# POSTECH-CVLab/PyTorch-StudioGAN

Measured on AMD Instinct MI355X. Metric: images/sec (G+D step) BigGAN ImageNet-128 bs256, higher is better.
Workload: dtype bf16

## Files before the change

include/sgamd.h:

```cpp
#ifndef SGAMD_H
#define SGAMD_H
#include <stdint.h>
#ifdef __cplusplus
extern "C" {
#endif

typedef void* sg_stream_t;

#define SG_DTYPE_F32 0
#define SG_DTYPE_BF16 1
#define SG_DTYPE_F64 2

#define SG_PIX_RELU 1
#define SG_PIX_UPSAMPLE 2
#define SG_PIX_QUAD 4
#define SG_PIX_TRANSPOSED 8
#define SG_EPI_OUT_F32 1
#define SG_EPI_ATOMIC 2
#define SG_EPI_POOL 4
#define SG_EPI_RELU 8
#define SG_EPI_RES_F32 16

const char* sg_last_error(void);
int sg_version(void);
int sg_prof_enable(int on);
int sg_prof_collect(double* out, int nkinds);

typedef struct {
  int dtype;
  int N, Hs, Ws, C, ldx;
  int Ho, Wo, Cout;
  int R, S, stride, pad_h, pad_w;
  int pix_flags, epi_flags;
  float alpha, beta;
  const void* x; const void* w;
  const float* bias; const void* res; const void* mask; void* out; const float* alpha_ptr;
  int ldo, ldr, ldm;
} sg_conv_fwd_desc;
int sg_conv2d_fwd(const sg_conv_fwd_desc* d, sg_stream_t stream);
int sg_set_f32_mode(int mode);
int sg_get_f32_mode(void);
long long sg_f32_split_launches(int mode);
long long sg_ew_vec_launches(void);

typedef struct {
  sg_conv_fwd_desc main;
  const void* x2; const void* w2; const float* bias2;
  int C2, ldx2, x2_up;
  float* stats;
} sg_conv_skip_desc;
int sg_conv2d_fwd_skip_stat_rows(const sg_conv_skip_desc* d);
int sg_conv2d_fwd_skip(const sg_conv_skip_desc* d, sg_stream_t stream);
int sg_conv2d_fwd_skip_ok(const sg_conv_skip_desc* d);
long long sg_conv_rs_launches(void);

typedef struct {
  sg_conv_fwd_desc conv;
  const float* pre; const float* post; const float* noise;
  long long noise_stride;
} sg_modconv_desc;
int sg_modconv2d_fwd(const sg_modconv_desc* d, sg_stream_t stream);
int sg_modconv2d_ok(const sg_modconv_desc* d);
long long sg_modconv_launches(void);
int sg_modconv_dcoef(const float* w, const float* s, float* Q, float* d, int N, int C, int Cout, int RS, sg_stream_t stream);
int sg_modconv_reduce_slabs(int P);
int sg_modconv_reduce(int dtype, const void* a, const void* b, const float* rowsub, long long rowsub_stride, const float* scale, void* out, float* part,
                      float* rowsum, int N, int P, int C, int lda, int ldb, sg_stream_t stream);

#define SG_Q_POOL 0
#define SG_Q_UP 1
typedef struct {
  int dtype, form;
  int N, Hl, Wl;
  int C, ldx, Cout;
  int pix_flags, epi_flags;
  float alpha, beta;
  const void* x; const void* wq;
  const float* bias; const void* res; const void* mask; void* out; const float* alpha_ptr;
  int ldo, ldr, ldm;
  const void* x2; const void* w2q; const float* bias2;
  int C2, ldx2;
  float* stats;
  int x2_norelu;
} sg_convq_desc;
int sg_conv2d_q_stat_rows(const sg_convq_desc* d);
int sg_conv2d_q(const sg_convq_desc* d, sg_stream_t stream);
int sg_conv2d_q_ok(const sg_convq_desc* d);
int sg_quad_pack(int dtype, int mode, const void* src, void* dst, int M, int Cs, sg_stream_t stream);
typedef struct { const void* src; void* dst; int M, Cs, mode, pad_; } sg_quad_item;
int sg_quad_pack_batch(int dtype, const sg_quad_item* items_dev, const sg_quad_item* items_host, int n, sg_stream_t stream);
typedef struct {
  int dtype, form;
  int N, Hl, Wl;
  int C, ldx, x_flags;
  int Cout, ldg;
  float alpha; const float* alpha_ptr;
  const void* x; const void* dy; float* dw; float* dbias;
  float* work; long long work_floats;
  int splits;
} sg_convq_wgrad_desc;
int sg_conv2d_q_wgrad_plan(const sg_convq_wgrad_desc* d, int* splits, long long* work_floats);
int sg_conv2d_q_wgrad(const sg_convq_wgrad_desc* d, sg_stream_t stream);
int sg_prof_collect_ex(double* out, int nkinds);
int sg_prof_collect_tags(double* out, int ntags);

typedef struct {
  int dtype;
  int N;
  int xHs, xWs, C, ldx, x_flags;
  int gHs, gWs, Cout, ldg, g_flags;
  int Ho, Wo;
  int R, S, stride, pad_h, pad_w;
  float alpha;
  const void* x; const void* dy; float* dw;
  const float* alpha_ptr;
  int splits;
  int no_tr;
  float* work; long long work_floats;
  float* dbias;
} sg_conv_wgrad_desc;
int sg_conv2d_wgrad(const sg_conv_wgrad_desc* d, sg_stream_t stream);
int sg_conv2d_wgrad_fuses_bias(const sg_conv_wgrad_desc* d);
int sg_conv2d_wgrad_plan(const sg_conv_wgrad_desc* d, int* splits, long long* work_floats);

typedef struct {
  int dtype, p_form, q_form;
  int I, J, K, batch;
  const void* p; long long p_bstride; int ldp;
  const void* q; long long q_bstride; int ldq;
  void* out; long long out_bstride; int ldo;
  const float* bias; const void* res; long long res_bstride; int ldr; float beta;
  float alpha; const float* alpha_ptr;
  int epi_flags; int splits; int no_tr;
} sg_gemm_desc;
int sg_gemm(const sg_gemm_desc* d, sg_stream_t stream);
typedef struct { const float* w; const float* y; const float* bias; float* out; int rows, K, ldy, ldo; } sg_linear_item;
int sg_linear_group(const sg_linear_item* items_dev, const sg_linear_item* items_host, int n, int B, sg_stream_t stream);
typedef struct { const float* w; const float* y; const float* bias; float* out; int rows, K, ldy, ldo; float wscale, bscale, oscale; int pad_; } sg_linear_item_scaled;
int sg_linear_group_scaled(const sg_linear_item_scaled* items_dev, const sg_linear_item_scaled* items_host, int n, int B, sg_stream_t stream);
long long sg_linear_group_scaled_launches(void);

int sg_nchw_to_nhwc(int dtype, const float* src, void* dst, int N, int C, int H, int W, int ldo, sg_stream_t s);
int sg_nhwc_to_nchw(int dtype, const void* src, float* dst, int N, int C, int H, int W, int lds, int apply_tanh, sg_stream_t s);
int sg_nchw_grad_to_nhwc(int dtype, const float* dy, const float* y, void* dst, int N, int C, int H, int W, int ldo, int apply_tanh, sg_stream_t s);
int sg_avgpool2_fwd(int dtype, const void* x, void* y, int N, int H, int W, int C, sg_stream_t s);
int sg_avgpool2_bwd(int dtype, const void* dy, void* dx, int N, int H, int W, int C, sg_stream_t s);
int sg_maxpool2_fwd(int dtype, const void* x, int ldx, void* y, int ldy, uint8_t* idx, int N, int H, int W, int C, sg_stream_t s);
int sg_maxpool2_bwd(int dtype, const void* dy, int ldy, const uint8_t* idx, void* dx, int ldx, int N, int H, int W, int C, sg_stream_t s);
int sg_softmax_rows(int dtype, const float* s_in, void* p_out, long long rows, int cols, sg_stream_t st);
int sg_softmax_rows_bwd(int dtype, const void* p, const float* dp, void* ds, long long rows, int cols, sg_stream_t st);
int sg_convert(int src_dtype, int dst_dtype, const void* x, void* y, long long n, sg_stream_t s);
int sg_add_relu(int dtype, const void* a, const void* x, void* out, long long n, sg_stream_t s);
int sg_relu_mask(int dtype, const void* dy, const void* x, void* dx, long long n, sg_stream_t s);
int sg_axpby(int dtype, const void* x, void* y, long long n, float a, float b, sg_stream_t s);
int sg_dot(int dtype, const void* x, const void* y, long long n, float* out, float scale, const float* scale_ptr, sg_stream_t s);
int sg_colsum(int dtype, const void* x, int ldx, const void* mask, int ldm, long long rows, int C, float* out, float alpha, sg_stream_t s);

int sg_bn_partial_stats(int dtype, const void* x, int ldx, long long rows, int C, double* partial, sg_stream_t s);
int sg_bn_stats_from_tiles(const float* stats, int nrows, int C, double* partial, sg_stream_t s);
int sg_bn_finalize(const double* partial, double count, int C, float eps, float momentum, float* mean, float* invstd,
                   float* running_mean, float* running_var, sg_stream_t s);
typedef void* sg_comm_t;
int sg_comm_unique_id(void* out128);
int sg_comm_init_rank(const void* id128, int nranks, int rank, sg_comm_t* comm);
int sg_comm_size(sg_comm_t comm, int* nranks);
int sg_comm_destroy(sg_comm_t comm);
int sg_allreduce_flat(sg_comm_t comm, void* buf, long long count, int dtype, sg_stream_t s);
int sg_bn_stats_sync(int dtype, const void* x, int ldx, long long rows, int C, double* partial, sg_comm_t comm, float eps, float momentum,
                     float* mean, float* invstd, float* running_mean, float* running_var, sg_stream_t s);
int sg_reduce_scatter_flat(sg_comm_t comm, float* buf, long long per_rank, sg_stream_t s);
int sg_allgather_flat(sg_comm_t comm, float* buf, long long per_rank, sg_stream_t s);

typedef void* sg_p2p_t;
int sg_p2p_create(int world, int rank, long long max_doubles, sg_p2p_t* out, void* handle_out64);
int sg_p2p_connect(sg_p2p_t p, const void* handles);
int sg_p2p_destroy(sg_p2p_t p);
int sg_p2p_timeouts(sg_p2p_t p, int* count);
int sg_p2p_allreduce_f64(sg_p2p_t p, double* buf, int n, sg_stream_t s);
int sg_bn_finalize_p2p(sg_p2p_t p, const double* partial, double count, int C, float eps, float momentum, float* mean, float* invstd,
                       float* running_mean, float* running_var, sg_stream_t s);
int sg_bn_stats_sync_p2p(int dtype, const void* x, int ldx, long long rows, int C, double* partial, sg_p2p_t p, float eps, float momentum,
                         float* mean, float* invstd, float* running_mean, float* running_var, sg_stream_t s);
int sg_bn_from_running(const float* running_mean, const float* running_var, int C, float eps, float* mean, float* invstd, sg_stream_t s);
int sg_bn_apply(int dtype, const void* x, void* y, int N, long long HW, int C, const float* mean, const float* invstd,
                const float* gain, const float* bias, int gb_stride_n, int relu, sg_stream_t s);
int sg_bn_bwd_reduce(int dtype, const void* x, const void* dy, int N, long long HW, int C, const float* mean, const float* invstd,
                     const float* gain, const float* bias, int gb_stride_n, int relu, float* sums, sg_stream_t s);
int sg_bn_bwd_finalize(const float* sums, int N, int C, const float* gain, int gb_stride_n, float* dgain, float* dbias,
                       double* chan, sg_stream_t s);
int sg_bn_bwd_apply(int dtype, const void* x, const void* dy, void* dx, int N, long long HW, int C, const float* mean,
                    const float* invstd, const float* gain, const float* bias, int gb_stride_n, int relu,
                    const double* chan, double count, int use_batch_stats, sg_stream_t s);
int sg_bn_bwd_apply_res(int dtype, const void* x, const void* dy, void* dx, int N, long long HW, int C, const float* mean,
                        const float* invstd, const float* gain, const float* bias, int gb_stride_n, int relu,
                        const double* chan, double count, int use_batch_stats, const void* res, sg_stream_t s);

int sg_bn_bwd2_reduce(int dtype, const void* x, const void* dy, const void* u, int N, long long HW, int C, const float* mean,
                      const float* invstd, const float* gain, const float* bias, int relu, float* sums, sg_stream_t s);
int sg_bn_bwd2_finalize(const float* sums, int N, int C, double* chan, sg_stream_t s);
int sg_bn_bwd2_dgain(const double* chan_local, const double* chan, double count, const float* invstd, int C,
                     int use_batch_stats, float* dgain, sg_stream_t s);
int sg_bn_bwd2_apply(int dtype, const void* x, const void* dy, const void* u, void* g_dy, void* g_x, int N, long long HW, int C,
                     const float* mean, const float* invstd, const float* gain, const float* bias, int relu, const double* chan,
                     double count, int use_batch_stats, sg_stream_t s);

int sg_cbn_bwd2_reduce(int dtype, const void* x, const void* dy, const void* u, int N, long long HW, int C, const float* mean,
                       const float* invstd, const float* gain, const float* bias, int gb_stride_n, int relu, float* sums,
                       sg_stream_t s);
int sg_cbn_bwd2_finalize(const float* sums, int N, int C, const float* gain, const float* A, int gb_stride_n, double* chan,
                         sg_stream_t s);
int sg_cbn_bwd2_dgain(const float* sums, const double* chan, double count, const float* invstd, int N, int C, int gb_stride_n,
                      int use_batch_stats, float* dgain, sg_stream_t s);
int sg_cbn_bwd2_apply(int dtype, const void* x, const void* dy, const void* u, void* g_dy, void* g_x, int N, long long HW, int C,
                      const float* mean, const float* invstd, const float* gain, const float* bias, const float* A, const float* B,
                      int gb_stride_n, int relu, const double* chan, double count, int use_batch_stats, sg_stream_t s);

typedef struct {
  const float* w;
  float* u; float* v;
  float* sigma;
  float* u_snap; float* v_snap;
  void* w_fwd;
  void* w_dgrad;
  float* w_f32;
  int rows, cols;
  int Cin, RS;
  int do_power_iter;
  int apply_sn;
  int rows_pad;
  long long work_off;
  int trans;
  int dgrad_noflip;
  int Cin_pad;
} sg_sn_layer;
int sg_sn_forward(int dtype, const sg_sn_layer* layers_dev, const sg_sn_layer* layers_host, int n, float eps, float* work, long long work_floats, sg_stream_t s);

typedef struct {
  const float* dwt;
  const float* w;
  const float* u; const float* v; const float* sigma;
  float* dw;
  int rows, cols, Cin, RS, natural, apply_sn, trans;
  int Cin_pad;
} sg_sn_bwd_layer;
int sg_sn_backward(const sg_sn_bwd_layer* layers_dev, const sg_sn_bwd_layer* layers_host, int n, float* work, long long work_floats, sg_stream_t s);

int sg_embedding_fwd(const float* table, const int64_t* idx, float* out, int B, int dim, int num, sg_stream_t s);
int sg_embedding_bwd(const float* dout, const int64_t* idx, float* dtable, int B, int dim, int num, sg_stream_t s);
int sg_relu_sum_hw_fwd(int dtype, const void* x, float* h, int B, int HW, int C, sg_stream_t s);
int sg_relu_sum_hw_bwd(int dtype, const void* x, const float* dh, void* dx, int B, int HW, int C, sg_stream_t s);
int sg_pd_head_fwd(const float* h, const float* w1, const float* b1, const float* emb, float* adv, int B, int C, sg_stream_t s);
int sg_pd_head_bwd(const float* h, const float* w1, const float* emb, const float* dadv, float* dh, float* dw1, float* db1,
                   float* demb, int B, int C, sg_stream_t s);
int sg_loss_d(int kind, const float* real, const float* fake, int B, float* loss, float* d_real, float* d_fake, sg_stream_t s);
int sg_loss_g(int kind, const float* fake, int B, float* loss, float* d_fake, sg_stream_t s);

int sg_interp_rows(const float* real, const float* fake, const float* alpha, float* out, int B, long long n, sg_stream_t s);
int sg_gp_fwd(int kind, const float* grads, int B, long long n, float* norms, float* loss, sg_stream_t s);
int sg_gp_bwd(int kind, const float* grads, const float* norms, const float* gout, float* dgrads, int B, long long n, sg_stream_t s);
int sg_masked_sum_hw(int dtype, const void* t, const void* x, float* out, int B, int HW, int C, sg_stream_t s);

int sg_attn_fwd_flash_ok(int B, int HW, int HW4, int Dp, int Cg);
int sg_attn_fwd_fused(const void* theta, const void* phi, const void* g, float* lse, void* O, float* O32, int B, int HW, int HW4, int Dp, int Cg, sg_stream_t s);
int sg_attn_bwd_fused_ok(int B, int HW, int HW4, int Dp, int Cg);
int sg_attn_bwd_fused(const void* theta, const void* phi, const void* g, const void* dO, const float* O32, const float* lse, float* delta, void* dtheta, void* dphi,
                      void* dg, int B, int HW, int HW4, int Dp, int Cg, sg_stream_t s);

int sg_attn_proj_ok(int B, int H, int W, int C, int ldx, int Dp, int Cg);
int sg_attn_proj_fwd(const void* x, int ldx, const void* w_theta, const void* w_phi, const void* w_g, void* theta, void* phi, void* g,
                     uint8_t* idx_phi, uint8_t* idx_g, int B, int H, int W, int C, int Dp, int Cg, int relu, sg_stream_t s);
int sg_attn_proj_bwd_data(const void* dtheta, const void* dphi, const void* dg, const uint8_t* idx_phi, const uint8_t* idx_g, const void* wd_theta,
                          const void* wd_phi, const void* wd_g, const void* res, void* dx, int B, int H, int W, int C, int Dp, int Cg, sg_stream_t s);

int sg_slice_up_fwd(int dtype, const void* x, void* y, int N, int Hs, int Ws, int ldx, int C, int up, sg_stream_t s);
int sg_slice_up_bwd(int dtype, const void* dy, void* dx, int N, int Hs, int Ws, int ldx, int C, int up, sg_stream_t s);
int sg_copy_channels(int dtype, const void* src, int ld_src, void* dst, int ld_dst, long long rows, int C, sg_stream_t s);

int sg_adam_ema(float* p, const float* g, float* m, float* v, float* ema, long long n, float lr, float beta1, float beta2,
                float eps, float wd, int step, float ema_decay, float grad_scale, sg_stream_t s);
int sg_ema_lerp(const float* src, float* ema, long long n, float decay, sg_stream_t s);

int sg_lecam(const float* real, const float* fake, int B, float ema_real, float ema_fake, float* loss, float* d_real, float* d_fake, sg_stream_t s);
int sg_u8_to_nhwc(int dtype, const uint8_t* x, const uint8_t* flip, void* y, int N, int H, int W, int cpad, sg_stream_t s);

int sg_quantize_resize_normalize(int dtype, const float* x, void* out, uint8_t* quant_out, int N, int C, int H, int W,
                                 int OH, int OW, int quantize, sg_stream_t s);
int sg_quantize_resize_normalize_ms(int dtype, const float* x, void* out, uint8_t* quant_out, int N, int C, int H, int W,
                                    int OH, int OW, int quantize, const float* mean, const float* std, sg_stream_t s);
int sg_pool2d(int dtype, const void* x, void* y, int N, int H, int W, int C, int k, int stride, int pad, int mode, int ldy, int c_off, sg_stream_t s);
int sg_pil_resize_normalize(int dtype, const float* x, void* out, float* tmp, int N, int C, int H, int W, int OH, int OW,
                            const int* bounds_h, const double* kk_h, int ksize_h, const int* bounds_v, const double* kk_v, int ksize_v,
                            int quantize, sg_stream_t s);
int sg_pil_resize_normalize_ms(int dtype, const float* x, void* out, float* tmp, int N, int C, int H, int W, int OH, int OW,
                               const int* bounds_h, const double* kk_h, int ksize_h, const int* bounds_v, const double* kk_v, int ksize_v,
                               int quantize, const float* mean, const float* std, sg_stream_t s);
int sg_global_avgpool(int dtype, const void* x, float* y, int N, int HW, int C, sg_stream_t s);
int sg_topk_hits(const float* scores, int ld, int ncls, const int64_t* labels, int k, int N, uint8_t* hits, sg_stream_t s);
int sg_topk_select(const float* x, int n, int k, float* vals, int* idx, sg_stream_t s);
int sg_topk_scatter(const float* g, const int* idx, int k, float* dx, int n, sg_stream_t s);
int sg_feat_moments_accumulate(const float* f, int n, int C, double* sum_f, double* sum_ff, sg_stream_t s);
int sg_gather_images_u8(const uint8_t* src, const int64_t* idx, const uint8_t* flip, uint8_t* dst, int B, int H, int W,
                        const int64_t* lab_src, int64_t* lab_dst, sg_stream_t s);
int sg_row_normalize_fwd(const float* x, float* y, float* inv, int rows, int cols, float eps, sg_stream_t s);
int sg_row_normalize_bwd(const float* y, const float* inv, const float* dy, float* dx, int rows, int cols, sg_stream_t s);
int sg_row_dot(const float* a, const float* b, float* p, int rows, int cols, sg_stream_t s);
int sg_row_scale(const float* g, const float* x, float* out, int rows, int cols, int accumulate, sg_stream_t s);
int sg_class_loss(int kind, const float* z, const int64_t* label, int rows, int cols, float* row_loss, float* loss, float* dz, sg_stream_t s);
int sg_contrastive_loss(int kind, const float* S, const float* p, const int64_t* label, int B, float temperature, float m_p,
                        float* row_loss, float* loss, float* dS, float* dp, sg_stream_t s);
int sg_gather_cols(const float* z, const int64_t* label, int rows, int cols, float* out, sg_stream_t s);
int sg_scatter_cols(const float* g, const int64_t* label, int rows, int cols, float* dz, sg_stream_t s);
int sg_layernorm_rows(int out_dtype, const float* x, long long pitch, const float* gamma, const float* beta, void* y, long long ldo, int rows, int C,
                      float eps, sg_stream_t s);
int sg_vit_tokens(const float* patch, const float* cls, const float* pos, float* x, int B, int N, int C, sg_stream_t s);
int sg_gelu_f32(const float* x, float* y, long long n, sg_stream_t s);
int sg_tok_gemm(int epi, const void* a, int lda, const void* w, const float* bias, void* out, int ldo, int M, int N, int K, sg_stream_t s);
int sg_mha_fwd_ok(int B, int N, int H, int D);
int sg_mha_fwd(const void* qkv, void* out, int B, int N, int H, int D, float scale, sg_stream_t s);
long long sg_tok_gemm_launches(void);
long long sg_mha_launches(void);

int sg_row_sqnorm(const float* f, int n, int C, float* sq, sg_stream_t s);
int sg_kth_smallest_rows(const float* D, long long ld, int rows, int cols, int k, const float* row_add, float* out, sg_stream_t s);
int sg_prdc_rows(const float* D, long long ld, int rows, int cols, const float* row_add, const float* r2_row, const float* r2_col,
                 int* col_cnt, uint8_t* row_any, float* row_min, sg_stream_t s);
int sg_chol_lower(double* A, int n, int* flag, sg_stream_t s);
int sg_dgemm_tn(const double* A, const double* B, double* C, int n, sg_stream_t s);
int sg_jacobi_sweep(double* M, int n, double* offd, sg_stream_t s);
int sg_row_norm_sum(const double* M, int n, double* out, sg_stream_t s);
int sg_seg_moments(const float* f, const long long* seg, int K, int C, double* mu, double* tr, sg_stream_t s);
int sg_seg_cross_gram(const float* fa, const long long* sega, const double* mua, const float* fb, const long long* segb, const double* mub, int K, int C,
                      double* M, const long long* moff, sg_stream_t s);
int sg_seg_nuclear_norm(const double* M, const long long* moff, const int* rows, const int* cols, int K, int max_sweeps, double tol,
                        double* nuc, double* offd, int* sweeps, sg_stream_t s);
int sg_seg_nuclear_fits(int rows, int cols);
int sg_seg_nuclear_lds_budget(void);

int sg_bias_act(int dtype, const void* x, const void* b, const void* xref, const void* yref, const void* dy, void* y, long long n,
                long long step_b, int size_b, int grad, int act, float alpha, float gain, float clamp, sg_stream_t s);
int sg_upfirdn2d(int dtype, const void* x, const float* f, void* y, int planes, int H, int W, int fh, int fw, int upx, int upy,
                 int downx, int downy, int padx0, int padx1, int pady0, int pady1, int flip_filter, float gain, sg_stream_t s);
int sg_filtered_lrelu(int dtype, const void* x, const float* fu, const float* fd, const void* b, void* y, int N, int C, int H, int W,
                      int fu_n, int fd_n, int up, int down, int px0, int px1, int py0, int py1, float gain, float slope, float clamp,
                      int flip_filter, sg_stream_t s);
int sg_fir_bias_act_nhwc(int dtype, const void* x, const float* f, void* y, const float* noise, long long noise_stride, const float* bias,
                         int N, int Hi, int Wi, int C, int fh, int fw, int padx0, int padx1, int pady0, int pady1, int flip_filter,
                         float filter_gain, int act, float alpha, float gain, float clamp, sg_stream_t s);
long long sg_fir_bias_act_launches(void);

#define SG_AUG_BRIGHTNESS 1
#define SG_AUG_SATURATION 2
#define SG_AUG_CONTRAST 4
#define SG_AUG_FLIP 8
#define SG_AUG_TRANSLATE 16
#define SG_AUG_TRANSLATE_REFLECT 32
#define SG_AUG_CUTOUT 64
typedef struct {
  int N, C, H, W;
  int ops;
  int cut_h, cut_w;
  int max_t;
  const float* color;
  const int* geom;
} sg_aug_desc;
int sg_augment_work_floats(const sg_aug_desc* d);
int sg_augment_fwd(const sg_aug_desc* d, const float* x, float* y, float* work, sg_stream_t s);
int sg_augment_bwd(const sg_aug_desc* d, const float* dy, float* dx, float* work, sg_stream_t s);
int sg_mse_work_floats(void);
int sg_mse_fwd(const float* a, const float* b, long long n, float* work, float* loss, sg_stream_t s);
int sg_mse_bwd(const float* a, const float* b, const float* gout, long long n, float* da, float* db, sg_stream_t s);
int sg_loss_ls_d(const float* real, const float* fake, int B, float* loss, float* d_real, float* d_fake, sg_stream_t s);
int sg_loss_ls_g(const float* fake, int B, float* loss, float* d_fake, sg_stream_t s);
int sg_fm_work_floats(int C);
int sg_fm_loss(const float* real_h, const float* fake_h, int B, int C, float* work, float* loss, float* d_fake, sg_stream_t s);
int sg_exp_fwd(const float* x, float* y, long long n, sg_stream_t s);
int sg_exp_bwd(const float* dy, const float* y, float* dx, long long n, sg_stream_t s);
int sg_normal_nll(const float* x, const float* mu, const float* var, int B, int K, float* loss, float* dmu, float* dvar, sg_stream_t s);
int sg_maxpool2_gather(int dtype, const void* x, int ldx, const uint8_t* idx, void* y, int ldy, int N, int H, int W, int C, sg_stream_t s);
int sg_softmax_rows_bwd2(const float* P, const float* dP, const float* u, float* gP, long long rows, int cols, sg_stream_t s);
int sg_scale_by_ptr(int dtype, const void* x, const float* sigma, void* y, long long n, sg_stream_t s);
int sg_tanh_bwd(const float* dy, const float* y, float* t, long long n, sg_stream_t s);
int sg_tanh_bwd2(const float* g, const float* dy, const float* y, float* out, long long n, sg_stream_t s);
int sg_clamp_flat(float* p, long long n, float lo, float hi, sg_stream_t s);
int sg_select_rows(const uint8_t* flag, const float* a, const float* b, float* out, int N, long long row, sg_stream_t s);
int sg_sign_count(const float* logit, int B, float* acc, sg_stream_t s);
int sg_reflect_pad2d_fwd(const float* x, float* y, int planes, int H, int W, int l, int r, int t, int b, sg_stream_t s);
int sg_reflect_pad2d_bwd(const float* dy, float* dx, int planes, int H, int W, int l, int r, int t, int b, sg_stream_t s);
int sg_affine_sample_fwd(const float* x, const float* theta, float* y, int N, int C, int Hi, int Wi, int Ho, int Wo, sg_stream_t s);
int sg_affine_sample_bwd(const float* dy, const float* theta, float* dx, int N, int C, int Hi, int Wi, int Ho, int Wo, sg_stream_t s);
int sg_color_affine(const float* x, const float* M, float* y, int N, int C, int HW, int transpose, sg_stream_t s);
int sg_fir_reflect(const float* x, const float* taps, float* y, int N, int C, int H, int W, int T, int axis, int transpose, sg_stream_t s);
int sg_ada_noise_cutout(const float* x, const float* noise, const float* sigma, const float* cut, float* y, int N, int C, int H, int W, sg_stream_t s);

#ifdef __cplusplus
}
#endif
#endif
```

pytorch-studiogan_amd/_lib.py:

```python
import ctypes as C
import os
import subprocess
import sys

import torch

_HERE = os.path.dirname(os.path.abspath(__file__))
LIB_PATH = os.path.join(_HERE, "libsgamd.so")
if os.environ.get("SG_LIBSGAMD"):
    LIB_PATH = os.path.abspath(os.environ["SG_LIBSGAMD"])
CSRC = os.path.join(_HERE, "csrc")

F32, BF16, F64 = 0, 1, 2
PIX_RELU, PIX_UPSAMPLE, PIX_QUAD, PIX_TRANSPOSED = 1, 2, 4, 8
Q_POOL, Q_UP = 0, 1
EPI_OUT_F32, EPI_ATOMIC, EPI_POOL, EPI_RELU, EPI_RES_F32 = 1, 2, 4, 8, 16

_vp, _i, _f, _ll = C.c_void_p, C.c_int, C.c_float, C.c_longlong


class ConvFwdDesc(C.Structure):
    _fields_ = [("dtype", _i), ("N", _i), ("Hs", _i), ("Ws", _i), ("C", _i), ("ldx", _i), ("Ho", _i), ("Wo", _i), ("Cout", _i),
                ("R", _i), ("S", _i), ("stride", _i), ("pad_h", _i), ("pad_w", _i), ("pix_flags", _i), ("epi_flags", _i),
                ("alpha", _f), ("beta", _f), ("x", _vp), ("w", _vp), ("bias", _vp), ("res", _vp), ("mask", _vp), ("out", _vp),
                ("alpha_ptr", _vp), ("ldo", _i), ("ldr", _i), ("ldm", _i)]


class ConvSkipDesc(C.Structure):
    _fields_ = [("main", ConvFwdDesc), ("x2", _vp), ("w2", _vp), ("bias2", _vp), ("C2", _i), ("ldx2", _i), ("x2_up", _i), ("stats", _vp)]


class ModConvDesc(C.Structure):
    _fields_ = [("conv", ConvFwdDesc), ("pre", _vp), ("post", _vp), ("noise", _vp), ("noise_stride", _ll)]


class ConvWgradDesc(C.Structure):
    _fields_ = [("dtype", _i), ("N", _i), ("xHs", _i), ("xWs", _i), ("C", _i), ("ldx", _i), ("x_flags", _i), ("gHs", _i), ("gWs", _i),
                ("Cout", _i), ("ldg", _i), ("g_flags", _i), ("Ho", _i), ("Wo", _i), ("R", _i), ("S", _i), ("stride", _i),
                ("pad_h", _i), ("pad_w", _i), ("alpha", _f), ("x", _vp), ("dy", _vp), ("dw", _vp), ("alpha_ptr", _vp),
                ("splits", _i), ("no_tr", _i), ("work", _vp), ("work_floats", _ll), ("dbias", _vp)]


class ConvQDesc(C.Structure):
    _fields_ = [("dtype", _i), ("form", _i), ("N", _i), ("Hl", _i), ("Wl", _i), ("C", _i), ("ldx", _i), ("Cout", _i),
                ("pix_flags", _i), ("epi_flags", _i), ("alpha", _f), ("beta", _f), ("x", _vp), ("wq", _vp), ("bias", _vp), ("res", _vp),
                ("mask", _vp), ("out", _vp), ("alpha_ptr", _vp), ("ldo", _i), ("ldr", _i), ("ldm", _i),
                ("x2", _vp), ("w2q", _vp), ("bias2", _vp), ("C2", _i), ("ldx2", _i), ("stats", _vp), ("x2_norelu", _i)]


class ConvQWgradDesc(C.Structure):
    _fields_ = [("dtype", _i), ("form", _i), ("N", _i), ("Hl", _i), ("Wl", _i), ("C", _i), ("ldx", _i), ("x_flags", _i), ("Cout", _i),
                ("ldg", _i), ("alpha", _f), ("alpha_ptr", _vp), ("x", _vp), ("dy", _vp), ("dw", _vp), ("dbias", _vp), ("work", _vp),
                ("work_floats", _ll), ("splits", _i)]


class QuadItem(C.Structure):
    _fields_ = [("src", _vp), ("dst", _vp), ("M", _i), ("Cs", _i), ("mode", _i), ("pad_", _i)]


class LinearItem(C.Structure):
    _fields_ = [("w", _vp), ("y", _vp), ("bias", _vp), ("out", _vp), ("rows", _i), ("K", _i), ("ldy", _i), ("ldo", _i)]


class LinearItemScaled(C.Structure):
    _fields_ = [("w", _vp), ("y", _vp), ("bias", _vp), ("out", _vp), ("rows", _i), ("K", _i), ("ldy", _i), ("ldo", _i),
                ("wscale", _f), ("bscale", _f), ("oscale", _f), ("pad_", _i)]


class GemmDesc(C.Structure):
    _fields_ = [("dtype", _i), ("p_form", _i), ("q_form", _i), ("I", _i), ("J", _i), ("K", _i), ("batch", _i),
                ("p", _vp), ("p_bstride", _ll), ("ldp", _i), ("q", _vp), ("q_bstride", _ll), ("ldq", _i),
                ("out", _vp), ("out_bstride", _ll), ("ldo", _i), ("bias", _vp), ("res", _vp), ("res_bstride", _ll), ("ldr", _i),
                ("beta", _f), ("alpha", _f), ("alpha_ptr", _vp), ("epi_flags", _i), ("splits", _i), ("no_tr", _i)]


class SnLayer(C.Structure):
    _fields_ = [("w", _vp), ("u", _vp), ("v", _vp), ("sigma", _vp), ("u_snap", _vp), ("v_snap", _vp), ("w_fwd", _vp), ("w_dgrad", _vp),
                ("w_f32", _vp), ("rows", _i), ("cols", _i), ("Cin", _i), ("RS", _i), ("do_power_iter", _i), ("apply_sn", _i),
                ("rows_pad", _i), ("work_off", _ll), ("trans", _i), ("dgrad_noflip", _i), ("Cin_pad", _i)]


class SnBwdLayer(C.Structure):
    _fields_ = [("dwt", _vp), ("w", _vp), ("u", _vp), ("v", _vp), ("sigma", _vp), ("dw", _vp), ("rows", _i), ("cols", _i),
                ("Cin", _i), ("RS", _i), ("natural", _i), ("apply_sn", _i), ("trans", _i), ("Cin_pad", _i)]


class AugDesc(C.Structure):
    _fields_ = [("N", _i), ("C", _i), ("H", _i), ("W", _i), ("ops", _i), ("cut_h", _i), ("cut_w", _i), ("max_t", _i), ("color", _vp), ("geom", _vp)]


AUG_BRIGHTNESS, AUG_SATURATION, AUG_CONTRAST, AUG_FLIP, AUG_TRANSLATE, AUG_TRANSLATE_REFLECT, AUG_CUTOUT = 1, 2, 4, 8, 16, 32, 64

_lib = None


def build(force=False, verbose=False):
    cmd = ["make", "-C", CSRC, "-j", str(max(2, os.cpu_count() or 2))]
    if force:
        subprocess.run(["make", "-C", CSRC, "clean"], check=True, stdout=subprocess.DEVNULL)
    res = subprocess.run(cmd, stdout=subprocess.PIPE, stderr=subprocess.STDOUT, text=True)
    if verbose or res.returncode != 0:
        sys.stderr.write(res.stdout)
    if res.returncode != 0:
        raise RuntimeError("building libsgamd.so failed")
    return LIB_PATH


_PROTOS = {
    "sg_prof_enable": [_i],
    "sg_prof_collect": [C.POINTER(C.c_double), _i],
    "sg_conv2d_fwd": [C.POINTER(ConvFwdDesc), _vp],
    "sg_conv2d_fwd_skip": [C.POINTER(ConvSkipDesc), _vp],
    "sg_conv2d_fwd_skip_ok": [C.POINTER(ConvSkipDesc)],
    "sg_conv_rs_launches": [],
    "sg_modconv2d_fwd": [C.POINTER(ModConvDesc), _vp],
    "sg_modconv2d_ok": [C.POINTER(ModConvDesc)],
    "sg_modconv_launches": [],
    "sg_modconv_dcoef": [_vp, _vp, _vp, _vp, _i, _i, _i, _i, _vp],
    "sg_modconv_reduce_slabs": [_i],
    "sg_modconv_reduce": [_i, _vp, _vp, _vp, _ll, _vp, _vp, _vp, _vp, _i, _i, _i, _i, _i, _vp],
    "sg_conv2d_q": [C.POINTER(ConvQDesc), _vp],
    "sg_conv2d_q_ok": [C.POINTER(ConvQDesc)],
    "sg_conv2d_q_stat_rows": [C.POINTER(ConvQDesc)],
    "sg_conv2d_fwd_skip_stat_rows": [C.POINTER(ConvSkipDesc)],
    "sg_bn_stats_from_tiles": [_vp, _i, _i, _vp, _vp],
    "sg_quad_pack": [_i, _i, _vp, _vp, _i, _i, _vp],
    "sg_quad_pack_batch": [_i, _vp, C.POINTER(QuadItem), _i, _vp],
    "sg_linear_group": [_vp, C.POINTER(LinearItem), _i, _i, _vp],
    "sg_linear_group_scaled": [_vp, C.POINTER(LinearItemScaled), _i, _i, _vp],
    "sg_linear_group_scaled_launches": [],
    "sg_conv2d_q_wgrad_plan": [C.POINTER(ConvQWgradDesc), C.POINTER(_i), C.POINTER(_ll)],
    "sg_conv2d_q_wgrad": [C.POINTER(ConvQWgradDesc), _vp],
    "sg_prof_collect_ex": [C.POINTER(C.c_double), _i],
    "sg_prof_collect_tags": [C.POINTER(C.c_double), _i],
    "sg_conv2d_wgrad": [C.POINTER(ConvWgradDesc), _vp],
    "sg_conv2d_wgrad_plan": [C.POINTER(ConvWgradDesc), C.POINTER(_i), C.POINTER(_ll)],
    "sg_conv2d_wgrad_fuses_bias": [C.POINTER(ConvWgradDesc)],
    "sg_gemm": [C.POINTER(GemmDesc), _vp],
    "sg_nchw_to_nhwc": [_i, _vp, _vp, _i, _i, _i, _i, _i, _vp],
    "sg_nhwc_to_nchw": [_i, _vp, _vp, _i, _i, _i, _i, _i, _i, _vp],
    "sg_nchw_grad_to_nhwc": [_i, _vp, _vp, _vp, _i, _i, _i, _i, _i, _i, _vp],
    "sg_avgpool2_fwd": [_i, _vp, _vp, _i, _i, _i, _i, _vp],
    "sg_avgpool2_bwd": [_i, _vp, _vp, _i, _i, _i, _i, _vp],
    "sg_maxpool2_fwd": [_i, _vp, _i, _vp, _i, _vp, _i, _i, _i, _i, _vp],
    "sg_maxpool2_bwd": [_i, _vp, _i, _vp, _vp, _i, _i, _i, _i, _i, _vp],
    "sg_softmax_rows": [_i, _vp, _vp, _ll, _i, _vp],
    "sg_softmax_rows_bwd": [_i, _vp, _vp, _vp, _ll, _i, _vp],
    "sg_axpby": [_i, _vp, _vp, _ll, _f, _f, _vp],
    "sg_convert": [_i, _i, _vp, _vp, _ll, _vp],
    "sg_add_relu": [_i, _vp, _vp, _vp, _ll, _vp],
    "sg_relu_mask": [_i, _vp, _vp, _vp, _ll, _vp],
    "sg_dot": [_i, _vp, _vp, _ll, _vp, _f, _vp, _vp],
    "sg_colsum": [_i, _vp, _i, _vp, _i, _ll, _i, _vp, _f, _vp],
    "sg_bn_partial_stats": [_i, _vp, _i, _ll, _i, _vp, _vp],
    "sg_bn_finalize": [_vp, C.c_double, _i, _f, _f, _vp, _vp, _vp, _vp, _vp],
    "sg_comm_unique_id": [_vp],
    "sg_comm_init_rank": [_vp, _i, _i, C.POINTER(_vp)],
    "sg_comm_size": [_vp, C.POINTER(_i)],
    "sg_comm_destroy": [_vp],
    "sg_allreduce_flat": [_vp, _vp, _ll, _i, _vp],
    "sg_bn_stats_sync": [_i, _vp, _i, _ll, _i, _vp, _vp, _f, _f, _vp, _vp, _vp, _vp, _vp],
    "sg_set_f32_mode": [_i],
    "sg_get_f32_mode": [],
    "sg_f32_split_launches": [_i],
    "sg_ew_vec_launches": [],
    "sg_reduce_scatter_flat": [_vp, _vp, _ll, _vp],
    "sg_allgather_flat": [_vp, _vp, _ll, _vp],
    "sg_p2p_create": [_i, _i, _ll, C.POINTER(_vp), _vp],
    "sg_p2p_connect": [_vp, _vp],
    "sg_p2p_destroy": [_vp],
    "sg_p2p_timeouts": [_vp, C.POINTER(_i)],
    "sg_p2p_allreduce_f64": [_vp, _vp, _i, _vp],
    "sg_bn_finalize_p2p": [_vp, _vp, C.c_double, _i, _f, _f, _vp, _vp, _vp, _vp, _vp],
    "sg_bn_stats_sync_p2p": [_i, _vp, _i, _ll, _i, _vp, _vp, _f, _f, _vp, _vp, _vp, _vp, _vp],
    "sg_bn_from_running": [_vp, _vp, _i, _f, _vp, _vp, _vp],
    "sg_bn_apply": [_i, _vp, _vp, _i, _ll, _i, _vp, _vp, _vp, _vp, _i, _i, _vp],
    "sg_bn_bwd_reduce": [_i, _vp, _vp, _i, _ll, _i, _vp, _vp, _vp, _vp, _i, _i, _vp, _vp],
    "sg_bn_bwd_finalize": [_vp, _i, _i, _vp, _i, _vp, _vp, _vp, _vp],
    "sg_bn_bwd_apply": [_i, _vp, _vp, _vp, _i, _ll, _i, _vp, _vp, _vp, _vp, _i, _i, _vp, C.c_double, _i, _vp],
    "sg_bn_bwd_apply_res": [_i, _vp, _vp, _vp, _i, _ll, _i, _vp, _vp, _vp, _vp, _i, _i, _vp, C.c_double, _i, _vp, _vp],
    "sg_bn_bwd2_reduce": [_i, _vp, _vp, _vp, _i, _ll, _i, _vp, _vp, _vp, _vp, _i, _vp, _vp],
    "sg_bn_bwd2_finalize": [_vp, _i, _i, _vp, _vp],
    "sg_bn_bwd2_dgain": [_vp, _vp, C.c_double, _vp, _i, _i, _vp, _vp],
    "sg_bn_bwd2_apply": [_i, _vp, _vp, _vp, _vp, _vp, _i, _ll, _i, _vp, _vp, _vp, _vp, _i, _vp, C.c_double, _i, _vp],
    "sg_cbn_bwd2_reduce": [_i, _vp, _vp, _vp, _i, _ll, _i, _vp, _vp, _vp, _vp, _i, _i, _vp, _vp],
    "sg_cbn_bwd2_finalize": [_vp, _i, _i, _vp, _vp, _i, _vp, _vp],
    "sg_cbn_bwd2_dgain": [_vp, _vp, C.c_double, _vp, _i, _i, _i, _i, _vp, _vp],
    "sg_cbn_bwd2_apply": [_i, _vp, _vp, _vp, _vp, _vp, _i, _ll, _i, _vp, _vp, _vp, _vp, _vp, _vp, _i, _i, _vp, C.c_double, _i, _vp],
    "sg_attn_fwd_flash_ok": [_i, _i, _i, _i, _i],
    "sg_attn_fwd_fused": [_vp, _vp, _vp, _vp, _vp, _vp, _i, _i, _i, _i, _i, _vp],
    "sg_attn_bwd_fused_ok": [_i, _i, _i, _i, _i],
    "sg_attn_bwd_fused": [_vp, _vp, _vp, _vp, _vp, _vp, _vp, _vp, _vp, _vp, _i, _i, _i, _i, _i, _vp],
    "sg_attn_proj_ok": [_i, _i, _i, _i, _i, _i, _i],
    "sg_attn_proj_fwd": [_vp, _i, _vp, _vp, _vp, _vp, _vp, _vp, _vp, _vp, _i, _i, _i, _i, _i, _i, _i, _vp],
    "sg_attn_proj_bwd_data": [_vp, _vp, _vp, _vp, _vp, _vp, _vp, _vp, _vp, _vp, _i, _i, _i, _i, _i, _i, _vp],
    "sg_slice_up_fwd": [_i, _vp, _vp, _i, _i, _i, _i, _i, _i, _vp],
    "sg_slice_up_bwd": [_i, _vp, _vp, _i, _i, _i, _i, _i, _i, _vp],
    "sg_copy_channels": [_i, _vp, _i, _vp, _i, _ll, _i, _vp],
    "sg_interp_rows": [_vp, _vp, _vp, _vp, _i, _ll, _vp],
    "sg_gp_fwd": [_i, _vp, _i, _ll, _vp, _vp, _vp],
    "sg_gp_bwd": [_i, _vp, _vp, _vp, _vp, _i, _ll, _vp],
    "sg_masked_sum_hw": [_i, _vp, _vp, _vp, _i, _i, _i, _vp],
    "sg_sn_forward": [_i, _vp, C.POINTER(SnLayer), _i, _f, _vp, _ll, _vp],
    "sg_sn_backward": [_vp, C.POINTER(SnBwdLayer), _i, _vp, _ll, _vp],
    "sg_embedding_fwd": [_vp, _vp, _vp, _i, _i, _i, _vp],
    "sg_embedding_bwd": [_vp, _vp, _vp, _i, _i, _i, _vp],
    "sg_relu_sum_hw_fwd": [_i, _vp, _vp, _i, _i, _i, _vp],
    "sg_relu_sum_hw_bwd": [_i, _vp, _vp, _vp, _i, _i, _i, _vp],
    "sg_pd_head_fwd": [_vp, _vp, _vp, _vp, _vp, _i, _i, _vp],
    "sg_pd_head_bwd": [_vp, _vp, _vp, _vp, _vp, _vp, _vp, _vp, _i, _i, _vp],
    "sg_loss_d": [_i, _vp, _vp, _i, _vp, _vp, _vp, _vp],
    "sg_loss_g": [_i, _vp, _i, _vp, _vp, _vp],
    "sg_adam_ema": [_vp, _vp, _vp, _vp, _vp, _ll, _f, _f, _f, _f, _f, _i, _f, _f, _vp],
    "sg_ema_lerp": [_vp, _vp, _ll, _f, _vp],
    "sg_quantize_resize_normalize": [_i, _vp, _vp, _vp, _i, _i, _i, _i, _i, _i, _i, _vp],
    "sg_pil_resize_normalize": [_i, _vp, _vp, _vp, _i, _i, _i, _i, _i, _i, _vp, _vp, _i, _vp, _vp, _i, _i, _vp],
    "sg_quantize_resize_normalize_ms": [_i, _vp, _vp, _vp, _i, _i, _i, _i, _i, _i, _i, C.POINTER(_f), C.POINTER(_f), _vp],
    "sg_pil_resize_normalize_ms": [_i, _vp, _vp, _vp, _i, _i, _i, _i, _i, _i, _vp, _vp, _i, _vp, _vp, _i, _i, C.POINTER(_f), C.POINTER(_f), _vp],
    "sg_layernorm_rows": [_i, _vp, _ll, _vp, _vp, _vp, _ll, _i, _i, _f, _vp],
    "sg_vit_tokens": [_vp, _vp, _vp, _vp, _i, _i, _i, _vp],
    "sg_gelu_f32": [_vp, _vp, _ll, _vp],
    "sg_tok_gemm": [_i, _vp, _i, _vp, _vp, _vp, _i, _i, _i, _i, _vp],
    "sg_mha_fwd_ok": [_i, _i, _i, _i],
    "sg_mha_fwd": [_vp, _vp, _i, _i, _i, _i, _f, _vp],
    "sg_tok_gemm_launches": [],
    "sg_mha_launches": [],
    "sg_pool2d": [_i, _vp, _vp, _i, _i, _i, _i, _i, _i, _i, _i, _i, _i, _vp],
    "sg_global_avgpool": [_i, _vp, _vp, _i, _i, _i, _vp],
    "sg_feat_moments_accumulate": [_vp, _i, _i, _vp, _vp, _vp],
    "sg_topk_hits": [_vp, _i, _i, _vp, _i, _i, _vp, _vp],
    "sg_row_normalize_fwd": [_vp, _vp, _vp, _i, _i, _f, _vp],
    "sg_row_normalize_bwd": [_vp, _vp, _vp, _vp, _i, _i, _vp],
    "sg_row_dot": [_vp, _vp, _vp, _i, _i, _vp],
    "sg_row_scale": [_vp, _vp, _vp, _i, _i, _i, _vp],
    "sg_class_loss": [_i, _vp, _vp, _i, _i, _vp, _vp, _vp, _vp],
    "sg_contrastive_loss": [_i, _vp, _vp, _vp, _i, _f, _f, _vp, _vp, _vp, _vp, _vp],
    "sg_gather_cols": [_vp, _vp, _i, _i, _vp, _vp],
    "sg_scatter_cols": [_vp, _vp, _i, _i, _vp, _vp],
    "sg_chol_lower": [_vp, _i, _vp, _vp],
    "sg_dgemm_tn": [_vp, _vp, _vp, _i, _vp],
    "sg_jacobi_sweep": [_vp, _i, _vp, _vp],
    "sg_row_norm_sum": [_vp, _i, _vp, _vp],
    "sg_seg_moments": [_vp, _vp, _i, _i, _vp, _vp, _vp],
    "sg_seg_cross_gram": [_vp, _vp, _vp, _vp, _vp, _vp, _i, _i, _vp, _vp, _vp],
    "sg_seg_nuclear_norm": [_vp, _vp, _vp, _vp, _i, _i, C.c_double, _vp, _vp, _vp, _vp],
    "sg_seg_nuclear_fits": [_i, _i],
    "sg_seg_nuclear_lds_budget": [],
    "sg_row_sqnorm": [_vp, _i, _i, _vp, _vp],
    "sg_kth_smallest_rows": [_vp, _ll, _i, _i, _i, _vp, _vp, _vp],
    "sg_prdc_rows": [_vp, _ll, _i, _i, _vp, _vp, _vp, _vp, _vp, _vp, _vp],
    "sg_topk_select": [_vp, _i, _i, _vp, _vp, _vp],
    "sg_lecam": [_vp, _vp, _i, _f, _f, _vp, _vp, _vp, _vp],
    "sg_u8_to_nhwc": [_i, _vp, _vp, _vp, _i, _i, _i, _i, _vp],
    "sg_gather_images_u8": [_vp, _vp, _vp, _vp, _i, _i, _i, _vp, _vp, _vp],
    "sg_topk_scatter": [_vp, _vp, _i, _vp, _i, _vp],
    "sg_bias_act": [_i, _vp, _vp, _vp, _vp, _vp, _vp, _ll, _ll, _i, _i, _i, _f, _f, _f, _vp],
    "sg_upfirdn2d": [_i, _vp, _vp, _vp, _i, _i, _i, _i, _i, _i, _i, _i, _i, _i, _i, _i, _i, _i, _f, _vp],
    "sg_filtered_lrelu": [_i, _vp, _vp, _vp, _vp, _vp, _i, _i, _i, _i, _i, _i, _i, _i, _i, _i, _i, _i, _f, _f, _f, _i, _vp],
    "sg_fir_bias_act_nhwc": [_i, _vp, _vp, _vp, _vp, _ll, _vp, _i, _i, _i, _i, _i, _i, _i, _i, _i, _i, _i, _f, _i, _f, _f, _f, _vp],
    "sg_fir_bias_act_launches": [],
    "sg_augment_work_floats": [C.POINTER(AugDesc)],
    "sg_augment_fwd": [C.POINTER(AugDesc), _vp, _vp, _vp, _vp],
    "sg_augment_bwd": [C.POINTER(AugDesc), _vp, _vp, _vp, _vp],
    "sg_mse_work_floats": [],
    "sg_mse_fwd": [_vp, _vp, _ll, _vp, _vp, _vp],
    "sg_mse_bwd": [_vp, _vp, _vp, _ll, _vp, _vp, _vp],
    "sg_loss_ls_d": [_vp, _vp, _i, _vp, _vp, _vp, _vp],
    "sg_loss_ls_g": [_vp, _i, _vp, _vp, _vp],
    "sg_fm_work_floats": [_i],
    "sg_fm_loss": [_vp, _vp, _i, _i, _vp, _vp, _vp, _vp],
    "sg_exp_fwd": [_vp, _vp, _ll, _vp],
    "sg_exp_bwd": [_vp, _vp, _vp, _ll, _vp],
    "sg_normal_nll": [_vp, _vp, _vp, _i, _i, _vp, _vp, _vp, _vp],
    "sg_maxpool2_gather": [_i, _vp, _i, _vp, _vp, _i, _i, _i, _i, _i, _vp],
    "sg_softmax_rows_bwd2": [_vp, _vp, _vp, _vp, _ll, _i, _vp],
    "sg_scale_by_ptr": [_i, _vp, _vp, _vp, _ll, _vp],
    "sg_tanh_bwd": [_vp, _vp, _vp, _ll, _vp],
    "sg_tanh_bwd2": [_vp, _vp, _vp, _vp, _ll, _vp],
    "sg_clamp_flat": [_vp, _ll, _f, _f, _vp],
    "sg_select_rows": [_vp, _vp, _vp, _vp, _i, _ll, _vp],
    "sg_sign_count": [_vp, _i, _vp, _vp],
    "sg_reflect_pad2d_fwd": [_vp, _vp, _i, _i, _i, _i, _i, _i, _i, _vp],
    "sg_reflect_pad2d_bwd": [_vp, _vp, _i, _i, _i, _i, _i, _i, _i, _vp],
    "sg_affine_sample_fwd": [_vp, _vp, _vp, _i, _i, _i, _i, _i, _i, _vp],
    "sg_affine_sample_bwd": [_vp, _vp, _vp, _i, _i, _i, _i, _i, _i, _vp],
    "sg_color_affine": [_vp, _vp, _vp, _i, _i, _i, _i, _vp],
    "sg_fir_reflect": [_vp, _vp, _vp, _i, _i, _i, _i, _i, _i, _i, _vp],
    "sg_ada_noise_cutout": [_vp, _vp, _vp, _vp, _vp, _i, _i, _i, _i, _vp],
}


def exported_symbols():
    return sorted(list(_PROTOS.keys()) + ["sg_last_error", "sg_version"])


def lib():
    global _lib
    if _lib is None:
        if not os.path.exists(LIB_PATH):
            raise RuntimeError(
                f"{LIB_PATH} is missing: run `python -c 'import __graft_entry__ as g; g.build()'` (make -C {CSRC}). "
                "There is no CPU/eager fallback on the product path.")
        l = C.CDLL(LIB_PATH)
        l.sg_last_error.restype = C.c_char_p
        l.sg_version.restype = _i
        for name, args in _PROTOS.items():
            fn = getattr(l, name)
            fn.argtypes = args
            fn.restype = _i
        l.sg_conv_rs_launches.restype = _ll
        l.sg_modconv_launches.restype = _ll
        l.sg_tok_gemm_launches.restype = _ll
        l.sg_mha_launches.restype = _ll
        l.sg_f32_split_launches.restype = _ll
        l.sg_ew_vec_launches.restype = _ll
        l.sg_linear_group_scaled_launches.restype = _ll
        l.sg_fir_bias_act_launches.restype = _ll
        f32_mode = {"bf16x3": 3, "bf16x6": 6}.get(os.environ.get("SG_F32_MODE", "exact"), 0)
        if f32_mode:
            l.sg_set_f32_mode(f32_mode)
        _lib = l
    return _lib


def check(rc, name=""):
    if rc != 0:
        raise RuntimeError(f"{name}: {lib().sg_last_error().decode()} (rc={rc})")


_STATE_WRITERS = frozenset(("sg_adam_ema", "sg_ema_lerp", "sg_allreduce_flat", "sg_clamp_flat", "sg_allgather_flat"))
write_epoch = [0]


def call(name, *args):
    if name in _STATE_WRITERS:
        write_epoch[0] += 1
    rc = getattr(lib(), name)(*args)
    if rc != 0:
        raise RuntimeError(f"{name}: {lib().sg_last_error().decode()} (rc={rc})")


def stream():
    return torch.cuda.current_stream().cuda_stream


def upload_bytes(raw, device):
    t = torch.frombuffer(bytearray(raw), dtype=torch.uint8)
    if torch.device(device).type == "cuda":
        return t.pin_memory().to(device, non_blocking=True)
    return t.to(device)


def dt(t):
    d = t if isinstance(t, torch.dtype) else t.dtype
    if d == torch.float32:
        return F32
    if d == torch.bfloat16:
        return BF16
    raise RuntimeError(f"unsupported dtype {d} (float32 / bfloat16 only)")


def require_gpu(dev):
    if dev.type != "cuda":
        raise RuntimeError("studiogan_amd modules run on the GPU only (no CPU fallback on the product path)")


def ptr(t):
    if t is None:
        return None
    if not t.is_cuda:
        raise RuntimeError("studiogan_amd kernels need a GPU tensor (no CPU fallback on the product path)")
    return t.data_ptr()
```

pytorch-studiogan_amd/backbones/big_resnet.py:

```python
import torch
import torch.nn as nn

from .. import functional as F
from .. import ops
from ..bank import get_bank
from .heads import build_heads, apply_heads


def _dtype(mixed_precision):
    return torch.bfloat16 if mixed_precision else torch.float32


def _need_graph(module, *inputs):
    if not torch.is_grad_enabled():
        return False
    for t in inputs:
        if torch.is_tensor(t) and t.requires_grad:
            return True
    return any(p.requires_grad for p in module.parameters())


class GenBlock(nn.Module):
    def __init__(self, in_channels, out_channels, g_cond_mtd, affine_input_dim, MODULES):
        super().__init__()
        self.g_cond_mtd = g_cond_mtd
        self.bn1 = MODULES.g_bn(affine_input_dim, in_channels, MODULES)
        self.bn2 = MODULES.g_bn(affine_input_dim, out_channels, MODULES)
        self.activation = MODULES.g_act_fn
        self.conv2d0 = MODULES.g_conv2d(in_channels=in_channels, out_channels=out_channels, kernel_size=1, stride=1, padding=0)
        self.conv2d1 = MODULES.g_conv2d(in_channels=in_channels, out_channels=out_channels, kernel_size=3, stride=1, padding=1)
        self.conv2d2 = MODULES.g_conv2d(in_channels=out_channels, out_channels=out_channels, kernel_size=3, stride=1, padding=1)

    def forward_nhwc(self, x, affine, slot):
        link = F.GradLink()
        h = self.bn1.forward_nhwc(x, affine, slot, relu=True, link=link)
        h = self.conv2d1.forward_nhwc(h, slot, in_upsample=True, stats=True)
        h = self.bn2.forward_nhwc(h, affine, slot, relu=True)
        return ops.conv_skip_nhwc(self.conv2d2, self.conv2d0, h, x, slot, skip_upsample=True, link=link, stats=True)


class Generator(nn.Module):
    def __init__(self, z_dim, g_shared_dim, img_size, g_conv_dim, apply_attn, attn_g_loc, g_cond_mtd, num_classes, g_init, g_depth,
                 mixed_precision, MODULES, MODEL):
        super().__init__()
        g_in_dims_collection = {
            "32": [g_conv_dim * 4, g_conv_dim * 4, g_conv_dim * 4],
            "64": [g_conv_dim * 16, g_conv_dim * 8, g_conv_dim * 4, g_conv_dim * 2],
            "128": [g_conv_dim * 16, g_conv_dim * 16, g_conv_dim * 8, g_conv_dim * 4, g_conv_dim * 2],
            "256": [g_conv_dim * 16, g_conv_dim * 16, g_conv_dim * 8, g_conv_dim * 8, g_conv_dim * 4, g_conv_dim * 2],
            "512": [g_conv_dim * 16, g_conv_dim * 16, g_conv_dim * 8, g_conv_dim * 8, g_conv_dim * 4, g_conv_dim * 2, g_conv_dim]
        }
        g_out_dims_collection = {
            "32": [g_conv_dim * 4, g_conv_dim * 4, g_conv_dim * 4],
            "64": [g_conv_dim * 8, g_conv_dim * 4, g_conv_dim * 2, g_conv_dim],
            "128": [g_conv_dim * 16, g_conv_dim * 8, g_conv_dim * 4, g_conv_dim * 2, g_conv_dim],
            "256": [g_conv_dim * 16, g_conv_dim * 8, g_conv_dim * 8, g_conv_dim * 4, g_conv_dim * 2, g_conv_dim],
            "512": [g_conv_dim * 16, g_conv_dim * 8, g_conv_dim * 8, g_conv_dim * 4, g_conv_dim * 2, g_conv_dim, g_conv_dim]
        }
        self.z_dim = z_dim
        self.g_shared_dim = g_shared_dim
        self.g_cond_mtd = g_cond_mtd
        self.num_classes = num_classes
        self.mixed_precision = mixed_precision
        self.MODEL = MODEL
        self.in_dims = g_in_dims_collection[str(img_size)]
        self.out_dims = g_out_dims_collection[str(img_size)]
        self.bottom = 4
        self.num_blocks = len(self.in_dims)
        self.chunk_size = z_dim // (self.num_blocks + 1)
        self.affine_input_dim = self.chunk_size
        assert self.z_dim % (self.num_blocks + 1) == 0, "z_dim should be divided by the number of blocks"
        self.info_type = getattr(MODEL, "info_type", "N/A")
        self.g_info_injection = getattr(MODEL, "g_info_injection", "N/A")
        info_dim = 0
        if self.info_type in ("discrete", "both"):
            info_dim += MODEL.info_num_discrete_c * MODEL.info_dim_discrete_c
        if self.info_type in ("continuous", "both"):
            info_dim += MODEL.info_num_conti_c
        if self.info_type != "N/A":
            if self.g_info_injection == "concat":
                self.info_mix_linear = MODULES.g_linear(in_features=self.z_dim + info_dim, out_features=self.z_dim, bias=True)
            elif self.g_info_injection == "cBN":
                self.affine_input_dim += self.g_shared_dim
                self.info_proj_linear = MODULES.g_linear(in_features=info_dim, out_features=self.g_shared_dim, bias=True)
            else:
                raise NotImplementedError(f"g_info_injection = {self.g_info_injection}")

        self.linear0 = MODULES.g_linear(in_features=self.chunk_size, out_features=self.in_dims[0] * self.bottom * self.bottom, bias=True)
        if self.g_cond_mtd != "W/O":
            self.affine_input_dim += self.g_shared_dim
            self.shared = ops.embedding(num_embeddings=self.num_classes, embedding_dim=self.g_shared_dim)

        blocks = []
        for index in range(self.num_blocks):
            blocks += [[GenBlock(in_channels=self.in_dims[index], out_channels=self.out_dims[index], g_cond_mtd=self.g_cond_mtd,
                                 affine_input_dim=self.affine_input_dim, MODULES=MODULES)]]
            if index + 1 in attn_g_loc and apply_attn:
                blocks += [[ops.SelfAttention(self.out_dims[index], is_generator=True, MODULES=MODULES)]]
        self.blocks = nn.ModuleList([nn.ModuleList(block) for block in blocks])

        self.bn4 = ops.batchnorm_2d(in_features=self.out_dims[-1])
        self.activation = MODULES.g_act_fn
        self.conv2d5 = MODULES.g_conv2d(in_channels=self.out_dims[-1], out_channels=3, kernel_size=3, stride=1, padding=1)
        self.tanh = nn.Tanh()
        self.conv2d5._sg_rows_pad = 8
        ops.init_weights(self.modules, g_init)
        ops.adopt(self, _dtype(mixed_precision))

    def forward(self, z, label, shared_label=None, eval=False):
        dtype = self.compute_dtype
        bank = get_bank(self, dtype)
        slot = bank.begin_forward(_need_graph(self, z, shared_label))
        affine_list = []
        if self.info_type != "N/A":
            if self.g_info_injection == "concat":
                z = self.info_mix_linear.forward_rt(z, slot)
            else:
                z, z_info = z[:, :self.z_dim], z[:, self.z_dim:]
                affine_list.append(self.info_proj_linear.forward_rt(z_info, slot))
        zs = torch.split(z, self.chunk_size, 1)
        z0 = zs[0]
        if self.g_cond_mtd != "W/O":
            if shared_label is None:
                shared_label = self.shared(label)
            affine_list.append(shared_label)
        if len(affine_list) == 0:
            affines = [item for item in zs[1:]]
        else:
            affines = [torch.cat(affine_list + [item], 1) for item in zs[1:]]

        pairs, counter = [], 0
        for blocklist in self.blocks:
            for block in blocklist:
                if not isinstance(block, ops.SelfAttention):
                    if isinstance(block.bn1, ops.ConditionalBatchNorm2d):
                        pairs += [(block.bn1, affines[counter]), (block.bn2, affines[counter])]
                    counter += 1
        F.cbn_prefetch(slot, pairs)

        act = self.linear0.forward_rt(z0, slot)
        act = F.NchwToNhwcFn.apply(act.view(-1, self.in_dims[0], self.bottom, self.bottom), dtype)
        act = ops.block_boundary(self, -1, act)
        counter = 0
        nxt = bank.boundaries(self.blocks) if bank.exchange is not None else None
        with ops.bump_batches_tracked(self):
            for bi, blocklist in enumerate(self.blocks):
                for block in blocklist:
                    if isinstance(block, ops.SelfAttention):
                        act = block.forward_nhwc(act, slot)
                    else:
                        act = block.forward_nhwc(act, affines[counter], slot)
                        counter += 1
                if nxt is not None:
                    act = bank.mark(act, nxt[bi])
                act = ops.block_boundary(self, bi, act)
            act = self.bn4.forward_nhwc(act, relu=True)
        act = self.conv2d5.forward_nhwc(act, slot)
        return F.NhwcToNchwFn.apply(act, True, 3)


class DiscOptBlock(nn.Module):
    def __init__(self, in_channels, out_channels, apply_d_sn, MODULES):
        super().__init__()
        self.apply_d_sn = apply_d_sn
        self.conv2d0 = MODULES.d_conv2d(in_channels=in_channels, out_channels=out_channels, kernel_size=1, stride=1, padding=0)
        self.conv2d1 = MODULES.d_conv2d(in_channels=in_channels, out_channels=out_channels, kernel_size=3, stride=1, padding=1)
        self.conv2d2 = MODULES.d_conv2d(in_channels=out_channels, out_channels=out_channels, kernel_size=3, stride=1, padding=1)
        if not apply_d_sn:
            self.bn0 = MODULES.d_bn(in_features=in_channels)
            self.bn1 = MODULES.d_bn(in_features=out_channels)
        self.activation = MODULES.d_act_fn
        self.average_pooling = nn.AvgPool2d(2)
        self.cpad = 8 if (apply_d_sn and in_channels < 8) else 0
        if self.cpad:
            self.conv2d1._sg_cin_pad = self.conv2d0._sg_cin_pad = self.cpad

    def forward_nhwc(self, x, slot):
        h = self.conv2d1.forward_nhwc(x, slot)
        if not self.apply_d_sn:
            h = self.bn1.forward_nhwc(h, relu=True)
            h = self.conv2d2.forward_nhwc(h, slot, out_pool=True)
        else:
            if self.cpad == 8 and h.dtype == torch.bfloat16 and not x.requires_grad:
                return ops.conv_skip_nhwc(self.conv2d2, self.conv2d0, h, x, slot, in_relu=True, out_pool=True, skip_relu=False)
            h = self.conv2d2.forward_nhwc(h, slot, in_relu=True, out_pool=True)
        x0 = F.AvgPool2Fn.apply(x)
        if not self.apply_d_sn:
            x0 = self.bn0.forward_nhwc(x0)
        return self.conv2d0.forward_nhwc(x0, slot, res=h)


class DiscBlock(nn.Module):
    def __init__(self, in_channels, out_channels, apply_d_sn, MODULES, downsample=True):
        super().__init__()
        self.apply_d_sn = apply_d_sn
        self.downsample = downsample
        self.activation = MODULES.d_act_fn
        self.ch_mismatch = in_channels != out_channels
        if self.ch_mismatch or downsample:
            self.conv2d0 = MODULES.d_conv2d(in_channels=in_channels, out_channels=out_channels, kernel_size=1, stride=1, padding=0)
            if not apply_d_sn:
                self.bn0 = MODULES.d_bn(in_features=in_channels)
        self.conv2d1 = MODULES.d_conv2d(in_channels=in_channels, out_channels=out_channels, kernel_size=3, stride=1, padding=1)
        self.conv2d2 = MODULES.d_conv2d(in_channels=out_channels, out_channels=out_channels, kernel_size=3, stride=1, padding=1)
        if not apply_d_sn:
            self.bn1 = MODULES.d_bn(in_features=in_channels)
            self.bn2 = MODULES.d_bn(in_features=out_channels)
        self.average_pooling = nn.AvgPool2d(2)

    def forward_nhwc(self, x, slot):
        if self.apply_d_sn:
            if self.downsample or self.ch_mismatch:
                link = F.GradLink()
                h = self.conv2d1.forward_nhwc(x, slot, in_relu=True, link=link)
                return ops.conv_skip_nhwc(self.conv2d2, self.conv2d0, h, x, slot, in_relu=True, out_pool=self.downsample, link=link)
            h = self.conv2d1.forward_nhwc(x, slot, in_relu=True)
            h = self.conv2d2.forward_nhwc(h, slot, in_relu=True, out_pool=False)
            return F.AddReluFn.apply(h, x)
        h = self.bn1.forward_nhwc(x, relu=True)
        h = self.conv2d1.forward_nhwc(h, slot)
        h = self.bn2.forward_nhwc(h, relu=True)
        h = self.conv2d2.forward_nhwc(h, slot, out_pool=self.downsample)
        if self.downsample or self.ch_mismatch:
            x0 = self.bn0.forward_nhwc(x)
            return self.conv2d0.forward_nhwc(x0, slot, out_pool=self.downsample, res=h)
        return F.AddFn.apply(h, x)


class Discriminator(nn.Module):
    def __init__(self, img_size, d_conv_dim, apply_d_sn, apply_attn, attn_d_loc, d_cond_mtd, aux_cls_type, d_embed_dim, normalize_d_embed,
                 num_classes, d_init, d_depth, mixed_precision, MODULES, MODEL):
        super().__init__()
        d_in_dims_collection = {
            "32": [3] + [d_conv_dim * 2, d_conv_dim * 2, d_conv_dim * 2],
            "64": [3] + [d_conv_dim, d_conv_dim * 2, d_conv_dim * 4, d_conv_dim * 8],
            "128": [3] + [d_conv_dim, d_conv_dim * 2, d_conv_dim * 4, d_conv_dim * 8, d_conv_dim * 16],
            "256": [3] + [d_conv_dim, d_conv_dim * 2, d_conv_dim * 4, d_conv_dim * 8, d_conv_dim * 8, d_conv_dim * 16],
            "512": [3] + [d_conv_dim, d_conv_dim, d_conv_dim * 2, d_conv_dim * 4, d_conv_dim * 8, d_conv_dim * 8, d_conv_dim * 16]
        }
        d_out_dims_collection = {
            "32": [d_conv_dim * 2, d_conv_dim * 2, d_conv_dim * 2, d_conv_dim * 2],
            "64": [d_conv_dim, d_conv_dim * 2, d_conv_dim * 4, d_conv_dim * 8, d_conv_dim * 16],
            "128": [d_conv_dim, d_conv_dim * 2, d_conv_dim * 4, d_conv_dim * 8, d_conv_dim * 16, d_conv_dim * 16],
            "256": [d_conv_dim, d_conv_dim * 2, d_conv_dim * 4, d_conv_dim * 8, d_conv_dim * 8, d_conv_dim * 16, d_conv_dim * 16],
            "512": [d_conv_dim, d_conv_dim, d_conv_dim * 2, d_conv_dim * 4, d_conv_dim * 8, d_conv_dim * 8, d_conv_dim * 16, d_conv_dim * 16]
        }
        d_down = {
            "32": [True, True, False, False],
            "64": [True, True, True, True, False],
            "128": [True, True, True, True, True, False],
            "256": [True, True, True, True, True, True, False],
            "512": [True, True, True, True, True, True, True, False]
        }
        self.d_cond_mtd = d_cond_mtd
        self.aux_cls_type = aux_cls_type
        self.normalize_d_embed = normalize_d_embed
        self.num_classes = num_classes
        self.mixed_precision = mixed_precision
        self.in_dims = d_in_dims_collection[str(img_size)]
        self.out_dims = d_out_dims_collection[str(img_size)]
        self.MODEL = MODEL
        down = d_down[str(img_size)]

        blocks = []
        for index in range(len(self.in_dims)):
            if index == 0:
                blocks += [[DiscOptBlock(in_channels=self.in_dims[index], out_channels=self.out_dims[index], apply_d_sn=apply_d_sn, MODULES=MODULES)]]
            else:
                blocks += [[DiscBlock(in_channels=self.in_dims[index], out_channels=self.out_dims[index], apply_d_sn=apply_d_sn,
                                      MODULES=MODULES, downsample=down[index])]]
            if index + 1 in attn_d_loc and apply_attn:
                blocks += [[ops.SelfAttention(self.out_dims[index], is_generator=False, MODULES=MODULES)]]
        self.blocks = nn.ModuleList([nn.ModuleList(block) for block in blocks])
        self.activation = MODULES.d_act_fn
        build_heads(self, MODULES, self.out_dims[-1], d_cond_mtd, aux_cls_type, d_embed_dim, num_classes, MODEL)
        if d_init:
            ops.init_weights(self.modules, d_init)
        ops.adopt(self, _dtype(mixed_precision))

    def forward(self, x, label, eval=False, adc_fake=False):
        dtype = self.compute_dtype
        bank = get_bank(self, dtype)
        slot = bank.begin_forward(_need_graph(self, x))
        h = ops.to_nhwc(x, dtype, self.blocks[0][0].cpad)
        nxt = bank.boundaries(self.blocks) if bank.exchange is not None else None
        for bi, blocklist in enumerate(self.blocks):
            for block in blocklist:
                h = block.forward_nhwc(h, slot)
            if nxt is not None:
                h = bank.mark(h, nxt[bi])
            h = ops.block_boundary(self, bi, h)
        hw = h.shape[1] * h.shape[2]
        h = F.ReluSumFn.apply(h)
        return apply_heads(self, h, label, slot, adc_fake, hw=hw)
```

pytorch-studiogan_amd/csrc/conv.hip:

```cpp
#include <type_traits>
#include "conv_common.h"
#include "conv_v2.h"

int g_sg_f32_mode = 0;
long long g_sg_f32_split_launches[2] = {0, 0};
extern "C" int sg_set_f32_mode(int mode) {
  SG_CHECK(mode == 0 || mode == 3 || mode == 6, "sg_set_f32_mode: 0 (exact fp32 MFMA), 3 (bf16x3 split) or 6 (bf16x6 split)");
  g_sg_f32_mode = mode;
  return 0;
}
extern "C" int sg_get_f32_mode() { return g_sg_f32_mode; }
extern "C" long long sg_f32_split_launches(int mode) {
  if (mode != 3 && mode != 6) return -1;
  return __atomic_load_n(&g_sg_f32_split_launches[mode == 6], __ATOMIC_RELAXED);
}

template <typename T, bool FAST>
static void conv_fwd_launch(const sg_conv_fwd_desc* d, const Epilogue<T>& e, int I, int J, int K, int pflags, hipStream_t st) {
  typedef StridedKC<T, FAST> LP;
  typedef ConvPixKC<T, FAST> LQ;
  LP lp;
  lp.base = (const T*)d->w; lp.bstride = 0; lp.ld = K; lp.rows = I; lp.K = K;
  lp.vec_ok = (K % ET<T>::VEC == 0) && aligned16(d->w);
  LQ lq;
  fill_geom<T>(lq.g, d->x, d->N, d->Hs, d->Ws, d->C, d->ldx, d->Ho, d->Wo, d->R, d->S, d->stride, d->pad_h, d->pad_w, pflags);
  lq.rows = J; lq.K = K;
  if constexpr (sizeof(T) == 4 && FAST) {
    const int mode = g_sg_f32_mode;
    if (mode == 3) { sg_f32_split_count(3); return conv_fwd_tiles<T, LP, LQ, 3>(lp, lq, e, I, J, K, st); }
    if (mode == 6) { sg_f32_split_count(6); return conv_fwd_tiles<T, LP, LQ, 6>(lp, lq, e, I, J, K, st); }
  }
  conv_fwd_tiles<T, LP, LQ, 0>(lp, lq, e, I, J, K, st);
}

static bool conv_fwd_v2_try(const ConvFwdProblem& pb, hipStream_t st) {
  const sg_conv_fwd_desc* d = pb.d;
  const int I = pb.I, J = pb.J, K = pb.K, pflags = pb.pflags;
  const char mode = env_mode("SG_CONV_V2");
  const bool force = mode == 'f';
  if (mode == '0' || (pflags & SG_PIX_TRANSPOSED)) return false;
  if (d->stride != 1 && (d->stride != 2 || (pflags & (SG_PIX_UPSAMPLE | SG_PIX_QUAD)))) return false;
  if (d->C % 8 || d->ldx % 8 || d->R * d->S > 25 || J < 256) return false;
  if (pb.xbytes >= (1ll << 31) || pb.wbytes >= (1ll << 30)) return false;
  if (!aligned16(d->x) || !aligned16(d->w)) return false;
  if (!epi_bf16_rows_ok(pb.e)) return false;
  const int tj = (J + 255) / 256;
  int best_tiles = 0;
  int best = cout_tile_search(I, tj, best_tiles);
  if (!best && I % 8 == 0 && I >= 32) {
    int best_pad = 0;
    for (int c = 0; c < 3; c++) {
      const int padded = ((I + kCoutTiles[c] - 1) / kCoutTiles[c]) * kCoutTiles[c];
      if (2 * padded > 3 * I) continue;
      const int tiles = (padded / kCoutTiles[c]) * tj;
      if (!best || padded < best_pad) { best = kCoutTiles[c]; best_pad = padded; best_tiles = tiles; }
    }
  }
  int min_tiles = 160;
  if (const char* mt = getenv("SG_CONV_V2_MIN_TILES")) { const int v = atoi(mt); if (v > 0) min_tiles = v; }
  if (!best || (best_tiles < min_tiles && !force)) return false;
  ConvV2Params p;
  p.x = (const bf16_t*)d->x; p.w = (const bf16_t*)d->w;
  p.N = d->N; p.Hs = d->Hs; p.Ws = d->Ws; p.C = d->C; p.ldx = d->ldx;
  p.Hin = d->Hs * (pb.up ? 2 : 1); p.Win = d->Ws * (pb.up ? 2 : 1); p.Ho = d->Ho; p.Wo = d->Wo;
  p.R = d->R; p.S = d->S; p.pad_h = d->pad_h; p.pad_w = d->pad_w; p.flags = pflags; p.stride = d->stride;
  p.I = I; p.J = J; p.K = K; p.cpt = d->C / 8; p.ntap = d->R * d->S;
  p.wshift = pb.wshift; p.hshift = pb.hshift;
  p.xbytes = (unsigned)pb.xbytes; p.wbytes = (unsigned)pb.wbytes;
  const Epilogue<bf16_t>& e = pb.e;
  int rc = 0;
  if (best == 192) rc = sg_launch_conv_v2<192, 4, 2, 256, 7>(p, e, st);
  else if (best == 128) rc = sg_launch_conv_v2<128, 4, 2, 256, 7>(p, e, st);
  else {
    if (J >= 512 * 256) rc = sg_launch_conv_v2<96, 8, 1, 512, 1>(p, e, st);
    else rc = sg_launch_conv_v2<96, 8, 1, 256, 1>(p, e, st);
  }
  return rc == 0;
}

template <typename T> static int conv_fwd_t(const sg_conv_fwd_desc* d, hipStream_t st) {
  const int K = d->R * d->S * d->C;
  const int I = d->Cout;
  const long long Jll = (long long)d->N * d->Ho * d->Wo;
  SG_CHECK(Jll < (1ll << 31), "sg_conv2d_fwd: too many output pixels");
  SG_CHECK((long long)d->N * d->Hs * d->Ws * d->ldx < (1ll << 31), "sg_conv2d_fwd: input tensor too large for 32-bit element offsets");
  const int J = (int)Jll;
  int pflags = d->pix_flags;
  if (d->epi_flags & SG_EPI_POOL) {
    SG_CHECK((d->Ho % 2 == 0) && (d->Wo % 2 == 0), "sg_conv2d_fwd: pooled output needs even Ho, Wo");
    pflags |= SG_PIX_QUAD;
  } else {
    pflags &= ~SG_PIX_QUAD;
  }
  const bool w_vec = (K % ET<T>::VEC == 0) && aligned16(d->w);
  const bool x_vec = (d->C % ET<T>::VEC == 0) && (d->ldx % ET<T>::VEC == 0) && aligned16(d->x);
  const Epilogue<T> e = make_epilogue<T>(d, I, J);
  const int prof = sg_prof_begin(st, 2.0 * (double)I * (double)J * (double)K, 0);
  int eng = SG_ENG_CONV_GEMM;
  if constexpr (std::is_same_v<T, bf16_t>) {
    if (w_vec && x_vec) {
      const ConvFwdProblem pb = conv_fwd_problem(d, e, I, J, K, pflags);
      if (sg_conv_fwd_sk_try(pb, st)) eng = SG_ENG_CONV_SK;
      else if (sg_conv_fwd_rs_try(pb, st)) eng = SG_ENG_CONV_RS;
      else if (sg_conv_fwd_v4_try(pb, st)) eng = SG_ENG_CONV_V4;
      else if (sg_conv_fwd_v3_try(pb, st)) eng = SG_ENG_CONV_V3;
      else if (conv_fwd_v2_try(pb, st)) eng = SG_ENG_CONV_V2;
    }
  }
  if (eng == SG_ENG_CONV_GEMM) {
    if (w_vec && x_vec) conv_fwd_launch<T, true>(d, e, I, J, K, pflags, st);
    else conv_fwd_launch<T, false>(d, e, I, J, K, pflags, st);
  }
  {
    const double es = sizeof(T), jout = (d->epi_flags & SG_EPI_POOL) ? (double)J / 4.0 : (double)J;
    const double b = es * ((double)d->N * d->Hs * d->Ws * d->C + (double)I * K + jout * I * (1.0 + (d->mask ? 1.0 : 0.0) + (d->res ? 1.0 : 0.0)));
    sg_prof_tag(prof, eng, b);
  }
  sg_prof_end(st, prof);
  SG_LAUNCH_CHECK();
  return 0;
}

static int conv_fwd_skip(const sg_conv_skip_desc* sk, hipStream_t st, bool dry) {
  const sg_conv_fwd_desc* d = &sk->main;
  if (d->dtype != SG_DTYPE_BF16 || d->R != 3 || d->S != 3 || d->stride != 1 || (d->pix_flags & (SG_PIX_UPSAMPLE | SG_PIX_TRANSPOSED))) return 0;
  const int K = 9 * d->C, I = d->Cout;
  const long long Jll = (long long)d->N * d->Ho * d->Wo;
  if (Jll >= (1ll << 31) || (long long)d->N * d->Hs * d->Ws * d->ldx >= (1ll << 31)) return 0;
  const int J = (int)Jll;
  int pflags = d->pix_flags;
  if (d->epi_flags & SG_EPI_POOL) { if ((d->Ho & 1) || (d->Wo & 1)) return 0; pflags |= SG_PIX_QUAD; } else pflags &= ~SG_PIX_QUAD;
  const ConvFwdProblem pb = conv_fwd_problem(d, make_epilogue<bf16_t>(d, I, J), I, J, K, pflags);
  if (dry) return sg_conv_fwd_v4_skip_try(pb, sk, st, true) ? 1 : 0;
  const int prof = sg_prof_begin(st, 2.0 * (double)I * (double)J * ((double)K + (double)sk->C2), 0);
  const bool ok = sg_conv_fwd_v4_skip_try(pb, sk, st, false);
  {
    const double jout = (d->epi_flags & SG_EPI_POOL) ? (double)J / 4.0 : (double)J;
    const double x2 = (double)d->N * (sk->x2_up ? (d->Ho / 2) * (d->Wo / 2) : d->Ho * d->Wo) * sk->C2;
    sg_prof_tag(prof, SG_ENG_CONV_V4_SKIP, 2.0 * ((double)d->N * d->Hs * d->Ws * d->C + x2 + (double)I * (K + sk->C2) + jout * I));
  }
  sg_prof_end(st, prof);
  return ok ? 1 : 0;
}
extern "C" int sg_conv2d_fwd_skip_stat_rows(const sg_conv_skip_desc* d) {
  if (!d) return 0;
  const long long J = (long long)d->main.N * d->main.Ho * d->main.Wo;
  return (int)((J + 255) / 256);
}
extern "C" int sg_conv2d_fwd_skip_ok(const sg_conv_skip_desc* d) {
  if (!d || !d->main.x || !d->main.w || !d->main.out || !d->x2 || !d->w2) return 0;
  return conv_fwd_skip(d, nullptr, true);
}
extern "C" int sg_conv2d_fwd_skip(const sg_conv_skip_desc* d, sg_stream_t stream) {
  SG_CHECK(d && d->main.x && d->main.w && d->main.out && d->x2 && d->w2, "sg_conv2d_fwd_skip: null pointer");
  SG_CHECK(conv_fwd_skip(d, (hipStream_t)stream, false) == 1, "sg_conv2d_fwd_skip: problem not eligible for the fused kernel (ask sg_conv2d_fwd_skip_ok first)");
  SG_LAUNCH_CHECK();
  return 0;
}

extern "C" int sg_conv2d_fwd(const sg_conv_fwd_desc* d, sg_stream_t stream) {
  SG_CHECK(d && d->x && d->w && d->out, "sg_conv2d_fwd: null pointer");
  SG_CHECK(d->N > 0 && d->C > 0 && d->Cout > 0 && d->R > 0 && d->S > 0 && d->stride > 0, "sg_conv2d_fwd: bad shape");
  SG_CHECK(!(d->epi_flags & SG_EPI_ATOMIC), "sg_conv2d_fwd: atomic epilogue not supported");
  if (d->dtype == SG_DTYPE_F32) return conv_fwd_t<float>(d, (hipStream_t)stream);
  if (d->dtype == SG_DTYPE_BF16) return conv_fwd_t<bf16_t>(d, (hipStream_t)stream);
  sg_set_error("sg_conv2d_fwd: bad dtype");
  return -1;
}
```

pytorch-studiogan_amd/csrc/conv_common.h:

```cpp
#pragma once
#include <stdlib.h>
#include "gemm_core.h"
#include "../../include/sgamd.h"

static inline int ilog2_exact(int v) {
  if (v <= 0 || (v & (v - 1))) return -1;
  int s = 0;
  while ((1 << s) < v) s++;
  return s;
}
static inline bool aligned16(const void* p) { return (((uintptr_t)p) & 15) == 0; }

template <typename T>
static void fill_geom(PixGeom<T>& g, const void* x, int N, int Hs, int Ws, int C, int ldx, int Ho, int Wo, int R, int S,
                      int stride, int pad_h, int pad_w, int flags) {
  g.x = (const T*)x; g.N = N; g.Hs = Hs; g.Ws = Ws;
  const int up = (flags & SG_PIX_UPSAMPLE) ? 2 : 1;
  g.Hin = Hs * up; g.Win = Ws * up; g.C = C; g.ldx = ldx; g.Ho = Ho; g.Wo = Wo;
  g.R = R; g.S = S; g.stride = stride; g.pad_h = pad_h; g.pad_w = pad_w; g.flags = flags;
  g.vec_ok = (C % ET<T>::VEC == 0) && (ldx % ET<T>::VEC == 0) && aligned16(x);
  g.wshift = ilog2_exact(Wo); g.hshift = ilog2_exact(Ho);
}

static inline char env_mode(const char* name) { const char* m = getenv(name); return m ? m[0] : 0; }

static inline long long bf16_extent(long long npix, int ld, int C) { return ((npix - 1) * ld + C) * 2; }

template <typename D> static inline bool is_3x3_s1_p1(const D* d) { return d->R == 3 && d->S == 3 && d->stride == 1 && d->pad_h == 1 && d->pad_w == 1; }

static inline int cout_blocks(int Cout) { return Cout % 96 == 0 ? 3 : Cout % 64 == 0 ? 2 : 0; }

static const int kCoutTiles[3] = {192, 128, 96};
static inline int cout_tile_search(int I, int tj, int& best_tiles) {
  int best = 0;
  best_tiles = 0;
  for (int c = 0; c < 3; c++) {
    if (I % kCoutTiles[c]) continue;
    const int tiles = (I / kCoutTiles[c]) * tj;
    if (tiles >= 512) { best = kCoutTiles[c]; best_tiles = tiles; break; }
    if (tiles > best_tiles) { best = kCoutTiles[c]; best_tiles = tiles; }
  }
  return best;
}

template <typename T, class LP, class LQ, int SPLIT, class EPI = Epilogue<T>>
static void conv_fwd_tiles(const LP& lp, const LQ& lq, const EPI& e, int I, int J, int K, hipStream_t st) {
  if (I <= 32) sg_launch_gemm<T, LP, LQ, 32, 256, 1, 4, true, SPLIT, EPI>(lp, lq, e, I, J, K, 1, 1, st);
  else if (I % 128 != 0 && (I % 96 == 0 || (I < 128 && I > 64))) sg_launch_gemm<T, LP, LQ, 96, 256, 1, 4, true, SPLIT, EPI>(lp, lq, e, I, J, K, 1, 1, st);
  else sg_launch_gemm<T, LP, LQ, 128, 128, 2, 2, true, SPLIT, EPI>(lp, lq, e, I, J, K, 1, 1, st);
}

template <typename T, typename D> static Epilogue<T> make_epilogue(const D* d, int I, int J) {
  Epilogue<T> e;
  e.out = d->out; e.out_bstride = 0; e.ldo = d->ldo; e.bias = d->bias;
  e.res = d->res; e.res_bstride = 0; e.ldr = d->ldr; e.beta = d->beta;
  e.mask = (const T*)d->mask; e.mask_bstride = 0; e.ldm = d->ldm; e.split_stride = 0;
  e.alpha = d->alpha; e.alpha_ptr = d->alpha_ptr; e.flags = d->epi_flags; e.I = I; e.J = J;
  return e;
}
static inline bool epi_bf16_rows_ok(const Epilogue<bf16_t>& e) {
  if ((e.flags & (SG_EPI_ATOMIC | SG_EPI_OUT_F32)) || (e.ldo & 7) || !aligned16(e.out)) return false;
  if (e.mask && ((e.ldm & 7) || !aligned16(e.mask))) return false;
  if (e.res && ((e.flags & SG_EPI_RES_F32) || (e.ldr & 7) || !aligned16(e.res))) return false;
  return true;
}

struct ConvFwdProblem {
  const sg_conv_fwd_desc* d;
  Epilogue<bf16_t> e;
  int I, J, K, pflags;
  bool up, quad;
  int wshift, hshift;
  long long xbytes, wbytes;
  bool out_is_in_times_up() const { return d->Ho == d->Hs * (up ? 2 : 1) && d->Wo == d->Ws * (up ? 2 : 1); }
};
static inline ConvFwdProblem conv_fwd_problem(const sg_conv_fwd_desc* d, const Epilogue<bf16_t>& e, int I, int J, int K, int pflags) {
  ConvFwdProblem pb;
  pb.d = d; pb.e = e; pb.I = I; pb.J = J; pb.K = K; pb.pflags = pflags;
  pb.up = (pflags & SG_PIX_UPSAMPLE) != 0; pb.quad = (pflags & SG_PIX_QUAD) != 0;
  pb.wshift = ilog2_exact(d->Wo); pb.hshift = ilog2_exact(d->Ho);
  pb.xbytes = bf16_extent((long long)d->N * d->Hs * d->Ws, d->ldx, d->C); pb.wbytes = (long long)I * K * 2;
  return pb;
}

bool sg_conv_fwd_sk_try(const ConvFwdProblem& pb, hipStream_t st);
bool sg_conv_fwd_rs_try(const ConvFwdProblem& pb, hipStream_t st);
bool sg_conv_fwd_v4_try(const ConvFwdProblem& pb, hipStream_t st);
bool sg_conv_fwd_v3_try(const ConvFwdProblem& pb, hipStream_t st);
bool sg_conv_fwd_v4_skip_try(const ConvFwdProblem& pb, const sg_conv_skip_desc* sk, hipStream_t st, bool dry);
```

pytorch-studiogan_amd/csrc/conv_sk.h:

```cpp
#pragma once
#include "conv_v2.h"

struct ConvSkParams {
  const bf16_t* x; const bf16_t* w;
  int C, ldx, Hs, Ws;
  int Ho, Wo, wshift, hshift;
  int mode3;
  int flags;
  int I, J, K;
  unsigned xbytes;
  unsigned obytes, sbytes;
  int nrb;
};

template <int TI, int NP, int TJ, int KS, int NW, bool POOL>
__global__ __launch_bounds__(64 * NW) void sg_conv_sk_kernel(ConvSkParams p, Epilogue<bf16_t> epi) {
  constexpr int BI = TI * NP * 32;
  constexpr int NCH = 2 * KS;
  constexpr int WP = KS * 32 + 16;
  constexpr int CP = TI * 64 + 16;
  constexpr int ROWS = 32 * TJ;
  constexpr int CPR = TI * 4;
  extern __shared__ __attribute__((aligned(16))) char smem[];
  char* const wsm = smem;
  float* const sbias = (float*)(smem + BI * WP);
  const int tid = threadIdx.x, lane = tid & 63;
  const int wave = __builtin_amdgcn_readfirstlane(tid >> 6);
  char* const stg = smem + BI * WP + BI * 4 + wave * (ROWS * CP);
  const int i0 = blockIdx.y * BI;

  for (int idx = tid; idx < BI * NCH; idx += 64 * NW) {
    const int row = idx / NCH, c = idx - row * NCH;
    u32x4 v = {0u, 0u, 0u, 0u};
    if (i0 + row < p.I && c * 8 < p.K) v = *(const u32x4*)(p.w + (long long)(i0 + row) * p.K + c * 8);
    *(u32x4*)(wsm + row * WP + c * 16) = v;
  }
  for (int i = tid; i < BI; i += 64 * NW) sbias[i] = (epi.bias && i0 + i < epi.I) ? epi.bias[i0 + i] : 0.f;
  __syncthreads();

  const auto rsx = __builtin_amdgcn_make_buffer_rsrc((void*)p.x, 0, (int)p.xbytes, 0x00020000);
  const auto rso = __builtin_amdgcn_make_buffer_rsrc(epi.out, 0, (int)p.obytes, 0x00020000);
  const auto rss = __builtin_amdgcn_make_buffer_rsrc((void*)(epi.mask ? (const void*)epi.mask : epi.res), 0, (int)p.sbytes, 0x00020000);
  constexpr int NIT = ((POOL ? ROWS / 4 : ROWS) * CPR + 63) / 64;
  const int frow = lane & 31, fhi = lane >> 5;
  const unsigned ldx2 = 2u * (unsigned)p.ldx;
  const bool up = (p.flags & SG_PIX_UPSAMPLE) != 0, quad = (p.flags & SG_PIX_QUAD) != 0;
  typedef short s16x2_t __attribute__((ext_vector_type(2)));
  const short fl = (p.flags & SG_PIX_RELU) ? (short)0 : (short)-32768;
  const s16x2_t floor2 = {fl, fl};

  int ctr[KS], cts[KS];
  unsigned cdelta[KS];
  bool cok[KS];
#pragma unroll
  for (int ks = 0; ks < KS; ks++) {
    const int c = 2 * ks + fhi;
    const int tr3 = (c * 11) >> 5;
    const int ts3 = c - 3 * tr3;
    ctr[ks] = p.mode3 ? tr3 : 1;
    cts[ks] = p.mode3 ? ts3 : 1;
    cdelta[ks] = p.mode3 ? (unsigned)((tr3 - 1) * p.Ws + (ts3 - 1)) * ldx2 : (unsigned)c * 16u;
    cok[ks] = p.mode3 ? (c < 9) : (c * 8 < p.C);
  }

  auto fetch = [&](int rb, u32x4 (&q)[TJ][KS]) {
#pragma unroll
    for (int b = 0; b < TJ; b++) {
      const int row = rb * ROWS + b * 32 + frow;
      int n, ho, wo;
      if (quad) {
        const int qd = row >> 2, dy = (row >> 1) & 1, dx = row & 1;
        const int wq = qd & ((p.Wo >> 1) - 1);
        const int t = qd >> (p.wshift - 1);
        const int hq = t & ((p.Ho >> 1) - 1);
        n = t >> (p.hshift - 1);
        ho = 2 * hq + dy; wo = 2 * wq + dx;
      } else {
        wo = row & (p.Wo - 1); const int t = row >> p.wshift; ho = t & (p.Ho - 1); n = t >> p.hshift;
      }
      const bool rok = row < p.J;
      const int hs = up ? (ho >> 1) : ho, ws = up ? (wo >> 1) : wo;
      const unsigned pixoff = ((unsigned)(n * p.Hs + hs) * (unsigned)p.Ws + (unsigned)ws) * ldx2;
      if constexpr (KS == 6) {
#pragma unroll
        for (int ks = 0; ks < KS; ks++) {
          const bool ok = rok && cok[ks] && (unsigned)(ho + ctr[ks] - 1) < (unsigned)p.Ho && (unsigned)(wo + cts[ks] - 1) < (unsigned)p.Wo;
          unsigned off = pixoff + cdelta[ks];
          off = ok ? off : 0x80000000u;
          q[b][ks] = __builtin_bit_cast(u32x4, __builtin_amdgcn_raw_buffer_load_b128(rsx, (int)off, 0, 0));
        }
      } else {
        const unsigned base = rok ? pixoff + (unsigned)fhi * 16u : 0x80000000u;
#pragma unroll
        for (int ks = 0; ks < KS; ks++) {
          const unsigned off = ((2 * ks + fhi) * 8 < p.C) ? base + (unsigned)ks * 32u : 0x80000000u;
          q[b][ks] = __builtin_bit_cast(u32x4, __builtin_amdgcn_raw_buffer_load_b128(rsx, (int)off, 0, 0));
        }
      }
    }
  };

  float al = epi.alpha;
  if (epi.alpha_ptr) al *= *epi.alpha_ptr;
  constexpr bool pool = POOL;
  const bool relu_out = (epi.flags & SG_EPI_RELU) != 0;
  const bool pre_mask = epi.mask != nullptr, pre_res = epi.res != nullptr;
  const int Jout = pool ? (epi.J >> 2) : epi.J;
  const int ncr = ((epi.I - i0 < BI ? epi.I - i0 : BI) + 7) >> 3;
  constexpr int rows_out_full = ROWS;

  auto compute_store = [&](int rb, u32x4 (&q)[TJ][KS]) {
#pragma unroll
    for (int b = 0; b < TJ; b++)
#pragma unroll
      for (int ks = 0; ks < KS; ks++)
#pragma unroll
        for (int e = 0; e < 4; e++) {
          const uint32_t xw = q[b][ks][e];
          s16x2_t t = __builtin_bit_cast(s16x2_t, xw);
          t = __builtin_elementwise_max(t, floor2);
          q[b][ks][e] = __builtin_bit_cast(uint32_t, t);
        }
    const int r0 = rb * ROWS;
    constexpr int rows_out = pool ? rows_out_full / 4 : rows_out_full;
    const int jbase = pool ? (r0 >> 2) : r0;
#pragma unroll
    for (int ps = 0; ps < NP; ps++) {
      f32x16 acc[TI][TJ];
#pragma unroll
      for (int a = 0; a < TI; a++)
#pragma unroll
        for (int b = 0; b < TJ; b++)
#pragma unroll
          for (int r = 0; r < 16; r++) acc[a][b][r] = 0.f;
#pragma unroll
      for (int ks = 0; ks < KS; ks++) {
        bf16x8_t pf[TI], qf[TJ];
#pragma unroll
        for (int a = 0; a < TI; a++) {
          const u32x4 v = *(const u32x4*)(wsm + ((ps * TI + a) * 32 + frow) * WP + (2 * ks + fhi) * 16);
          pf[a] = __builtin_bit_cast(bf16x8_t, v);
        }
#pragma unroll
        for (int b = 0; b < TJ; b++) qf[b] = __builtin_bit_cast(bf16x8_t, q[b][ks]);
#pragma unroll
        for (int a = 0; a < TI; a++)
#pragma unroll
          for (int b = 0; b < TJ; b++)
            acc[a][b] = __builtin_amdgcn_mfma_f32_32x32x16_bf16(pf[a], qf[b], acc[a][b], 0, 0, 0);
      }
      const int ic0 = ps * TI * 32;
      const int ncp = ncr - ps * CPR;
      asm volatile("s_waitcnt lgkmcnt(0)" ::: "memory");
      if (pre_mask || pre_res) {
        const int ld = pre_mask ? epi.ldm : epi.ldr;
        u32x4 pre[NIT];
#pragma unroll
        for (int it = 0; it < NIT; it++) {
          const int idx = lane + 64 * it;
          const int r = idx / CPR, c = idx - r * CPR;
          const int jg = jbase + r;
          const bool ok = idx < rows_out * CPR && jg < Jout && c < ncp;
          const unsigned off = ok ? ((unsigned)jg * (unsigned)ld + (unsigned)(i0 + ic0 + c * 8)) * 2u : 0x80000000u;
          pre[it] = __builtin_bit_cast(u32x4, __builtin_amdgcn_raw_buffer_load_b128(rss, (int)off, 0, 0));
        }
#pragma unroll
        for (int it = 0; it < NIT; it++) {
          const int idx = lane + 64 * it;
          const int r = idx / CPR, c = idx - r * CPR;
          if (idx < rows_out * CPR) *(u32x4*)(stg + r * CP + c * 16) = pre[it];
        }
        asm volatile("s_waitcnt lgkmcnt(0)" ::: "memory");
      }
#pragma unroll
      for (int ta = 0; ta < TI; ta++)
#pragma unroll
        for (int tb = 0; tb < TJ; tb++) {
          const int jl = tb * 32 + (lane & 31);
#pragma unroll
          for (int g4 = 0; g4 < 4; g4++) {
            const int il = ta * 32 + 8 * g4 + 4 * (lane >> 5);
            float v[4] = {acc[ta][tb][4 * g4 + 0], acc[ta][tb][4 * g4 + 1], acc[ta][tb][4 * g4 + 2], acc[ta][tb][4 * g4 + 3]};
            if (pool) {
#pragma unroll
              for (int e = 0; e < 4; e++) v[e] = quad_sum(v[e]);
            }
            const int jo = pool ? (jl >> 2) : jl;
            const bool act = (!pool || (lane & 3) == 0) && (jbase + jo < Jout);
            if (act) {
              char* loc = stg + jo * CP + il * 2;
#pragma unroll
              for (int e = 0; e < 4; e++) v[e] *= al;
              {
                const f32x4 bv = *(const f32x4*)(sbias + ic0 + il);
#pragma unroll
                for (int e = 0; e < 4; e++) v[e] += bv[e];
              }
              if (pre_mask) {
                const u32x2 m = *(const u32x2*)loc;
#pragma unroll
                for (int e = 0; e < 4; e++) { const bf16_t h = (bf16_t)((m[e >> 1] >> (16 * (e & 1))) & 0xffffu); if (!(bf2f(h) > 0.f)) v[e] = 0.f; }
              }
              if (pre_res) {
                const u32x2 r = *(const u32x2*)loc;
#pragma unroll
                for (int e = 0; e < 4; e++) { const bf16_t h = (bf16_t)((r[e >> 1] >> (16 * (e & 1))) & 0xffffu); v[e] += epi.beta * bf2f(h); }
              }
              if (relu_out) {
#pragma unroll
                for (int e = 0; e < 4; e++) v[e] = fmaxf(v[e], 0.f);
              }
              u32x2 t;
              t[0] = pack2bf(v[0], v[1]);
              t[1] = pack2bf(v[2], v[3]);
              *(u32x2*)loc = t;
            }
          }
        }
      asm volatile("s_waitcnt lgkmcnt(0)" ::: "memory");
#pragma unroll
      for (int it = 0; it < NIT; it++) {
        const int idx = lane + 64 * it;
        const int r = idx / CPR, c = idx - r * CPR;
        const int jg = jbase + r;
        const bool ok = idx < rows_out * CPR && jg < Jout && c < ncp;
        const unsigned off = ok ? ((unsigned)jg * (unsigned)epi.ldo + (unsigned)(i0 + ic0 + c * 8)) * 2u : 0x80000000u;
        const int rr = idx < rows_out * CPR ? r : 0;
        const u32x4 v = *(const u32x4*)(stg + rr * CP + c * 16);
        __builtin_amdgcn_raw_buffer_store_b128(v, rso, (int)off, 0, 0);
      }
    }
  };

  const int stride = gridDim.x * NW;
  int rb = blockIdx.x * NW + wave;
  u32x4 qa[TJ][KS], qb[TJ][KS];
  if (rb >= p.nrb) return;
  fetch(rb, qa);
#pragma unroll
  for (int it = 0; it < NP * NIT; it++) {
    const u32x4 z = {0u, 0u, 0u, 0u};
    __builtin_amdgcn_raw_buffer_store_b128(z, rso, (int)(0x80000000u + 16u * it), 0, 0);
  }
  while (true) {
    fetch(rb + stride, qb);
    compute_store(rb, qa);
    rb += stride;
    if (rb >= p.nrb) break;
    fetch(rb + stride, qa);
    compute_store(rb, qb);
    rb += stride;
    if (rb >= p.nrb) break;
  }
}

template <int TI, int NP, int TJ, int KS, bool POOL>
static inline int sg_launch_conv_sk_tp(ConvSkParams p, const Epilogue<bf16_t>& e, hipStream_t st) {
  constexpr int BI = TI * NP * 32, WP = KS * 32 + 16, CP = TI * 64 + 16, ROWS = 32 * TJ;
  constexpr int lds4 = BI * WP + BI * 4 + 4 * ROWS * CP;
  constexpr int NW = (2 * lds4 <= 160 * 1024) ? 4 : 8;
  constexpr int lds = BI * WP + BI * 4 + NW * ROWS * CP;
  static_assert(lds <= 160 * 1024, "LDS");
  static bool attr_done = false;
  if (!attr_done) {
    if (hipFuncSetAttribute((const void*)sg_conv_sk_kernel<TI, NP, TJ, KS, NW, POOL>, hipFuncAttributeMaxDynamicSharedMemorySize, lds) != hipSuccess) return -1;
    attr_done = true;
  }
  p.nrb = (p.J + ROWS - 1) / ROWS;
  const int tilesI = (p.I + BI - 1) / BI;
  int gx = (p.nrb + NW - 1) / NW;
  const int cap = (256 * (8 / NW) + tilesI - 1) / tilesI;
  if (gx > cap) gx = cap;
  hipLaunchKernelGGL((sg_conv_sk_kernel<TI, NP, TJ, KS, NW, POOL>), dim3(gx, tilesI), dim3(64 * NW), lds, st, p, e);
  return 0;
}
template <int TI, int NP, int TJ, int KS>
static inline int sg_launch_conv_sk_t(const ConvSkParams& p, const Epilogue<bf16_t>& e, hipStream_t st) {
  return (e.flags & SG_EPI_POOL) ? sg_launch_conv_sk_tp<TI, NP, TJ, KS, true>(p, e, st) : sg_launch_conv_sk_tp<TI, NP, TJ, KS, false>(p, e, st);
}

static inline int sg_launch_conv_sk(const ConvSkParams& p, const Epilogue<bf16_t>& e, hipStream_t st) {
  const int ti = p.I <= 32 ? 1 : p.I <= 64 ? 2 : p.I <= 96 ? 3 : p.I <= 128 ? 4 : 6;
  const int ks = p.K <= 16 ? 1 : p.K <= 48 ? 3 : p.K <= 96 ? 6 : 12;
#define SG_SK_CASE(T_, TI_, NP_, KS_, TJ_) if (ti == T_ && ks == KS_) return sg_launch_conv_sk_t<TI_, NP_, TJ_, KS_>(p, e, st);
  SG_SK_CASE(1, 1, 1, 1, 2) SG_SK_CASE(1, 1, 1, 3, 2) SG_SK_CASE(1, 1, 1, 6, 2) SG_SK_CASE(1, 1, 1, 12, 1)
  SG_SK_CASE(2, 2, 1, 1, 2) SG_SK_CASE(2, 2, 1, 3, 2) SG_SK_CASE(2, 2, 1, 6, 1) SG_SK_CASE(2, 2, 1, 12, 1)
  SG_SK_CASE(3, 3, 1, 1, 1) SG_SK_CASE(3, 3, 1, 3, 1) SG_SK_CASE(3, 3, 1, 6, 1) SG_SK_CASE(3, 3, 1, 12, 1)
  SG_SK_CASE(4, 2, 2, 1, 2) SG_SK_CASE(4, 2, 2, 3, 2) SG_SK_CASE(4, 2, 2, 6, 1) SG_SK_CASE(4, 2, 2, 12, 1)
  SG_SK_CASE(6, 3, 2, 1, 1) SG_SK_CASE(6, 3, 2, 3, 1) SG_SK_CASE(6, 3, 2, 6, 1) SG_SK_CASE(6, 2, 3, 12, 1)
#undef SG_SK_CASE
  return -1;
}
```

pytorch-studiogan_amd/csrc/conv_sk.hip:

```cpp
#include "conv_common.h"
#include "conv_sk.h"

bool sg_conv_fwd_sk_try(const ConvFwdProblem& pb, hipStream_t st) {
  const sg_conv_fwd_desc* d = pb.d;
  const Epilogue<bf16_t>& e = pb.e;
  const int I = pb.I, J = pb.J;
  const char mode = env_mode("SG_CONV_SK");
  if (mode == '0') return false;
  const bool force = mode == 'f';
  if (d->stride != 1 || (pb.pflags & SG_PIX_TRANSPOSED)) return false;
  const bool one = d->R == 1 && d->S == 1 && d->pad_h == 0 && d->pad_w == 0 && d->C <= 192;
  const bool stem = is_3x3_s1_p1(d) && d->C == 8 && !pb.up;
  if (!one && !stem) return false;
  if (d->C % 8 || d->ldx % 8 || I % 8 || I > 384 || !aligned16(d->x) || !aligned16(d->w)) return false;
  if (!pb.out_is_in_times_up()) return false;
  if (pb.wshift < 1 || pb.hshift < 1) return false;
  if (pb.xbytes >= (1ll << 31) || J >= (1 << 30)) return false;
  if (!epi_bf16_rows_ok(e) || (e.mask && e.res)) return false;
  if (J < 16384 && !force) return false;
  const long long jout = (e.flags & SG_EPI_POOL) ? (J >> 2) : J;
  const long long obytes = bf16_extent(jout, e.ldo, I);
  const long long sbytes = e.mask ? bf16_extent(jout, e.ldm, I) : (e.res ? bf16_extent(jout, e.ldr, I) : 16);
  if (obytes >= (1ll << 31) || sbytes >= (1ll << 31)) return false;
  ConvSkParams p;
  p.obytes = (unsigned)obytes; p.sbytes = (unsigned)sbytes;
  p.x = (const bf16_t*)d->x; p.w = (const bf16_t*)d->w;
  p.C = d->C; p.ldx = d->ldx; p.Hs = d->Hs; p.Ws = d->Ws;
  p.Ho = d->Ho; p.Wo = d->Wo; p.wshift = pb.wshift; p.hshift = pb.hshift;
  p.mode3 = stem ? 1 : 0; p.flags = pb.pflags;
  p.I = I; p.J = J; p.K = pb.K; p.xbytes = (unsigned)pb.xbytes; p.nrb = 0;
  return sg_launch_conv_sk(p, e, st) == 0;
}
```

pytorch-studiogan_amd/csrc/conv_wgrad.hip:

```cpp
#include <type_traits>
#include "conv_common.h"
#include "wgrad_v2.h"
#include "wgrad_sk.h"
#include "wgrad_v3.h"

static bool wgrad_bf16_ok(const sg_conv_wgrad_desc* d) {
  if (d->dtype != SG_DTYPE_BF16 || d->stride != 1 || d->no_tr) return false;
  if ((d->x_flags | d->g_flags) & SG_PIX_TRANSPOSED) return false;
  return (long long)d->N * d->xHs * d->xWs * d->ldx * 2 < (1ll << 31) && (long long)d->N * d->gHs * d->gWs * d->ldg * 2 < (1ll << 31);
}
static inline unsigned wgrad_xbytes(const sg_conv_wgrad_desc* d) { return (unsigned)bf16_extent((long long)d->N * d->xHs * d->xWs, d->ldx, d->C); }
static inline unsigned wgrad_gbytes(const sg_conv_wgrad_desc* d) { return (unsigned)bf16_extent((long long)d->N * d->gHs * d->gWs, d->ldg, d->Cout); }

struct SkPlan { bool ok, taps; int NI, NJ, swap, nw; long long n; };
static SkPlan wgrad_sk_plan(const sg_conv_wgrad_desc* d) {
  SkPlan s; s.ok = false; s.taps = false; s.NI = s.NJ = s.swap = s.nw = 0; s.n = 0;
  if (env_mode("SG_WGRAD_SK") == '0' || !wgrad_bf16_ok(d)) return s;
  if (ilog2_exact(d->Wo) < 0 || ilog2_exact(d->Ho) < 0) return s;
  if (d->C % 8 || d->ldx % 8 || d->Cout % 8 || d->ldg % 8 || !aligned16(d->x) || !aligned16(d->dy)) return s;
  const long long K = (long long)d->N * d->Ho * d->Wo;
  if (K % 32 || K / 32 >= (1ll << 30)) return s;
  const bool xup = d->x_flags & SG_PIX_UPSAMPLE, gup = d->g_flags & SG_PIX_UPSAMPLE, xrelu = d->x_flags & SG_PIX_RELU;
  if (d->R == 1 && d->S == 1 && d->pad_h == 0 && d->pad_w == 0) {
    if (d->C > 192 || d->Cout > 96) return s;
    const int ni = (d->C + 31) / 32, nj = (d->Cout + 31) / 32;
    if (ni == 4 || ni == 5) return s;
    s.ok = true; s.NI = ni; s.NJ = nj; s.n = (long long)d->C * d->Cout;
  } else if (is_3x3_s1_p1(d) && !xup && !gup && !xrelu && d->Wo >= 32) {
    if (d->C == 8 && d->Cout <= 96) { s.ok = true; s.taps = true; s.NI = 3; s.NJ = (d->Cout + 31) / 32; s.n = 72ll * d->Cout; }
    else if (d->Cout == 8 && d->C <= 96) { s.ok = true; s.taps = true; s.swap = 1; s.NI = 3; s.NJ = (d->C + 31) / 32; s.n = 72ll * d->C; }
  }
  if (s.ok) s.nw = sg_wgrad_sk_waves((int)(K / 32));
  return s;
}
static int wgrad_sk_launch(const sg_conv_wgrad_desc* d, const SkPlan& s, hipStream_t st) {
  WgradSkParams p;
  const long long K = (long long)d->N * d->Ho * d->Wo;
  const unsigned xbytes = wgrad_xbytes(d), gbytes = wgrad_gbytes(d);
  p.H = d->Ho; p.W = d->Wo; p.wshift = ilog2_exact(d->Wo); p.hshift = ilog2_exact(d->Ho);
  p.nchunk = (int)(K / 32);
  p.arelu = (d->x_flags & SG_PIX_RELU) ? 1 : 0;
  p.work = (float*)d->work; p.n = s.n;
  p.alpha = d->alpha; p.alpha_ptr = d->alpha_ptr;
  const int xup = (d->x_flags & SG_PIX_UPSAMPLE) ? 1 : 0, gup = (d->g_flags & SG_PIX_UPSAMPLE) ? 1 : 0;
  if (!s.swap) {
    p.a = (const bf16_t*)d->x; p.lda = d->ldx; p.CA = d->C; p.upA = xup; p.HsA = d->xHs; p.WsA = d->xWs; p.abytes = xbytes;
    p.b = (const bf16_t*)d->dy; p.ldb = d->ldg; p.CB = d->Cout; p.upB = gup; p.HsB = d->gHs; p.WsB = d->gWs; p.bbytes = gbytes;
    p.sgn = 1; p.swap = 0; p.I = s.taps ? 72 : d->C; p.J = d->Cout;
  } else {
    p.a = (const bf16_t*)d->dy; p.lda = d->ldg; p.CA = 8; p.upA = 0; p.HsA = d->gHs; p.WsA = d->gWs; p.abytes = gbytes;
    p.b = (const bf16_t*)d->x; p.ldb = d->ldx; p.CB = d->C; p.upB = 0; p.HsB = d->xHs; p.WsB = d->xWs; p.bbytes = xbytes;
    p.sgn = -1; p.swap = 1; p.I = 72; p.J = d->C;
  }
  return sg_launch_wgrad_sk(p, s.taps, s.NI, s.NJ, st);
}

struct V3Plan { bool ok; int NB, nci, nco, splits, nchunk; long long n, stride; };
static V3Plan wgrad_v3_plan(const sg_conv_wgrad_desc* d) {
  V3Plan s; s.ok = false; s.NB = s.nci = s.nco = s.splits = s.nchunk = 0; s.n = 0; s.stride = 0;
  const char mode = env_mode("SG_WGRAD_V3");
  if (mode == '0') return s;
  const bool force = mode == 'f';
  if (!wgrad_bf16_ok(d) || !is_3x3_s1_p1(d)) return s;
  if (d->Wo != 4 && d->Wo != 8 && d->Wo != 16 && d->Wo != 32 && d->Wo % 64) return s;
  if (d->Wo == 4) {
    if (d->Ho != 4 || d->N % 4 || ((d->x_flags | d->g_flags) & SG_PIX_UPSAMPLE)) return s;
  } else if (d->Wo < 64 && d->Ho % (64 / d->Wo)) return s;
  if (d->C % 32 || d->ldx % 8 || d->ldg % 8 || !aligned16(d->x) || !aligned16(d->dy)) return s;
  s.NB = cout_blocks(d->Cout);
  if (!s.NB) return s;
  const long long K = (long long)d->N * d->Ho * d->Wo;
  if (K % 64 || (!force && K < (d->Wo == 4 ? 4096 : 16384)) || K >= (1ll << 31)) return s;
  s.nci = d->C / 32; s.nco = d->Cout / (32 * s.NB); s.nchunk = (int)(K / 64);
  s.n = 9ll * d->C * d->Cout;
  s.stride = s.n + (d->dbias ? d->Cout : 0);
  const int tiles = s.nci * s.nco;
  int sp = d->splits > 0 ? d->splits : (768 >= tiles ? 768 / tiles : 1);
  const int maxs = s.nchunk / 8 > 0 ? s.nchunk / 8 : 1;
  if (sp > maxs) sp = maxs;
  if (sp > 512) sp = 512;
  s.splits = sp;
  s.ok = true;
  return s;
}
static int wgrad_v3_launch(const sg_conv_wgrad_desc* d, const V3Plan& s, hipStream_t st) {
  WgradV3Params p;
  p.x = (const bf16_t*)d->x; p.dy = (const bf16_t*)d->dy;
  p.xHs = d->xHs; p.xWs = d->xWs; p.ldx = d->ldx; p.x_up = (d->x_flags & SG_PIX_UPSAMPLE) ? 1 : 0; p.x_relu = (d->x_flags & SG_PIX_RELU) ? 1 : 0;
  p.gHs = d->gHs; p.gWs = d->gWs; p.ldg = d->ldg; p.g_up = (d->g_flags & SG_PIX_UPSAMPLE) ? 1 : 0;
  p.N = d->N; p.H = d->Ho; p.W = d->Wo; p.C = d->C; p.Cout = d->Cout;
  p.nci = s.nci; p.nco = s.nco; p.nchunk = s.nchunk; p.splits = s.splits;
  p.xbytes = wgrad_xbytes(d); p.gbytes = wgrad_gbytes(d);
  p.out = d->work; p.split_stride = s.stride;
  p.bias_off = d->dbias ? s.n : -1; p.bias_scale = p.g_up ? 0.25f : 1.f;
  p.alpha = d->alpha; p.alpha_ptr = d->alpha_ptr;
  return sg_launch_wgrad_v3(p, s.NB, env_mode("SG_WGRAD_V3_LEAN") != '0', st);
}

static bool wgrad_v2_ok(const sg_conv_wgrad_desc* d) {
  const char mode = env_mode("SG_CONV_V2");
  if (mode == '0' || !wgrad_bf16_ok(d)) return false;
  if (ilog2_exact(d->Ho) < 0 || ilog2_exact(d->Wo) < 0) return false;
  if (d->C % 8 || d->ldx % 8 || d->Cout % 8 || d->ldg % 8 || !aligned16(d->x) || !aligned16(d->dy)) return false;
  const long long K = (long long)d->N * d->Ho * d->Wo;
  const int I = d->R * d->S * d->C;
  if (mode != 'f' && (I < 64 || d->Cout < 64 || K < 4096)) return false;
  return true;
}
static int wgrad_v2_launch(const sg_conv_wgrad_desc* d, const Epilogue<bf16_t>& e, int I, int J, int K, int splits, hipStream_t st) {
  WgradV2Params p;
  p.x = (const bf16_t*)d->x; p.dy = (const bf16_t*)d->dy;
  p.xHs = d->xHs; p.xWs = d->xWs; p.C = d->C; p.ldx = d->ldx;
  p.x_up = (d->x_flags & SG_PIX_UPSAMPLE) ? 1 : 0; p.x_relu = (d->x_flags & SG_PIX_RELU) ? 1 : 0;
  p.Hin = d->xHs * (p.x_up ? 2 : 1); p.Win = d->xWs * (p.x_up ? 2 : 1);
  p.gHs = d->gHs; p.gWs = d->gWs; p.Cout = d->Cout; p.ldg = d->ldg; p.g_up = (d->g_flags & SG_PIX_UPSAMPLE) ? 1 : 0;
  p.Ho = d->Ho; p.Wo = d->Wo; p.wshift = ilog2_exact(d->Wo); p.hshift = ilog2_exact(d->Ho);
  p.R = d->R; p.S = d->S; p.pad_h = d->pad_h; p.pad_w = d->pad_w;
  p.I = I; p.J = J; p.K = K;
  p.xbytes = wgrad_xbytes(d); p.gbytes = wgrad_gbytes(d);
  int klen = K;
  if (splits > 1) { klen = (K + splits - 1) / splits; klen = ((klen + 63) / 64) * 64; splits = (K + klen - 1) / klen; }
  p.klen = klen;
  return sg_launch_wgrad_v2(p, e, splits, st);
}

static void wgrad_plan(int I, int J, int K, int bk, int want_splits, int& BI, int& BJ, int& splits, bool v2 = false) {
  if (v2) { BI = 256; BJ = sg_wgrad_v2_bj(I, J, K); bk = 64; }
  else if (I <= 32) { BI = 32; BJ = 256; }
  else if (J <= 32) { BI = 256; BJ = 32; }
  else if (J % 128 != 0 && (J % 96 == 0 || (J < 128 && J > 64))) { BI = 256; BJ = 96; }
  else { BI = 128; BJ = 128; }
  const int tiles = ((I + BI - 1) / BI) * ((J + BJ - 1) / BJ);
  splits = want_splits;
  if (splits <= 0) {
    splits = (768 + tiles - 1) / tiles;
    int maxs = K / (bk * 16); if (maxs < 1) maxs = 1;
    if (splits > maxs) splits = maxs;
    if (splits > 512) splits = 512;
  }
  if (splits > 1) {
    int klen = (K + splits - 1) / splits; klen = ((klen + bk - 1) / bk) * bk;
    splits = (K + klen - 1) / klen;
  }
}

enum WgradEngine { WG_SK, WG_V3, WG_V2, WG_GEMM };
struct WgradChoice {
  WgradEngine engine;
  int splits; long long n, stride, work_floats;
  bool fuses_bias;
  SkPlan sk; V3Plan v3; int BI, BJ;
};
static WgradChoice wgrad_choose(const sg_conv_wgrad_desc* d, bool launching) {
  WgradChoice c = {};
  const auto have = [&](long long floats) { return !launching || (d->work && d->work_floats >= floats); };
  c.sk = wgrad_sk_plan(d);
  if (c.sk.ok && have((long long)c.sk.nw * c.sk.n)) {
    c.engine = WG_SK; c.splits = c.sk.nw; c.n = c.stride = c.sk.n; c.work_floats = (long long)c.sk.nw * c.sk.n;
    return c;
  }
  c.v3 = wgrad_v3_plan(d);
  if (c.v3.ok && have((long long)c.v3.splits * c.v3.stride)) {
    c.engine = WG_V3; c.splits = c.v3.splits; c.n = c.v3.n; c.stride = c.v3.stride; c.work_floats = (long long)c.v3.splits * c.v3.stride;
    c.fuses_bias = d->dbias != nullptr;
    return c;
  }
  const int I = d->R * d->S * d->C, J = d->Cout, K = (int)((long long)d->N * d->Ho * d->Wo);
  const bool v2 = wgrad_v2_ok(d);
  wgrad_plan(I, J, K, d->dtype == SG_DTYPE_BF16 ? ET<bf16_t>::BK : ET<float>::BK, d->splits, c.BI, c.BJ, c.splits, v2);
  c.engine = v2 ? WG_V2 : WG_GEMM; c.n = c.stride = (long long)I * J; c.work_floats = c.splits > 1 ? c.splits * c.n : 0;
  return c;
}

extern "C" int sg_conv2d_wgrad_fuses_bias(const sg_conv_wgrad_desc* d) {
  return (d && wgrad_choose(d, false).fuses_bias) ? 1 : 0;
}

extern "C" int sg_conv2d_wgrad_plan(const sg_conv_wgrad_desc* d, int* splits, long long* work_floats) {
  SG_CHECK(d && splits && work_floats, "sg_conv2d_wgrad_plan: null");
  const WgradChoice c = wgrad_choose(d, false);
  *splits = c.splits;
  *work_floats = c.work_floats;
  return 0;
}

__global__ __launch_bounds__(256) void k_splitk_reduce(const float* partial, float* out, int splits, long long n, long long stride = 0, float* out2 = nullptr, long long n2 = 0) {
  __shared__ float sm[4][64];
  if (stride == 0) stride = n;
  const long long nt = n + n2;
  const int li = threadIdx.x & 63, q = threadIdx.x >> 6;
  for (long long i0 = blockIdx.x * 64ll; i0 < nt; i0 += (long long)gridDim.x * 64) {
    const long long i = i0 + li;
    float a0 = 0.f, a1 = 0.f, a2 = 0.f, a3 = 0.f;
    if (i < nt) {
      int s = q;
      for (; s + 12 < splits; s += 16) {
        a0 += partial[(long long)s * stride + i];
        a1 += partial[(long long)(s + 4) * stride + i];
        a2 += partial[(long long)(s + 8) * stride + i];
        a3 += partial[(long long)(s + 12) * stride + i];
      }
      for (; s < splits; s += 4) a0 += partial[(long long)s * stride + i];
    }
    sm[q][li] = (a0 + a1) + (a2 + a3);
    __syncthreads();
    if (q == 0 && i < nt) {
      const float t = (sm[0][li] + sm[1][li]) + (sm[2][li] + sm[3][li]);
      if (i < n) out[i] += t; else out2[i - n] += t;
    }
    __syncthreads();
  }
}

__global__ __launch_bounds__(256) void k_splitk_reduce_v4(const float* partial, float* out, int splits, long long n, long long stride, float* out2, long long n2) {
  __shared__ f32x4 sm[4][64];
  const long long nt4 = (n + n2) >> 2, n4 = n >> 2;
  const int li = threadIdx.x & 63, q = threadIdx.x >> 6;
  for (long long i0 = blockIdx.x * 64ll; i0 < nt4; i0 += (long long)gridDim.x * 64) {
    const long long i = i0 + li;
    f32x4 a[8];
#pragma unroll
    for (int k = 0; k < 8; k++) a[k] = (f32x4){0.f, 0.f, 0.f, 0.f};
    if (i < nt4) {
      const float* src = partial + 4 * i;
      int s = q;
      for (; s + 28 < splits; s += 32) {
        f32x4 v[8];
#pragma unroll
        for (int k = 0; k < 8; k++) v[k] = *(const f32x4*)(src + (long long)(s + 4 * k) * stride);
#pragma unroll
        for (int k = 0; k < 8; k++) a[k] += v[k];
      }
      for (; s < splits; s += 4) a[0] += *(const f32x4*)(src + (long long)s * stride);
    }
    sm[q][li] = ((a[0] + a[1]) + (a[2] + a[3])) + ((a[4] + a[5]) + (a[6] + a[7]));
    __syncthreads();
    if (q == 0 && i < nt4) {
      const f32x4 t = (sm[0][li] + sm[1][li]) + (sm[2][li] + sm[3][li]);
      float* dst = i < n4 ? out + 4 * i : out2 + 4 * (i - n4);
      f32x4 o = *(f32x4*)dst;
      *(f32x4*)dst = o + t;
    }
    __syncthreads();
  }
}
static void splitk_reduce_launch(const float* partial, float* out, int splits, long long n, long long stride, float* out2, long long n2, hipStream_t st) {
  const bool v4 = (n % 4 == 0) && (n2 % 4 == 0) && (stride % 4 == 0) && ((((uintptr_t)partial | (uintptr_t)out | (uintptr_t)out2) & 15) == 0);
  if (v4) {
    long long blocks = ((n + n2) / 4 + 63) / 64; if (blocks > 8192) blocks = 8192; if (blocks < 1) blocks = 1;
    hipLaunchKernelGGL(k_splitk_reduce_v4, dim3((int)blocks), dim3(256), 0, st, partial, out, splits, n, stride, out2, n2);
  } else {
    long long blocks = (n + n2 + 63) / 64; if (blocks > 8192) blocks = 8192;
    hipLaunchKernelGGL(k_splitk_reduce, dim3((int)blocks), dim3(256), 0, st, partial, out, splits, n, stride, out2, n2);
  }
}

template <typename T, class LM, bool TR, int SPLIT>
static void conv_wgrad_tiles(const LM& lp, const LM& lq, const Epilogue<T>& e, int I, int J, int K, int BI, int BJ, int splits, hipStream_t st) {
  if (BI == 32) sg_launch_gemm<T, LM, LM, 32, 256, 1, 4, TR, SPLIT>(lp, lq, e, I, J, K, splits, 1, st);
  else if (BJ == 32) sg_launch_gemm<T, LM, LM, 256, 32, 4, 1, TR, SPLIT>(lp, lq, e, I, J, K, splits, 1, st);
  else if (BJ == 96) sg_launch_gemm<T, LM, LM, 256, 96, 4, 1, TR, SPLIT>(lp, lq, e, I, J, K, splits, 1, st);
  else sg_launch_gemm<T, LM, LM, 128, 128, 2, 2, TR, SPLIT>(lp, lq, e, I, J, K, splits, 1, st);
}

template <typename T, bool TR, bool FAST>
static void conv_wgrad_launch(const sg_conv_wgrad_desc* d, const Epilogue<T>& e, int I, int J, int K, int BI, int BJ, int splits, hipStream_t st) {
  typedef ConvPixMC<T, FAST> LM;
  LM lp;
  fill_geom<T>(lp.g, d->x, d->N, d->xHs, d->xWs, d->C, d->ldx, d->Ho, d->Wo, d->R, d->S, d->stride, d->pad_h, d->pad_w,
               d->x_flags & ~SG_PIX_QUAD);
  lp.rows = I; lp.K = K;
  LM lq;
  fill_geom<T>(lq.g, d->dy, d->N, d->gHs, d->gWs, d->Cout, d->ldg, d->Ho, d->Wo, 1, 1, 1, 0, 0, d->g_flags & ~SG_PIX_QUAD);
  lq.rows = J; lq.K = K;
  if constexpr (sizeof(T) == 4 && FAST) {
    const int mode = g_sg_f32_mode;
    if (mode == 3) { sg_f32_split_count(3); return conv_wgrad_tiles<T, LM, TR, 3>(lp, lq, e, I, J, K, BI, BJ, splits, st); }
    if (mode == 6) { sg_f32_split_count(6); return conv_wgrad_tiles<T, LM, TR, 6>(lp, lq, e, I, J, K, BI, BJ, splits, st); }
  }
  conv_wgrad_tiles<T, LM, TR, 0>(lp, lq, e, I, J, K, BI, BJ, splits, st);
}

template <typename T> static double wgrad_alg_bytes(const sg_conv_wgrad_desc* d) {
  return sizeof(T) * ((double)d->N * d->xHs * d->xWs * d->C + (double)d->N * d->gHs * d->gWs * d->Cout) + 8.0 * (double)d->R * d->S * d->C * d->Cout;
}
template <typename T, bool TR> static int conv_wgrad_t(const sg_conv_wgrad_desc* d, hipStream_t st) {
  const int I = d->R * d->S * d->C;
  const int J = d->Cout;
  const long long Kll = (long long)d->N * d->Ho * d->Wo;
  SG_CHECK(Kll < (1ll << 31), "sg_conv2d_wgrad: too many pixels");
  SG_CHECK((long long)d->N * d->xHs * d->xWs * d->ldx < (1ll << 31) && (long long)d->N * d->gHs * d->gWs * d->ldg < (1ll << 31),
           "sg_conv2d_wgrad: tensor too large for 32-bit element offsets");
  const int K = (int)Kll;
  const WgradChoice c = wgrad_choose(d, true);
  const int prof = sg_prof_begin(st, 2.0 * (double)I * (double)J * (double)K, 1);
  int eng = SG_ENG_WGRAD_GEMM;
  bool two_stage = true;
  if (c.engine == WG_SK) {
    if (wgrad_sk_launch(d, c.sk, st) != 0) { sg_set_error("sg_conv2d_wgrad: streaming kernel launch failed"); return -2; }
    eng = SG_ENG_WGRAD_SK;
  } else if (c.engine == WG_V3) {
    if (wgrad_v3_launch(d, c.v3, st) != 0) { sg_set_error("sg_conv2d_wgrad: halo kernel launch failed"); return -2; }
    eng = SG_ENG_WGRAD_V3;
  } else {
    two_stage = c.work_floats > 0 && d->work && d->work_floats >= c.work_floats;
    Epilogue<T> e;
    e.out = d->dw; e.out_bstride = 0; e.ldo = I; e.bias = nullptr; e.res = nullptr; e.res_bstride = 0; e.ldr = 0; e.beta = 0.f;
    e.mask = nullptr; e.mask_bstride = 0; e.ldm = 0; e.alpha = d->alpha; e.alpha_ptr = d->alpha_ptr; e.split_stride = 0;
    e.flags = SG_EPI_OUT_F32; e.I = I; e.J = J;
    if (c.splits == 1) { e.res = d->dw; e.ldr = I; e.beta = 1.f; e.flags |= SG_EPI_RES_F32; }
    else if (two_stage) { e.out = d->work; e.split_stride = c.n; }
    else e.flags |= SG_EPI_ATOMIC;
    if constexpr (std::is_same_v<T, bf16_t>) {
      if (c.engine == WG_V2 && wgrad_v2_launch(d, e, I, J, K, c.splits, st) == 0) eng = SG_ENG_WGRAD_V2;
    }
    if (eng == SG_ENG_WGRAD_GEMM) {
      const bool fast = (d->C % ET<T>::VEC == 0) && (d->ldx % ET<T>::VEC == 0) && aligned16(d->x) &&
                        (d->Cout % ET<T>::VEC == 0) && (d->ldg % ET<T>::VEC == 0) && aligned16(d->dy);
      if (fast) conv_wgrad_launch<T, TR, true>(d, e, I, J, K, c.BI, c.BJ, c.splits, st);
      else conv_wgrad_launch<T, TR, false>(d, e, I, J, K, c.BI, c.BJ, c.splits, st);
    }
  }
  if (two_stage) {
    splitk_reduce_launch((const float*)d->work, d->dw, c.splits, c.n, c.stride, c.fuses_bias ? d->dbias : nullptr, c.fuses_bias ? d->Cout : 0, st);
  }
  sg_prof_tag(prof, eng, wgrad_alg_bytes<T>(d));
  sg_prof_end(st, prof);
  SG_LAUNCH_CHECK();
  return 0;
}

extern "C" int sg_conv2d_wgrad(const sg_conv_wgrad_desc* d, sg_stream_t stream) {
  SG_CHECK(d && d->x && d->dy && d->dw, "sg_conv2d_wgrad: null pointer");
  SG_CHECK(d->N > 0 && d->C > 0 && d->Cout > 0 && d->R > 0 && d->S > 0 && d->stride > 0, "sg_conv2d_wgrad: bad shape");
  if (d->dtype == SG_DTYPE_F32) return conv_wgrad_t<float, true>(d, (hipStream_t)stream);
  if (d->dtype == SG_DTYPE_BF16) {
    if (d->no_tr) return conv_wgrad_t<bf16_t, false>(d, (hipStream_t)stream);
    return conv_wgrad_t<bf16_t, true>(d, (hipStream_t)stream);
  }
  sg_set_error("sg_conv2d_wgrad: bad dtype");
  return -1;
}
```

pytorch-studiogan_amd/functional/_base.py:

```python
import os

import torch
import torch.distributed as dist

from .. import _lib as L
from .. import comm as _comm
from ..bank import ensure_grad


def _first_order_only(name):
    if torch.is_grad_enabled():
        raise NotImplementedError(name + ": no differentiable backward (create_graph=True). Second-order passes exist for the discriminator's conv / BN / pooling / "
                                         "self-attention / head path (gradient penalties, R1) and for the ResNet / BigGAN / BigGAN-Deep generators incl. conditional "
                                         "batch norm (latent optimisation); not for third order, nor for the DCGAN generator's transposed convolutions")


def _param_grad_wanted(*params):
    for p in params:
        if p is None or not torch.is_tensor(p) or not p.requires_grad:
            continue
        try:
            if torch._C._will_engine_execute_node(torch.autograd.graph.get_gradient_edge(p).node):
                return True
        except Exception:
            return True
    return False


def _c(t):
    return t if t.is_contiguous() else t.contiguous()


_ZERO_POOL = {}
_ZERO_POOL_BYTES = 8 << 20
_ZERO_POOL_ON = [os.environ.get("SG_ZERO_POOL", "1") != "0"]


def zeros_small(shape, dtype, device):
    if isinstance(shape, int):
        shape = (shape,)
    n = 1
    for d in shape:
        n *= int(d)
    nbytes = n * torch.empty((), dtype=dtype).element_size()
    if not _ZERO_POOL_ON[0] or nbytes == 0 or nbytes > (_ZERO_POOL_BYTES >> 1) or torch.device(device).type != "cuda":
        return torch.zeros(shape, dtype=dtype, device=device)
    key = torch.device(device)
    ent = _ZERO_POOL.get(key)
    step = (nbytes + 255) & ~255
    if ent is None or ent[1] + step > _ZERO_POOL_BYTES:
        ent = _ZERO_POOL[key] = [torch.zeros(_ZERO_POOL_BYTES, dtype=torch.uint8, device=device), 0]
    off = ent[1]
    ent[1] = off + step
    return ent[0][off:off + nbytes].view(dtype).view(shape)


def zeros_like_small(t):
    return zeros_small(tuple(t.shape), t.dtype, t.device)


_SEQ = [0]
_STATS_OFFER = [None]
_BN_FUSED_STATS = [os.environ.get("SG_BN_FUSED_STATS", "1") != "0"]
_CBN_MERGED = [os.environ.get("SG_CBN_MERGED", "1") != "0"]


def _tick():
    _SEQ[0] += 1


def _offer_stats(out, st, rows, C):
    _STATS_OFFER[0] = (_SEQ[0], out.data_ptr(), tuple(out.shape), st, rows, C, out._version)


def _take_stats(x):
    ent, _STATS_OFFER[0] = _STATS_OFFER[0], None
    if ent is None or ent[0] != _SEQ[0] - 1 or ent[1] != x.data_ptr() or ent[2] != tuple(x.shape) or ent[5] != x.shape[3] or ent[6] != x._version:
        return None
    return ent[3], ent[4]


class f32_mode:
    MODES = {"exact": 0, "bf16x3": 3, "bf16x6": 6}

    def __init__(self, mode):
        if mode not in self.MODES:
            raise ValueError(f"f32_mode: {mode!r} (one of {sorted(self.MODES)})")
        self.mode = self.MODES[mode]

    def __enter__(self):
        self.saved = L.lib().sg_get_f32_mode()
        L.call("sg_set_f32_mode", self.mode)
        return self

    def __exit__(self, *exc):
        L.call("sg_set_f32_mode", self.saved)
        return False


def conv2d_raw(x, w_ptr, Cin, Cout, R, S, stride=1, pad_h=0, pad_w=0, pix_flags=0, epi_flags=0, bias=None, res=None, mask=None,
               alpha=1.0, beta=1.0, alpha_ptr=None, out=None, ldx=None, transposed_out_hw=None, out_coff=0, x_coff=0, desc=None):
    N, Hs, Ws = x.shape[0], x.shape[1], x.shape[2]
    ldx = x.shape[3] if ldx is None else ldx
    up = 2 if (pix_flags & L.PIX_UPSAMPLE) else 1
    Hin, Win = Hs * up, Ws * up
    if pix_flags & L.PIX_TRANSPOSED:
        Ho, Wo = transposed_out_hw
    else:
        Ho = (Hin + 2 * pad_h - R) // stride + 1
        Wo = (Win + 2 * pad_w - S) // stride + 1
    pool = bool(epi_flags & L.EPI_POOL)
    Hy, Wy = (Ho // 2, Wo // 2) if pool else (Ho, Wo)
    if out is None:
        odt = torch.float32 if (epi_flags & L.EPI_OUT_F32) else x.dtype
        out = torch.empty((N, Hy, Wy, Cout), dtype=odt, device=x.device)
    d = desc if desc is not None else L.ConvFwdDesc()
    d.dtype = L.dt(x)
    d.N, d.Hs, d.Ws, d.C, d.ldx = N, Hs, Ws, Cin, ldx
    d.Ho, d.Wo, d.Cout = Ho, Wo, Cout
    d.R, d.S, d.stride, d.pad_h, d.pad_w = R, S, stride, pad_h, pad_w
    d.pix_flags, d.epi_flags = pix_flags, epi_flags
    d.alpha, d.beta = alpha, beta
    d.x, d.w = L.ptr(x) + x_coff * x.element_size(), w_ptr
    d.bias = L.ptr(bias)
    d.res = L.ptr(res)
    d.mask = L.ptr(mask)
    d.out = L.ptr(out) + out_coff * out.element_size()
    d.alpha_ptr = L.ptr(alpha_ptr)
    d.ldo = out.shape[-1]
    d.ldr = res.shape[-1] if res is not None else 0
    d.ldm = mask.shape[-1] if mask is not None else 0
    if desc is not None:
        return out
    L.call("sg_conv2d_fwd", d, L.stream())
    return out


def conv2d_skip_raw(x, w_ptr, Cin, Cout, x2, w2_ptr, C2, x2_up=False, pix_flags=0, epi_flags=0, bias=None, bias2=None, alpha=1.0, dry=False, stats=False):
    sk = L.ConvSkipDesc()
    out = conv2d_raw(x, w_ptr, Cin, Cout, 3, 3, 1, 1, 1, pix_flags, epi_flags, bias=bias, alpha=alpha, desc=sk.main)
    sk.x2, sk.w2, sk.bias2 = L.ptr(x2), w2_ptr, L.ptr(bias2)
    sk.C2, sk.ldx2, sk.x2_up = C2, x2.shape[3], 1 if x2_up else 0
    if L.lib().sg_conv2d_fwd_skip_ok(L.C.byref(sk)) != 1:
        return None
    if dry:
        return out
    if stats and not (epi_flags & L.EPI_POOL):
        rows = L.lib().sg_conv2d_fwd_skip_stat_rows(L.C.byref(sk))
        st = torch.empty((rows, Cout, 2), dtype=torch.float32, device=x.device)
        sk.stats = st.data_ptr()
        L.call("sg_conv2d_fwd_skip", sk, L.stream())
        _offer_stats(out, st, rows, Cout)
        return out
    L.call("sg_conv2d_fwd_skip", sk, L.stream())
    return out


def conv2d_wgrad_raw(x, dy, dw_ptr, Cin, Cout, R, S, Ho, Wo, stride=1, pad_h=0, pad_w=0, x_flags=0, g_flags=0, alpha=1.0,
                     alpha_ptr=None, splits=0, no_tr=0, ldg=None, dy_coff=0, dbias=None):
    d = L.ConvWgradDesc()
    d.dtype = L.dt(x)
    d.N = x.shape[0]
    d.xHs, d.xWs, d.C, d.ldx, d.x_flags = x.shape[1], x.shape[2], Cin, x.shape[3], x_flags
    d.gHs, d.gWs, d.Cout, d.ldg, d.g_flags = dy.shape[1], dy.shape[2], Cout, (dy.shape[3] if ldg is None else ldg), g_flags
    d.Ho, d.Wo = Ho, Wo
    d.R, d.S, d.stride, d.pad_h, d.pad_w = R, S, stride, pad_h, pad_w
    d.alpha = alpha
    d.x, d.dy, d.dw = L.ptr(x), L.ptr(dy) + dy_coff * dy.element_size(), dw_ptr
    d.alpha_ptr = L.ptr(alpha_ptr)
    d.splits, d.no_tr = splits, no_tr
    fused = False
    if dbias is not None:
        d.dbias = L.ptr(dbias)
        fused = L.lib().sg_conv2d_wgrad_fuses_bias(L.C.byref(d)) == 1
        if not fused:
            d.dbias = None
    sp, wf = L.C.c_int(0), L.C.c_longlong(0)
    L.call("sg_conv2d_wgrad_plan", d, L.C.byref(sp), L.C.byref(wf))
    work = None
    if wf.value > 0:
        work = torch.empty(wf.value, dtype=torch.float32, device=x.device)
        d.splits, d.work, d.work_floats = sp.value, work.data_ptr(), wf.value
    L.call("sg_conv2d_wgrad", d, L.stream())
    return fused


def quad_pack_raw(src_ptr, dst, mode, M, Cs):
    L.call("sg_quad_pack", L.dt(dst), mode, src_ptr, L.ptr(dst), M, Cs, L.stream())
    return dst


def conv2d_q_raw(x, wq_ptr, form, Cin, Cout, pix_flags=0, epi_flags=0, bias=None, res=None, mask=None, alpha=1.0, beta=1.0, dry=False,
                 x2=None, w2q_ptr=None, bias2=None, stats=False, x2_norelu=False):
    N = x.shape[0]
    if form == L.Q_POOL:
        if x.shape[1] % 2 or x.shape[2] % 2:
            return None
        Hl, Wl = x.shape[1] // 2, x.shape[2] // 2
        oshape = (N, Hl, Wl, Cout)
    else:
        Hl, Wl = x.shape[1], x.shape[2]
        oshape = (N, 2 * Hl, 2 * Wl, Cout)
    if x.dtype != torch.bfloat16:
        return None
    d = L.ConvQDesc()
    d.dtype, d.form = L.dt(x), form
    d.N, d.Hl, d.Wl, d.C, d.ldx, d.Cout = N, Hl, Wl, Cin, x.shape[3], Cout
    d.pix_flags, d.epi_flags, d.alpha, d.beta = pix_flags, epi_flags, alpha, beta
    out = torch.empty(oshape, dtype=x.dtype, device=x.device)
    d.x, d.wq, d.bias, d.res, d.mask, d.out = L.ptr(x), wq_ptr, L.ptr(bias), L.ptr(res), L.ptr(mask), L.ptr(out)
    d.ldo = Cout
    d.ldr = res.shape[-1] if res is not None else 0
    d.ldm = mask.shape[-1] if mask is not None else 0
    if x2 is not None:
        d.x2, d.w2q, d.bias2, d.C2, d.ldx2 = L.ptr(x2), w2q_ptr, L.ptr(bias2), x2.shape[3], x2.shape[3]
        d.x2_norelu = 1 if x2_norelu else 0
    if L.lib().sg_conv2d_q_ok(L.C.byref(d)) != 1:
        return None
    if not dry:
        st = None
        if stats:
            rows = L.lib().sg_conv2d_q_stat_rows(L.C.byref(d))
            st = torch.empty((rows, Cout, 2), dtype=torch.float32, device=x.device)
            d.stats = st.data_ptr()
        L.call("sg_conv2d_q", d, L.stream())
        if st is not None:
            _offer_stats(out, st, rows, Cout)
    return out


def conv2d_q_wgrad_raw(x, dy, dw_ptr, form, Cin, Cout, x_flags=0, alpha=1.0, dbias=None, splits=0):
    if x.dtype != torch.bfloat16:
        return False
    d = L.ConvQWgradDesc()
    d.dtype, d.form = L.dt(x), form
    lo = dy if form == L.Q_POOL else x
    d.N, d.Hl, d.Wl = lo.shape[0], lo.shape[1], lo.shape[2]
    d.C, d.ldx, d.x_flags, d.Cout, d.ldg = Cin, x.shape[3], x_flags, Cout, dy.shape[3]
    d.alpha = alpha
    d.x, d.dy, d.dw, d.dbias = L.ptr(x), L.ptr(dy), dw_ptr, L.ptr(dbias)
    d.splits = splits
    sp, wf = L.C.c_int(0), L.C.c_longlong(0)
    L.call("sg_conv2d_q_wgrad_plan", d, L.C.byref(sp), L.C.byref(wf))
    if sp.value == 0:
        return False
    work = torch.empty(wf.value, dtype=torch.float32, device=x.device)
    d.work, d.work_floats, d.splits = work.data_ptr(), wf.value, sp.value
    L.call("sg_conv2d_q_wgrad", d, L.stream())
    return True


def gemm_raw(dtype, p, p_form, ldp, q, q_form, ldq, out, ldo, I, J, K, batch=1, p_bs=0, q_bs=0, out_bs=0, bias=None, res=None,
             res_bs=0, ldr=0, beta=1.0, alpha=1.0, alpha_ptr=None, epi_flags=0, splits=1, no_tr=0):
    d = L.GemmDesc()
    d.dtype, d.p_form, d.q_form = dtype, p_form, q_form
    d.I, d.J, d.K, d.batch = I, J, K, batch
    d.p = p if isinstance(p, int) else L.ptr(p)
    d.q = q if isinstance(q, int) else L.ptr(q)
    d.out = out if isinstance(out, int) else L.ptr(out)
    d.p_bstride, d.ldp, d.q_bstride, d.ldq, d.out_bstride, d.ldo = p_bs, ldp, q_bs, ldq, out_bs, ldo
    d.bias = bias if (bias is None or isinstance(bias, int)) else L.ptr(bias)
    d.res = res if (res is None or isinstance(res, int)) else L.ptr(res)
    d.res_bstride, d.ldr, d.beta = res_bs, ldr, beta
    d.alpha = alpha
    d.alpha_ptr = L.ptr(alpha_ptr)
    d.epi_flags, d.splits, d.no_tr = epi_flags, splits, no_tr
    L.call("sg_gemm", d, L.stream())


_DGRAD_SPLITK = [os.environ.get("SG_DGRAD_SPLITK", "1") != "0"]


def gemm_dgrad_rows(w_ptr, dy, dx, B, K, O):
    S = 1
    tiles = ((K + 127) // 128) * ((B + 127) // 128)
    if _DGRAD_SPLITK[0] and tiles < 64:
        while S < 32 and tiles * S < 256 and O % (2 * S) == 0 and O // (2 * S) >= 96:
            S *= 2
    if S == 1:
        gemm_raw(L.F32, w_ptr, 1, K, dy, 0, dy.shape[1] if torch.is_tensor(dy) else O, dx, K, K, B, O)
        return dx
    ldq = dy.shape[1]
    ws = torch.empty((S, B, K), dtype=torch.float32, device=dx.device)
    gemm_raw(L.F32, w_ptr, 1, K, dy, 0, ldq, ws, K, K, B, O // S, batch=S, p_bs=(O // S) * K, q_bs=O // S, out_bs=B * K)
    torch.sum(ws, dim=0, out=dx)
    return dx


__all__ = ['L', 'zeros_small', 'zeros_like_small', '_BN_FUSED_STATS', '_CBN_MERGED', '_DGRAD_SPLITK', '_SEQ', '_STATS_OFFER', '_c', '_comm', '_first_order_only', '_offer_stats', '_param_grad_wanted', '_take_stats', '_tick', 'conv2d_q_raw', 'conv2d_q_wgrad_raw', 'conv2d_raw', 'conv2d_skip_raw', 'conv2d_wgrad_raw', 'dist', 'ensure_grad', 'f32_mode', 'gemm_dgrad_rows', 'gemm_raw', 'os', 'quad_pack_raw', 'torch']
```

pytorch-studiogan_amd/functional/attention.py:

```python
from ._base import *
from .layout import ConvertFn
from .conv import ConvCfg, ConvDgradFn, ConvFn, _conv_wgrad

class MaxPool2Fn(torch.autograd.Function):

    @staticmethod
    def forward(ctx, x):
        x = _c(x)
        B, H, W, Cc = x.shape
        y = torch.empty((B, (H // 2) * (W // 2), Cc), dtype=x.dtype, device=x.device)
        idx = torch.empty((B, (H // 2) * (W // 2), Cc), dtype=torch.uint8, device=x.device)
        L.call("sg_maxpool2_fwd", L.dt(x), L.ptr(x), Cc, L.ptr(y), Cc, L.ptr(idx), B, H, W, Cc, L.stream())
        ctx.save_for_backward(idx)
        ctx.dims = (B, H, W, Cc)
        return y

    @staticmethod
    def backward(ctx, dy):
        (idx,) = ctx.saved_tensors
        if torch.is_grad_enabled():
            return MaxPool2BwdFn.apply(dy, idx, ctx.dims)
        return _maxpool2_bwd(dy, idx, ctx.dims)


def _maxpool2_bwd(dy, idx, dims):
    B, H, W, Cc = dims
    dy = _c(dy)
    dx = torch.empty((B, H, W, Cc), dtype=dy.dtype, device=dy.device)
    L.call("sg_maxpool2_bwd", L.dt(dy), L.ptr(dy), Cc, L.ptr(idx), L.ptr(dx), Cc, B, H, W, Cc, L.stream())
    return dx


class MaxPool2BwdFn(torch.autograd.Function):
    @staticmethod
    def forward(ctx, dy, idx, dims):
        ctx.save_for_backward(idx)
        ctx.dims = dims
        return _maxpool2_bwd(dy, idx, dims)

    @staticmethod
    def backward(ctx, ddx):
        (idx,) = ctx.saved_tensors
        B, H, W, Cc = ctx.dims
        ddx = _c(ddx)
        y = torch.empty((B, (H // 2) * (W // 2), Cc), dtype=ddx.dtype, device=ddx.device)
        L.call("sg_maxpool2_gather", L.dt(ddx), L.ptr(ddx), Cc, L.ptr(idx), L.ptr(y), Cc, B, H, W, Cc, L.stream())
        return y, None, None


class BmmFn(torch.autograd.Function):

    @staticmethod
    def forward(ctx, A, Bm, ta, tb):
        A, Bm = _c(A), _c(Bm)
        if A.dtype != torch.float32 or Bm.dtype != torch.float32 or A.dim() != 3 or Bm.dim() != 3 or A.shape[0] != Bm.shape[0]:
            raise RuntimeError("BmmFn: two fp32 [batch, rows, cols] tensors expected")
        nb = A.shape[0]
        M, K = (A.shape[2], A.shape[1]) if ta else (A.shape[1], A.shape[2])
        K2, N = (Bm.shape[2], Bm.shape[1]) if tb else (Bm.shape[1], Bm.shape[2])
        if K != K2:
            raise RuntimeError("BmmFn: inner dimensions differ")
        out = torch.empty((nb, M, N), dtype=torch.float32, device=A.device)
        gemm_raw(L.F32, Bm, 0 if tb else 1, Bm.shape[2], A, 1 if ta else 0, A.shape[2], out, N, N, M, K, batch=nb,
                 p_bs=Bm.shape[1] * Bm.shape[2], q_bs=A.shape[1] * A.shape[2], out_bs=M * N)
        ctx.save_for_backward(A, Bm)
        ctx.t = (ta, tb)
        return out

    @staticmethod
    def backward(ctx, dC):
        A, Bm = ctx.saved_tensors
        ta, tb = ctx.t
        dA = dB = None
        if ctx.needs_input_grad[0]:
            dA = BmmFn.apply(Bm, dC, tb, True) if ta else BmmFn.apply(dC, Bm, False, not tb)
        if ctx.needs_input_grad[1]:
            dB = BmmFn.apply(dC, A, True, ta) if tb else BmmFn.apply(A, dC, not ta, False)
        return dA, dB, None, None


class SoftmaxRowsFn(torch.autograd.Function):

    @staticmethod
    def forward(ctx, S):
        S = _c(S)
        P = torch.empty_like(S)
        L.call("sg_softmax_rows", L.F32, L.ptr(S), L.ptr(P), S.numel() // S.shape[-1], S.shape[-1], L.stream())
        ctx.save_for_backward(P)
        return P

    @staticmethod
    def backward(ctx, dP):
        (P,) = ctx.saved_tensors
        return SoftmaxRowsBwdFn.apply(P, dP)


class SoftmaxRowsBwdFn(torch.autograd.Function):
    @staticmethod
    def forward(ctx, P, dP):
        P, dP = _c(P), _c(dP)
        dS = torch.empty_like(P)
        L.call("sg_softmax_rows_bwd", L.F32, L.ptr(P), L.ptr(dP), L.ptr(dS), P.numel() // P.shape[-1], P.shape[-1], L.stream())
        ctx.save_for_backward(P, dP)
        return dS

    @staticmethod
    def backward(ctx, u):
        _first_order_only("SoftmaxRowsBwdFn")
        P, dP = ctx.saved_tensors
        u = _c(u)
        rows, cols = P.numel() // P.shape[-1], P.shape[-1]
        gP = gdP = None
        if ctx.needs_input_grad[0]:
            gP = torch.empty_like(P)
            L.call("sg_softmax_rows_bwd2", L.ptr(P), L.ptr(dP), L.ptr(u), L.ptr(gP), rows, cols, L.stream())
        if ctx.needs_input_grad[1]:
            gdP = torch.empty_like(P)
            L.call("sg_softmax_rows_bwd", L.F32, L.ptr(P), L.ptr(u), L.ptr(gdP), rows, cols, L.stream())
        return gP, gdP


class ScalePtrFn(torch.autograd.Function):

    @staticmethod
    def forward(ctx, x, sigma):
        x = _c(x)
        y = torch.empty_like(x)
        L.call("sg_scale_by_ptr", L.dt(x), L.ptr(x), L.ptr(sigma), L.ptr(y), x.numel(), L.stream())
        ctx.save_for_backward(x, sigma)
        ctx.sigma_param = sigma
        return y

    @staticmethod
    def backward(ctx, dy):
        x, sigma = ctx.saved_tensors
        dx = None
        if torch.is_grad_enabled():
            if _param_grad_wanted(ctx.sigma_param):
                raise NotImplementedError("create_graph=True is supported for input gradients only (WGAN-GP / R1 path)")
            return (ScalePtrFn.apply(dy, sigma) if ctx.needs_input_grad[0] else None), None
        dy = _c(dy)
        if ctx.needs_input_grad[1]:
            g = ensure_grad(ctx.sigma_param)
            L.call("sg_dot", L.dt(dy), L.ptr(dy), L.ptr(x), dy.numel(), L.ptr(g), 1.0, None, L.stream())
        if ctx.needs_input_grad[0]:
            dx = torch.empty_like(dy)
            L.call("sg_scale_by_ptr", L.dt(dy), L.ptr(dy), L.ptr(sigma), L.ptr(dx), dy.numel(), L.stream())
        return dx, None


class AttnCoreFn:

    @staticmethod
    def apply(theta, phi_full, g_full):
        return AttnPooledFn.apply(theta, MaxPool2Fn.apply(phi_full), MaxPool2Fn.apply(g_full))


def _attn_reference_graph(theta, phi, g, dims):
    B, H, W, Dp, Cg = dims
    T = theta.dtype
    th = ConvertFn.apply(theta, torch.float32).reshape(B, H * W, Dp)
    ph, gg = ConvertFn.apply(phi, torch.float32), ConvertFn.apply(g, torch.float32)
    P = SoftmaxRowsFn.apply(BmmFn.apply(th, ph, False, True))
    o = BmmFn.apply(P, gg, False, False).reshape(B, H, W, Cg)
    return ConvertFn.apply(o, T)


class AttnPooledFn(torch.autograd.Function):

    @staticmethod
    def forward(ctx, theta, phi, g):
        theta, phi, g = _c(theta), _c(phi), _c(g)
        B, H, W, Dp = theta.shape
        Cg = g.shape[2]
        HW, HW4 = H * W, (H // 2) * (W // 2)
        dev, T = theta.device, theta.dtype
        sd = L.dt(T)
        need_grad = any(ctx.needs_input_grad)
        fused = (T == torch.bfloat16 and L.lib().sg_attn_fwd_flash_ok(B, HW, HW4, Dp, Cg) == 1
                 and (not need_grad or L.lib().sg_attn_bwd_fused_ok(B, HW, HW4, Dp, Cg) == 1))
        P = lse = o32 = None
        o = torch.empty((B, H, W, Cg), dtype=T, device=dev)
        if fused:
            lse = torch.empty((B, HW), dtype=torch.float32, device=dev)
            o32 = torch.empty((B, HW, Cg), dtype=torch.float32, device=dev) if need_grad else None
            L.call("sg_attn_fwd_fused", L.ptr(theta), L.ptr(phi), L.ptr(g), L.ptr(lse), L.ptr(o), L.ptr(o32), B, HW, HW4, Dp, Cg, L.stream())
        else:
            S = torch.empty((B, HW, HW4), dtype=torch.float32, device=dev)
            gemm_raw(sd, phi, 0, Dp, theta, 0, Dp, S, HW4, HW4, HW, Dp, batch=B, p_bs=HW4 * Dp, q_bs=HW * Dp, out_bs=HW * HW4, epi_flags=L.EPI_OUT_F32)
            P = torch.empty((B, HW, HW4), dtype=T, device=dev)
            L.call("sg_softmax_rows", sd, L.ptr(S), L.ptr(P), B * HW, HW4, L.stream())
            del S
            gemm_raw(sd, g, 1, Cg, P, 0, HW4, o, Cg, Cg, HW, HW4, batch=B, p_bs=HW4 * Cg, q_bs=HW * HW4, out_bs=HW * Cg)
        ctx.save_for_backward(theta, phi, g, P, lse, o32)
        ctx.dims = (B, H, W, Dp, Cg)
        return o

    @staticmethod
    def backward(ctx, do):
        theta, phi, g, P, lse, o32 = ctx.saved_tensors
        B, H, W, Dp, Cg = ctx.dims
        if torch.is_grad_enabled():
            with torch.enable_grad():
                ins = [t for t, need in zip((theta, phi, g), ctx.needs_input_grad) if need]
                grads = list(torch.autograd.grad(_attn_reference_graph(theta, phi, g, ctx.dims), ins, do, create_graph=True)) if ins else []
            return tuple(grads.pop(0) if need else None for need in ctx.needs_input_grad)
        HW, HW4 = H * W, (H // 2) * (W // 2)
        do = _c(do)
        dev, T = do.device, do.dtype
        sd = L.dt(T)
        dtheta = torch.empty((B, H, W, Dp), dtype=T, device=dev)
        dphi = torch.empty((B, HW4, Dp), dtype=T, device=dev)
        dg = torch.empty((B, HW4, Cg), dtype=T, device=dev)
        if P is None:
            delta = torch.empty((B, HW), dtype=torch.float32, device=dev)
            L.call("sg_attn_bwd_fused", L.ptr(theta), L.ptr(phi), L.ptr(g), L.ptr(do), L.ptr(o32), L.ptr(lse), L.ptr(delta), L.ptr(dtheta), L.ptr(dphi),
                   L.ptr(dg), B, HW, HW4, Dp, Cg, L.stream())
            return dtheta, dphi, dg
        gemm_raw(sd, do, 1, Cg, P, 1, HW4, dg, Cg, Cg, HW4, HW, batch=B, p_bs=HW * Cg, q_bs=HW * HW4, out_bs=HW4 * Cg)
        dP = torch.empty((B, HW, HW4), dtype=torch.float32, device=dev)
        gemm_raw(sd, g, 0, Cg, do, 0, Cg, dP, HW4, HW4, HW, Cg, batch=B, p_bs=HW4 * Cg, q_bs=HW * Cg, out_bs=HW * HW4, epi_flags=L.EPI_OUT_F32)
        dS = torch.empty((B, HW, HW4), dtype=T, device=dev)
        L.call("sg_softmax_rows_bwd", sd, L.ptr(P), L.ptr(dP), L.ptr(dS), B * HW, HW4, L.stream())
        del dP
        gemm_raw(sd, phi, 1, Dp, dS, 0, HW4, dtheta, Dp, Dp, HW, HW4, batch=B, p_bs=HW4 * Dp, q_bs=HW * HW4, out_bs=HW * Dp)
        gemm_raw(sd, theta, 1, Dp, dS, 1, HW4, dphi, Dp, Dp, HW4, HW, batch=B, p_bs=HW * Dp, q_bs=HW * HW4, out_bs=HW4 * Dp)
        return dtheta, dphi, dg


def attn_proj_on():
    return os.environ.get("SG_ATTN_PROJ", "1") != "0"


def attn_proj_ok(x, rts):
    rt_t, rt_p, rt_g = rts
    if x.dtype != torch.bfloat16 or x.dim() != 4 or rt_t.rows_pad != rt_p.rows_pad or any(r.RS != 1 or r.trans or r.cin_pad != x.shape[3] for r in rts):
        return False
    B, H, W, Cc = x.shape
    return L.lib().sg_attn_proj_ok(B, H, W, Cc, Cc, rt_t.rows_pad, rt_g.rows_pad) == 1


class AttnProjFn(torch.autograd.Function):

    @staticmethod
    def forward(ctx, x, w_theta, w_phi, w_g, rts, slot, link=None):
        x = _c(x)
        rt_t, rt_p, rt_g = rts
        bank = rt_t.bank()
        B, H, W, Cc = x.shape
        Dp, Cg = rt_t.rows_pad, rt_g.rows_pad
        ctx.link = link
        if link is not None and link.chain:
            link.pending += 1
        for _ in rts:
            _tick()
        HW4 = (H // 2) * (W // 2)
        theta = torch.empty((B, H, W, Dp), dtype=x.dtype, device=x.device)
        phi = torch.empty((B, HW4, Dp), dtype=x.dtype, device=x.device)
        g = torch.empty((B, HW4, Cg), dtype=x.dtype, device=x.device)
        iphi = torch.empty((B, HW4, Dp), dtype=torch.uint8, device=x.device)
        ig = torch.empty((B, HW4, Cg), dtype=torch.uint8, device=x.device)
        L.call("sg_attn_proj_fwd", L.ptr(x), Cc, bank.w_fwd(slot, rt_t), bank.w_fwd(slot, rt_p), bank.w_fwd(slot, rt_g), L.ptr(theta), L.ptr(phi), L.ptr(g),
               L.ptr(iphi), L.ptr(ig), B, H, W, Cc, Dp, Cg, 0, L.stream())
        ctx.save_for_backward(x, iphi, ig)
        ctx.rts, ctx.slot = rts, slot
        ctx.weights = (w_theta, w_phi, w_g)
        return theta, phi, g

    @staticmethod
    def backward(ctx, dtheta, dphi, dg):
        x, iphi, ig = ctx.saved_tensors
        rts, slot = ctx.rts, ctx.slot
        B, H, W, Cc = x.shape
        cfg = ConvCfg(1, 1)
        if torch.is_grad_enabled():
            if not ctx.needs_input_grad[0]:
                return (None,) * 7
            with torch.enable_grad():
                outs = (ConvFn.apply(x, ctx.weights[0], None, None, rts[0], slot, cfg, None),
                        MaxPool2Fn.apply(ConvFn.apply(x, ctx.weights[1], None, None, rts[1], slot, cfg, None)),
                        MaxPool2Fn.apply(ConvFn.apply(x, ctx.weights[2], None, None, rts[2], slot, cfg, None)))
                (dx,) = torch.autograd.grad(outs, [x], [dtheta, dphi, dg], create_graph=True)
            return (dx,) + (None,) * 6
        bank = rts[0].bank()
        Dp, Cg = rts[0].rows_pad, rts[2].rows_pad
        dtheta, dphi, dg = _c(dtheta), _c(dphi), _c(dg)
        dx = None
        skip_dx = ctx.link.take() if ctx.link is not None else None
        if ctx.needs_input_grad[0]:
            dx = torch.empty_like(x)
            L.call("sg_attn_proj_bwd_data", L.ptr(dtheta), L.ptr(dphi), L.ptr(dg), L.ptr(iphi), L.ptr(ig), bank.w_dgrad(slot, rts[0]), bank.w_dgrad(slot, rts[1]),
                   bank.w_dgrad(slot, rts[2]), L.ptr(skip_dx), L.ptr(dx), B, H, W, Cc, Dp, Cg, L.stream())
        elif skip_dx is not None:
            raise RuntimeError("GradLink: a residual gradient was handed over but the attention block's input needs no gradient")
        if ctx.link is not None and ctx.link.chain:
            ctx.link.pending -= 1
        for k, (dy, idx) in enumerate(((dtheta, None), (dphi, iphi), (dg, ig))):
            if ctx.needs_input_grad[1 + k]:
                full = dy if idx is None else _maxpool2_bwd(dy, idx, (B, H, W, dy.shape[-1]))
                _conv_wgrad(x, full, rts[k], slot, cfg)
        return (dx,) + (None,) * 6


class AttnOutFn(torch.autograd.Function):

    @staticmethod
    def forward(ctx, x, o, weight, sigma, rt, slot, link=None):
        bank = rt.bank()
        x, o = _c(x), _c(o)
        ctx.link = link
        y = conv2d_raw(o, bank.w_fwd(slot, rt), rt.Cin, rt.rows, 1, 1, res=x, alpha_ptr=sigma)
        ctx.save_for_backward(o, sigma)
        ctx.rt, ctx.slot = rt, slot
        ctx.sigma_param = sigma
        ctx.weight = weight
        return y

    @staticmethod
    def backward(ctx, dy):
        o, sigma = ctx.saved_tensors
        rt, slot = ctx.rt, ctx.slot
        if torch.is_grad_enabled():
            if _param_grad_wanted(ctx.weight, ctx.sigma_param):
                raise NotImplementedError("create_graph=True is supported for input gradients only (WGAN-GP / R1 path)")
            do = ScalePtrFn.apply(ConvDgradFn.apply(dy, o, ctx.weight, rt, slot, ConvCfg(1, 1)), ctx.sigma_param) if ctx.needs_input_grad[1] else None
            return (dy if ctx.needs_input_grad[0] else None), do, None, None, None, None, None
        bank = rt.bank()
        dy = _c(dy)
        N, H, W, Cc = dy.shape
        do = None
        if ctx.needs_input_grad[3]:
            t = conv2d_raw(o, bank.w_fwd(slot, rt), rt.Cin, rt.rows, 1, 1)
            g = ensure_grad(ctx.sigma_param)
            L.call("sg_dot", L.dt(dy), L.ptr(dy), L.ptr(t), dy.numel(), L.ptr(g), 1.0, None, L.stream())
        if ctx.needs_input_grad[1]:
            do = conv2d_raw(dy, bank.w_dgrad(slot, rt), rt.rows, rt.Cin, 1, 1, alpha_ptr=sigma)
        if ctx.needs_input_grad[2]:
            conv2d_wgrad_raw(o, dy, bank.dwt(slot, rt), rt.Cin, rt.rows, 1, 1, H, W, alpha_ptr=sigma)
        dx = dy
        if ctx.link is not None and ctx.link.pending > 0 and ctx.needs_input_grad[0]:
            ctx.link.dx, dx = dy, None
        return dx, do, None, None, None, None, None


__all__ = ['AttnCoreFn', 'AttnOutFn', 'AttnPooledFn', 'AttnProjFn', 'attn_proj_ok', 'attn_proj_on', 'BmmFn', 'MaxPool2BwdFn', 'MaxPool2Fn', 'ScalePtrFn', 'SoftmaxRowsBwdFn', 'SoftmaxRowsFn', '_attn_reference_graph', '_maxpool2_bwd']
```

pytorch-studiogan_amd/ops.py:

```python
import torch
import torch.nn as nn
from torch.nn import init
import torch.nn.functional as F_

from . import functional as F
from .bank import get_bank

COMPUTE_DTYPE = torch.float32


def to_nhwc(x, dtype, cpad=0):
    if x.dim() != 4:
        raise RuntimeError("expected a 4-D NCHW tensor")
    if x.dtype == torch.uint8:
        return F.u8_to_nhwc(x, dtype, max(cpad, 3))
    if cpad > x.shape[1]:
        return F.NchwToNhwcFn.apply(x.float(), dtype, cpad)
    if x.dtype == dtype and x.is_contiguous(memory_format=torch.channels_last) and not (x.shape[1] > 1 and x.is_contiguous() and x.shape[2] * x.shape[3] > 1):
        return x.permute(0, 2, 3, 1)
    if x.dtype == torch.float32 and x.is_contiguous():
        return F.NchwToNhwcFn.apply(x, dtype)
    y = x.permute(0, 2, 3, 1).contiguous()
    if y.dtype != dtype:
        y = F.ConvertFn.apply(y, dtype)
    return y


def to_nchw(y):
    return y.permute(0, 3, 1, 2)


BLOCK_HOOKS = [False]


def block_boundary(net, bi, act):
    if not BLOCK_HOOKS[0]:
        return act
    tf = net.__dict__.get("_sg_teacher")
    return act if tf is None else tf(bi, act)


def _root_and_bank(m):
    root = m.__dict__.get("_sg_root")
    root = root() if root is not None else None
    if root is None:
        root = m
    dtype = getattr(root, "compute_dtype", None) or getattr(m, "compute_dtype", None) or COMPUTE_DTYPE
    return root, get_bank(root, dtype)


def _standalone_slot(m, x):
    root, bank = _root_and_bank(m)
    if root is m:
        need_graph = torch.is_grad_enabled() and (x.requires_grad or any(p.requires_grad for p in m.parameters()))
        return bank.begin_forward(need_graph)
    return bank.current


class _WeightLayerMixin:
    _sg_weight_layer = True

    def _sg_setup(self, kind, rows, cols, cin, rs, sn, eps=1e-6):
        self._sg_kind, self._sg_rows, self._sg_cols, self._sg_cin, self._sg_rs = kind, rows, cols, cin, rs
        self._sg_sn = bool(sn)
        self._sg_eps = eps
        if sn:
            w = self.weight
            del self._parameters["weight"]
            self.register_parameter("weight_orig", w)
            with torch.no_grad():
                mat = w.reshape(rows, cols)
                u = F_.normalize(w.new_empty(rows).normal_(0, 1), dim=0, eps=eps)
                v = F_.normalize(w.new_empty(cols).normal_(0, 1), dim=0, eps=eps)
            self.register_buffer("weight_u", u)
            self.register_buffer("weight_v", v)

    @property
    def master_weight(self):
        return self.weight_orig if self._sg_sn else self.weight

    def __getattr__(self, name):
        if name == "weight" and "weight_orig" in self.__dict__.get("_parameters", {}):
            return self._parameters["weight_orig"].data
        return super().__getattr__(name)


class Conv2d(_WeightLayerMixin, nn.Conv2d):
    def __init__(self, in_channels, out_channels, kernel_size, stride=1, padding=0, dilation=1, groups=1, bias=True, sn=False,
                 cout_pad=0):
        nn.Conv2d.__init__(self, in_channels, out_channels, kernel_size, stride, padding, dilation, groups, bias)
        if self.dilation != (1, 1) or self.groups != 1:
            raise NotImplementedError("dilation/groups are not on the StudioGAN hot path")
        if self.kernel_size[0] != self.kernel_size[1] and self.stride != (1, 1):
            raise NotImplementedError
        kh, kw = self.kernel_size
        self._sg_rows_pad = cout_pad
        self._sg_dgrad_noflip = self.stride[0] != 1
        self._sg_setup("conv", out_channels, in_channels * kh * kw, in_channels, kh * kw, sn)

    def forward_nhwc(self, x, slot=None, in_relu=False, in_upsample=False, out_pool=False, res=None, link=None, stats=False):
        rt = self._sg_rt
        slot = slot if slot is not None else rt.bank().current
        kh, kw = self.kernel_size
        cfg = F.ConvCfg(kh, kw, self.stride[0], self.padding[0], self.padding[1], in_relu, in_upsample, out_pool, stats and self.training)
        return F.ConvFn.apply(x, self.master_weight, self.bias, res, rt, slot, cfg, link)

    def forward(self, x):
        slot = _standalone_slot(self, x)
        _, bank = _root_and_bank(self)
        y = self.forward_nhwc(to_nhwc(x, bank.dtype, getattr(self, "_sg_cin_pad", 0)), slot)
        if self._sg_rows_pad and self._sg_rows_pad != self.out_channels:
            y = y[..., :self.out_channels]
        return to_nchw(y)


def conv_skip_nhwc(conv_main, conv_skip, h, x, slot=None, in_relu=False, out_pool=False, skip_upsample=False, link=None, stats=False, skip_relu=None):
    rt2, rt0 = conv_main._sg_rt, conv_skip._sg_rt
    slot = slot if slot is not None else rt2.bank().current
    cfg2 = F.ConvCfg(3, 3, 1, 1, 1, in_relu, False, out_pool, stats)
    cfg0 = F.ConvCfg(1, 1, 1, 0, 0, in_relu if skip_relu is None else skip_relu, skip_upsample, out_pool)
    return F.ConvSkipFn.apply(h, x, conv_main.master_weight, conv_main.bias, conv_skip.master_weight, conv_skip.bias, rt2, rt0, slot, cfg2, cfg0, link)


class ConvTranspose2d(_WeightLayerMixin, nn.ConvTranspose2d):

    def __init__(self, in_channels, out_channels, kernel_size, stride=2, padding=0, dilation=1, groups=1, bias=True, sn=False):
        nn.ConvTranspose2d.__init__(self, in_channels, out_channels, kernel_size, stride, padding, 0, groups, bias, dilation)
        if self.dilation != (1, 1) or self.groups != 1 or self.output_padding != (0, 0):
            raise NotImplementedError
        kh, kw = self.kernel_size
        self._sg_trans = True
        self._sg_dgrad_noflip = True
        self._sg_setup("conv", out_channels, in_channels * kh * kw, in_channels, kh * kw, sn)

    def forward_nhwc(self, x, slot=None):
        rt = self._sg_rt
        slot = slot if slot is not None else rt.bank().current
        kh, kw = self.kernel_size
        cfg = F.ConvCfg(kh, kw, self.stride[0], self.padding[0], self.padding[1])
        return F.ConvTransposeFn.apply(x, self.master_weight, self.bias, rt, slot, cfg)

    def forward(self, x, output_size=None):
        slot = _standalone_slot(self, x)
        _, bank = _root_and_bank(self)
        return to_nchw(self.forward_nhwc(to_nhwc(x, bank.dtype), slot))


class Linear(_WeightLayerMixin, nn.Linear):
    def __init__(self, in_features, out_features, bias=True, sn=False):
        nn.Linear.__init__(self, in_features, out_features, bias)
        self._sg_setup("linear", out_features, in_features, in_features, 1, sn)

    def forward_rt(self, x, slot=None, const_bias=None):
        rt = self._sg_rt
        slot = slot if slot is not None else rt.bank().current
        return F.LinearFn.apply(x, self.master_weight, self.bias, rt, slot, const_bias)

    def forward(self, x):
        slot = _standalone_slot(self, x)
        shp = x.shape
        y = self.forward_rt(x.reshape(-1, shp[-1]), slot)
        return y.reshape(*shp[:-1], self.out_features)


class Embedding(_WeightLayerMixin, nn.Embedding):
    def __init__(self, num_embeddings, embedding_dim, sn=False):
        nn.Embedding.__init__(self, num_embeddings, embedding_dim)
        self._sg_setup("embedding", num_embeddings, embedding_dim, embedding_dim, 1, sn)

    def forward(self, idx):
        if not self._sg_sn:
            return F.EmbeddingFn.apply(self.weight, idx.reshape(-1)).reshape(*idx.shape, self.embedding_dim)
        slot = _standalone_slot(self, idx)
        rt = self._sg_rt
        return F.SNEmbeddingFn.apply(self.weight_orig, idx.reshape(-1), rt, slot).reshape(*idx.shape, self.embedding_dim)


_NBT_BULK = [False]


class bump_batches_tracked:

    def __init__(self, root):
        self.on = False
        bns = root.__dict__.get("_sg_bn_list")
        if bns is None:
            bns = [m for m in root.modules() if isinstance(m, BatchNorm2d)]
            root.__dict__["_sg_bn_list"] = bns
        if not bns or _NBT_BULK[0]:
            return
        for m in bns:
            if not (m.training and m.track_running_stats and m.running_mean is not None and m.num_batches_tracked is not None):
                return
        from .bank import get_buffer_arena
        ar = get_buffer_arena(root)
        if ar.inumel != len(bns) or any(b is not m.num_batches_tracked for b, m in zip(ar.ibufs, bns)):
            return
        with torch.no_grad():
            ar.idata.add_(1)
        self.on = True

    def __enter__(self):
        if self.on:
            _NBT_BULK[0] = True
        return self

    def __exit__(self, *a):
        if self.on:
            _NBT_BULK[0] = False


class BatchNorm2d(nn.BatchNorm2d):
    sync_group = None

    def _cfg(self, relu):
        batch_stats = self.training or (self.running_mean is None)
        track = self.training and self.track_running_stats and self.running_mean is not None
        mom = 0.0 if self.momentum is None else self.momentum
        return F.BNCfg(batch_stats, track, self.eps, mom, relu, self.sync_group)

    def forward_nhwc(self, x, gain=None, bias=None, relu=False, link=None, packed=False):
        cfg = self._cfg(relu)
        cfg.packed = packed
        if cfg.track and self.num_batches_tracked is not None and not _NBT_BULK[0]:
            self.num_batches_tracked.add_(1)
        if gain is None and self.affine:
            gain, bias = self.weight, self.bias
        return F.BNFn.apply(x, gain, bias, self.running_mean, self.running_var, cfg, link)

    def forward(self, x):
        dtype = getattr(self, "compute_dtype", None) or (x.dtype if x.dtype in (torch.float32, torch.bfloat16) else COMPUTE_DTYPE)
        return to_nchw(self.forward_nhwc(to_nhwc(x, dtype)))


class ConditionalBatchNorm2d(nn.Module):

    def __init__(self, in_features, out_features, MODULES):
        super().__init__()
        self.in_features = in_features
        self.bn = batchnorm_2d(out_features, eps=1e-4, momentum=0.1, affine=False)
        self.gain = MODULES.g_linear(in_features=in_features, out_features=out_features, bias=False)
        self.bias = MODULES.g_linear(in_features=in_features, out_features=out_features, bias=False)
        self.register_buffer("_ones", torch.ones(out_features), persistent=False)
        self.register_buffer("_ones2", torch.cat([torch.ones(out_features), torch.zeros(out_features)]), persistent=False)

    def forward_nhwc(self, x, y, slot=None, relu=False, link=None):
        pre = slot.__dict__.get("cbn_rows") if slot is not None else None
        if pre:
            gb = pre.pop(id(self), None)
            if gb is not None:
                return self.bn.forward_nhwc(x, gb, None, relu, link, packed=True)
        if F._CBN_MERGED[0] and self.gain.bias is None and self.bias.bias is None:
            rt_g, rt_b = self.gain._sg_rt, self.bias._sg_rt
            slot = slot if slot is not None else rt_g.bank().current
            gb = F.CbnAffineFn.apply(y, self.gain.master_weight, self.bias.master_weight, rt_g, rt_b, slot, self._ones2)
            return self.bn.forward_nhwc(x, gb, None, relu, link, packed=True)
        gain = self.gain.forward_rt(y, slot, const_bias=self._ones)
        bias = self.bias.forward_rt(y, slot)
        return self.bn.forward_nhwc(x, gain, bias, relu, link)

    def forward(self, x, y):
        _, bank = _root_and_bank(self.gain)
        if self.gain.__dict__.get("_sg_root") is None:
            raise RuntimeError("ConditionalBatchNorm2d must live inside a studiogan_amd backbone (its two linears share the network's bank)")
        return to_nchw(self.forward_nhwc(to_nhwc(x, bank.dtype), y))


class SelfAttention(nn.Module):

    def __init__(self, in_channels, is_generator, MODULES):
        super().__init__()
        self.in_channels = in_channels
        conv = MODULES.g_conv2d if is_generator else MODULES.d_conv2d
        c8, c2 = in_channels // 8, in_channels // 2
        pad8 = (c8 + 7) // 8 * 8
        self.conv1x1_theta = conv(in_channels=in_channels, out_channels=c8, kernel_size=1, stride=1, padding=0, bias=False)
        self.conv1x1_phi = conv(in_channels=in_channels, out_channels=c8, kernel_size=1, stride=1, padding=0, bias=False)
        self.conv1x1_g = conv(in_channels=in_channels, out_channels=c2, kernel_size=1, stride=1, padding=0, bias=False)
        self.conv1x1_attn = conv(in_channels=c2, out_channels=in_channels, kernel_size=1, stride=1, padding=0, bias=False)
        for m in (self.conv1x1_theta, self.conv1x1_phi):
            m._sg_rows_pad = pad8
        self.sigma = nn.Parameter(torch.zeros(1), requires_grad=True)

    def forward_nhwc(self, x, slot=None):
        link = F.GradLink(chain=True) if (F._GRAD_LINK[0] and torch.is_grad_enabled() and x.requires_grad) else None
        rt = self.conv1x1_attn._sg_rt
        slot = slot if slot is not None else rt.bank().current
        convs = (self.conv1x1_theta, self.conv1x1_phi, self.conv1x1_g)
        rts = tuple(m._sg_rt for m in convs)
        if F.attn_proj_on() and all(m.bias is None for m in convs) and F.attn_proj_ok(x, rts):
            theta, phi_p, g_p = F.AttnProjFn.apply(x, convs[0].master_weight, convs[1].master_weight, convs[2].master_weight, rts, slot, link)
            o = F.AttnPooledFn.apply(theta, phi_p, g_p)
        else:
            theta = self.conv1x1_theta.forward_nhwc(x, slot, link=link)
            phi = self.conv1x1_phi.forward_nhwc(x, slot, link=link)
            g = self.conv1x1_g.forward_nhwc(x, slot, link=link)
            o = F.AttnCoreFn.apply(theta, phi, g)
        return F.AttnOutFn.apply(x, o, self.conv1x1_attn.master_weight, self.sigma, rt, slot, link)

    def forward(self, x):
        _, bank = _root_and_bank(self.conv1x1_theta)
        return to_nchw(self.forward_nhwc(to_nhwc(x, bank.dtype)))


class LeCamEMA(object):

    def __init__(self, init=7777, decay=0.9, start_iter=0):
        self.G_loss = init
        self.D_loss_real = init
        self.D_loss_fake = init
        self.D_real = init
        self.D_fake = init
        self.decay = decay
        self.start_itr = start_iter

    def update(self, cur, mode, itr):
        decay = 0.0 if itr < self.start_itr else self.decay
        if mode not in ("G_loss", "D_loss_real", "D_loss_fake", "D_real", "D_fake"):
            raise ValueError(mode)
        setattr(self, mode, getattr(self, mode) * decay + cur * (1 - decay))


def conv2d(in_channels, out_channels, kernel_size, stride=1, padding=0, dilation=1, groups=1, bias=True):
    return Conv2d(in_channels, out_channels, kernel_size, stride, padding, dilation, groups, bias, sn=False)


def snconv2d(in_channels, out_channels, kernel_size, stride=1, padding=0, dilation=1, groups=1, bias=True):
    return Conv2d(in_channels, out_channels, kernel_size, stride, padding, dilation, groups, bias, sn=True)


def deconv2d(in_channels, out_channels, kernel_size, stride=2, padding=0, dilation=1, groups=1, bias=True):
    return ConvTranspose2d(in_channels, out_channels, kernel_size, stride, padding, dilation, groups, bias, sn=False)


def sndeconv2d(in_channels, out_channels, kernel_size, stride=2, padding=0, dilation=1, groups=1, bias=True):
    return ConvTranspose2d(in_channels, out_channels, kernel_size, stride, padding, dilation, groups, bias, sn=True)


def linear(in_features, out_features, bias=True):
    return Linear(in_features, out_features, bias, sn=False)


def snlinear(in_features, out_features, bias=True):
    return Linear(in_features, out_features, bias, sn=True)


def embedding(num_embeddings, embedding_dim):
    return Embedding(num_embeddings, embedding_dim, sn=False)


def sn_embedding(num_embeddings, embedding_dim):
    return Embedding(num_embeddings, embedding_dim, sn=True)


def batchnorm_2d(in_features, eps=1e-4, momentum=0.1, affine=True):
    return BatchNorm2d(in_features, eps=eps, momentum=momentum, affine=affine, track_running_stats=True)


def init_weights(modules, initialize):
    for module in modules():
        if isinstance(module, (nn.Conv2d, nn.ConvTranspose2d, nn.Linear)):
            w = module.master_weight if hasattr(module, "master_weight") else module.weight
            if initialize == "ortho":
                init.orthogonal_(w)
            elif initialize == "N02":
                init.normal_(w, 0, 0.02)
            elif initialize in ["glorot", "xavier"]:
                init.xavier_uniform_(w)
            else:
                continue
            if module.bias is not None:
                module.bias.data.fill_(0.)
        elif isinstance(module, nn.Embedding):
            w = module.master_weight if hasattr(module, "master_weight") else module.weight
            if initialize == "ortho":
                init.orthogonal_(w)
            elif initialize == "N02":
                init.normal_(w, 0, 0.02)
            elif initialize in ["glorot", "xavier"]:
                init.xavier_uniform_(w)


def adopt(root, compute_dtype):
    import weakref
    root.compute_dtype = compute_dtype
    ref = weakref.ref(root)
    for m in root.modules():
        if m is not root:
            m.__dict__["_sg_root"] = ref


class Modules:

    def __init__(self, apply_g_sn=False, apply_d_sn=False, g_cond_mtd="W/O", backbone="big_resnet", g_act_fn="ReLU", d_act_fn="ReLU", g_info_injection="N/A"):
        self.g_conv2d = snconv2d if apply_g_sn else conv2d
        self.g_deconv2d = sndeconv2d if apply_g_sn else deconv2d
        self.d_deconv2d = sndeconv2d if apply_d_sn else deconv2d
        self.g_linear = snlinear if apply_g_sn else linear
        self.g_embedding = sn_embedding if apply_g_sn else embedding
        self.d_conv2d = snconv2d if apply_d_sn else conv2d
        self.d_linear = snlinear if apply_d_sn else linear
        self.d_embedding = sn_embedding if apply_d_sn else embedding
        if g_cond_mtd == "cBN" or g_info_injection == "cBN" or backbone == "big_resnet":
            self.g_bn = ConditionalBatchNorm2d
        else:
            self.g_bn = batchnorm_2d
        if not apply_d_sn:
            self.d_bn = batchnorm_2d
        if g_act_fn != "ReLU" or d_act_fn != "ReLU":
            raise NotImplementedError("only ReLU is on the benchmarked hot path")
        self.g_act_fn = nn.ReLU(inplace=True)
        self.d_act_fn = nn.ReLU(inplace=True)
```

Baseline: 2085.

## Fuse attention sigma gradient into wgrad split-K finish and add conv BN-stats epilogue

```diff
diff --git a/include/sgamd.h b/include/sgamd.h
--- a/include/sgamd.h
+++ b/include/sgamd.h
@@ -38,6 +38,8 @@
   int ldo, ldr, ldm;
 } sg_conv_fwd_desc;
 int sg_conv2d_fwd(const sg_conv_fwd_desc* d, sg_stream_t stream);
+int sg_conv2d_fwd_stat_rows(const sg_conv_fwd_desc* d);
+int sg_conv2d_fwd_stats(const sg_conv_fwd_desc* d, float* stats, sg_stream_t stream);
 int sg_set_f32_mode(int mode);
 int sg_get_f32_mode(void);
 long long sg_f32_split_launches(int mode);
@@ -121,6 +123,10 @@
 } sg_conv_wgrad_desc;
 int sg_conv2d_wgrad(const sg_conv_wgrad_desc* d, sg_stream_t stream);
 int sg_conv2d_wgrad_fuses_bias(const sg_conv_wgrad_desc* d);
+#define SG_WGRAD_DSIGMA_SCRATCH 132
+int sg_conv2d_wgrad_dsigma_ok(const sg_conv_wgrad_desc* d);
+int sg_conv2d_wgrad_dsigma_plan(const sg_conv_wgrad_desc* d, int* splits, long long* work_floats);
+int sg_conv2d_wgrad_dsigma(const sg_conv_wgrad_desc* d, const void* w_fwd, float* dsigma, float* scratch, sg_stream_t stream);
 int sg_conv2d_wgrad_plan(const sg_conv_wgrad_desc* d, int* splits, long long* work_floats);
 
 typedef struct {
diff --git a/pytorch-studiogan_amd/_lib.py b/pytorch-studiogan_amd/_lib.py
--- a/pytorch-studiogan_amd/_lib.py
+++ b/pytorch-studiogan_amd/_lib.py
@@ -15,6 +15,7 @@
 PIX_RELU, PIX_UPSAMPLE, PIX_QUAD, PIX_TRANSPOSED = 1, 2, 4, 8
 Q_POOL, Q_UP = 0, 1
 EPI_OUT_F32, EPI_ATOMIC, EPI_POOL, EPI_RELU, EPI_RES_F32 = 1, 2, 4, 8, 16
+WGRAD_DSIGMA_SCRATCH = 132
 
 _vp, _i, _f, _ll = C.c_void_p, C.c_int, C.c_float, C.c_longlong
 
@@ -133,9 +134,14 @@
     "sg_conv2d_q_wgrad": [C.POINTER(ConvQWgradDesc), _vp],
     "sg_prof_collect_ex": [C.POINTER(C.c_double), _i],
     "sg_prof_collect_tags": [C.POINTER(C.c_double), _i],
+    "sg_conv2d_fwd_stat_rows": [C.POINTER(ConvFwdDesc)],
+    "sg_conv2d_fwd_stats": [C.POINTER(ConvFwdDesc), _vp, _vp],
     "sg_conv2d_wgrad": [C.POINTER(ConvWgradDesc), _vp],
     "sg_conv2d_wgrad_plan": [C.POINTER(ConvWgradDesc), C.POINTER(_i), C.POINTER(_ll)],
     "sg_conv2d_wgrad_fuses_bias": [C.POINTER(ConvWgradDesc)],
+    "sg_conv2d_wgrad_dsigma_ok": [C.POINTER(ConvWgradDesc)],
+    "sg_conv2d_wgrad_dsigma_plan": [C.POINTER(ConvWgradDesc), C.POINTER(_i), C.POINTER(_ll)],
+    "sg_conv2d_wgrad_dsigma": [C.POINTER(ConvWgradDesc), _vp, _vp, _vp, _vp],
     "sg_gemm": [C.POINTER(GemmDesc), _vp],
     "sg_nchw_to_nhwc": [_i, _vp, _vp, _i, _i, _i, _i, _i, _vp],
     "sg_nhwc_to_nchw": [_i, _vp, _vp, _i, _i, _i, _i, _i, _i, _vp],
diff --git a/pytorch-studiogan_amd/backbones/big_resnet.py b/pytorch-studiogan_amd/backbones/big_resnet.py
--- a/pytorch-studiogan_amd/backbones/big_resnet.py
+++ b/pytorch-studiogan_amd/backbones/big_resnet.py
@@ -147,7 +147,7 @@
             for bi, blocklist in enumerate(self.blocks):
                 for block in blocklist:
                     if isinstance(block, ops.SelfAttention):
-                        act = block.forward_nhwc(act, slot)
+                        act = block.forward_nhwc(act, slot, stats=True)
                     else:
                         act = block.forward_nhwc(act, affines[counter], slot)
                         counter += 1
diff --git a/pytorch-studiogan_amd/csrc/conv.hip b/pytorch-studiogan_amd/csrc/conv.hip
--- a/pytorch-studiogan_amd/csrc/conv.hip
+++ b/pytorch-studiogan_amd/csrc/conv.hip
@@ -158,6 +158,34 @@
   return 0;
 }
 
+static int conv_fwd_stats(const sg_conv_fwd_desc* d, float* stats, hipStream_t st, int* rows) {
+  if (d->dtype != SG_DTYPE_BF16 || (d->epi_flags & (SG_EPI_POOL | SG_EPI_OUT_F32 | SG_EPI_ATOMIC)) || d->N <= 0 || d->C <= 0 || d->Cout <= 0) return 0;
+  if (d->R != 1 || d->S != 1 || d->stride != 1 || d->Cout % 8) return 0;
+  const int K = d->C, I = d->Cout;
+  const long long Jll = (long long)d->N * d->Ho * d->Wo;
+  if (Jll >= (1ll << 31) || (long long)d->N * d->Hs * d->Ws * d->ldx >= (1ll << 31)) return 0;
+  const int J = (int)Jll;
+  if (K % 8 || d->ldx % 8 || !aligned16(d->w) || !aligned16(d->x) || (stats && !aligned16(stats))) return 0;
+  const ConvFwdProblem pb = conv_fwd_problem(d, make_epilogue<bf16_t>(d, I, J), I, J, K, d->pix_flags & ~SG_PIX_QUAD);
+  if (rows) return sg_conv_fwd_sk_try(pb, st, nullptr, rows) ? 1 : 0;
+  const int prof = sg_prof_begin(st, 2.0 * (double)I * (double)J * (double)K, 0);
+  const bool ok = sg_conv_fwd_sk_try(pb, st, stats, nullptr);
+  sg_prof_tag(prof, SG_ENG_CONV_SK, 2.0 * ((double)d->N * d->Hs * d->Ws * d->C + (double)I * K + (double)J * I * (1.0 + (d->mask ? 1.0 : 0.0) + (d->res ? 1.0 : 0.0))));
+  sg_prof_end(st, prof);
+  return ok ? 1 : 0;
+}
+extern "C" int sg_conv2d_fwd_stat_rows(const sg_conv_fwd_desc* d) {
+  int rows = 0;
+  if (!d || !d->x || !d->w || !d->out || conv_fwd_stats(d, nullptr, nullptr, &rows) != 1) return 0;
+  return rows;
+}
+extern "C" int sg_conv2d_fwd_stats(const sg_conv_fwd_desc* d, float* stats, sg_stream_t stream) {
+  SG_CHECK(d && d->x && d->w && d->out && stats, "sg_conv2d_fwd_stats: null pointer");
+  SG_CHECK(conv_fwd_stats(d, stats, (hipStream_t)stream, nullptr) == 1, "sg_conv2d_fwd_stats: problem not eligible (ask sg_conv2d_fwd_stat_rows first)");
+  SG_LAUNCH_CHECK();
+  return 0;
+}
+
 extern "C" int sg_conv2d_fwd(const sg_conv_fwd_desc* d, sg_stream_t stream) {
   SG_CHECK(d && d->x && d->w && d->out, "sg_conv2d_fwd: null pointer");
   SG_CHECK(d->N > 0 && d->C > 0 && d->Cout > 0 && d->R > 0 && d->S > 0 && d->stride > 0, "sg_conv2d_fwd: bad shape");
diff --git a/pytorch-studiogan_amd/csrc/conv_common.h b/pytorch-studiogan_amd/csrc/conv_common.h
--- a/pytorch-studiogan_amd/csrc/conv_common.h
+++ b/pytorch-studiogan_amd/csrc/conv_common.h
@@ -83,7 +83,7 @@
   return pb;
 }
 
-bool sg_conv_fwd_sk_try(const ConvFwdProblem& pb, hipStream_t st);
+bool sg_conv_fwd_sk_try(const ConvFwdProblem& pb, hipStream_t st, float* stats = nullptr, int* stat_rows = nullptr);
 bool sg_conv_fwd_rs_try(const ConvFwdProblem& pb, hipStream_t st);
 bool sg_conv_fwd_v4_try(const ConvFwdProblem& pb, hipStream_t st);
 bool sg_conv_fwd_v3_try(const ConvFwdProblem& pb, hipStream_t st);
diff --git a/pytorch-studiogan_amd/csrc/conv_sk.h b/pytorch-studiogan_amd/csrc/conv_sk.h
--- a/pytorch-studiogan_amd/csrc/conv_sk.h
+++ b/pytorch-studiogan_amd/csrc/conv_sk.h
@@ -11,9 +11,10 @@
   unsigned xbytes;
   unsigned obytes, sbytes;
   int nrb;
+  float* stats;
 };
 
-template <int TI, int NP, int TJ, int KS, int NW, bool POOL>
+template <int TI, int NP, int TJ, int KS, int NW, bool POOL, bool STATS = false>
 __global__ __launch_bounds__(64 * NW) void sg_conv_sk_kernel(ConvSkParams p, Epilogue<bf16_t> epi) {
   constexpr int BI = TI * NP * 32;
   constexpr int NCH = 2 * KS;
@@ -103,6 +104,23 @@
   float al = epi.alpha;
   if (epi.alpha_ptr) al *= *epi.alpha_ptr;
   constexpr bool pool = POOL;
+  static_assert(!(STATS && POOL), "statistics of a pooled result are not taken here");
+  constexpr int SPAIRS = TI * 16;
+  static_assert(SPAIRS <= 64, "one lane per cout pair of a pass");
+  float ssum[NP][2], ssq[NP][2];
+#pragma unroll
+  for (int ps = 0; ps < NP; ps++) { ssum[ps][0] = ssum[ps][1] = 0.f; ssq[ps][0] = ssq[ps][1] = 0.f; }
+  auto write_stats = [&]() {
+    float* const srow = p.stats + (long long)(blockIdx.x * NW + wave) * (long long)p.I * 2;
+#pragma unroll
+    for (int ps = 0; ps < NP; ps++) {
+      const int c = i0 + ps * TI * 32 + 2 * lane;
+      if (lane < SPAIRS && c < p.I) {
+        const f32x4 o4 = {ssum[ps][0], ssq[ps][0], ssum[ps][1], ssq[ps][1]};
+        *(f32x4*)(srow + (long long)c * 2) = o4;
+      }
+    }
+  };
   const bool relu_out = (epi.flags & SG_EPI_RELU) != 0;
   const bool pre_mask = epi.mask != nullptr, pre_res = epi.res != nullptr;
   const int Jout = pool ? (epi.J >> 2) : epi.J;
@@ -218,6 +236,18 @@
           }
         }
       asm volatile("s_waitcnt lgkmcnt(0)" ::: "memory");
+      if constexpr (STATS) {
+        const char* const scol = stg + (lane < SPAIRS ? lane : 0) * 4;
+        const int rows_valid = Jout - jbase;
+#pragma unroll 8
+        for (int r = 0; r < ROWS; r++) {
+          uint32_t u = *(const uint32_t*)(scol + r * CP);
+          u = r < rows_valid ? u : 0u;
+          const float a = __uint_as_float(u << 16), b = __uint_as_float(u & 0xffff0000u);
+          ssum[ps][0] += a; ssq[ps][0] += a * a;
+          ssum[ps][1] += b; ssq[ps][1] += b * b;
+        }
+      }
 #pragma unroll
       for (int it = 0; it < NIT; it++) {
         const int idx = lane + 64 * it;
@@ -235,7 +265,10 @@
   const int stride = gridDim.x * NW;
   int rb = blockIdx.x * NW + wave;
   u32x4 qa[TJ][KS], qb[TJ][KS];
-  if (rb >= p.nrb) return;
+  if (rb >= p.nrb) {
+    if constexpr (STATS) write_stats();
+    return;
+  }
   fetch(rb, qa);
 #pragma unroll
   for (int it = 0; it < NP * NIT; it++) {
@@ -252,26 +285,28 @@
     rb += stride;
     if (rb >= p.nrb) break;
   }
+  if constexpr (STATS) write_stats();
 }
 
-template <int TI, int NP, int TJ, int KS, bool POOL>
-static inline int sg_launch_conv_sk_tp(ConvSkParams p, const Epilogue<bf16_t>& e, hipStream_t st) {
+template <int TI, int NP, int TJ, int KS, bool POOL, bool STATS = false>
+static inline int sg_launch_conv_sk_tp(ConvSkParams p, const Epilogue<bf16_t>& e, hipStream_t st, int* stat_rows = nullptr) {
   constexpr int BI = TI * NP * 32, WP = KS * 32 + 16, CP = TI * 64 + 16, ROWS = 32 * TJ;
   constexpr int lds4 = BI * WP + BI * 4 + 4 * ROWS * CP;
   constexpr int NW = (2 * lds4 <= 160 * 1024) ? 4 : 8;
   constexpr int lds = BI * WP + BI * 4 + NW * ROWS * CP;
   static_assert(lds <= 160 * 1024, "LDS");
-  static bool attr_done = false;
-  if (!attr_done) {
-    if (hipFuncSetAttribute((const void*)sg_conv_sk_kernel<TI, NP, TJ, KS, NW, POOL>, hipFuncAttributeMaxDynamicSharedMemorySize, lds) != hipSuccess) return -1;
-    attr_done = true;
-  }
   p.nrb = (p.J + ROWS - 1) / ROWS;
   const int tilesI = (p.I + BI - 1) / BI;
   int gx = (p.nrb + NW - 1) / NW;
   const int cap = (256 * (8 / NW) + tilesI - 1) / tilesI;
   if (gx > cap) gx = cap;
-  hipLaunchKernelGGL((sg_conv_sk_kernel<TI, NP, TJ, KS, NW, POOL>), dim3(gx, tilesI), dim3(64 * NW), lds, st, p, e);
+  if (stat_rows) { *stat_rows = gx * NW; return 0; }
+  static bool attr_done = false;
+  if (!attr_done) {
+    if (hipFuncSetAttribute((const void*)sg_conv_sk_kernel<TI, NP, TJ, KS, NW, POOL, STATS>, hipFuncAttributeMaxDynamicSharedMemorySize, lds) != hipSuccess) return -1;
+    attr_done = true;
+  }
+  hipLaunchKernelGGL((sg_conv_sk_kernel<TI, NP, TJ, KS, NW, POOL, STATS>), dim3(gx, tilesI), dim3(64 * NW), lds, st, p, e);
   return 0;
 }
 template <int TI, int NP, int TJ, int KS>
@@ -279,9 +314,15 @@
   return (e.flags & SG_EPI_POOL) ? sg_launch_conv_sk_tp<TI, NP, TJ, KS, true>(p, e, st) : sg_launch_conv_sk_tp<TI, NP, TJ, KS, false>(p, e, st);
 }
 
-static inline int sg_launch_conv_sk(const ConvSkParams& p, const Epilogue<bf16_t>& e, hipStream_t st) {
+static inline int sg_launch_conv_sk(const ConvSkParams& p, const Epilogue<bf16_t>& e, hipStream_t st, int* stat_rows = nullptr) {
   const int ti = p.I <= 32 ? 1 : p.I <= 64 ? 2 : p.I <= 96 ? 3 : p.I <= 128 ? 4 : 6;
   const int ks = p.K <= 16 ? 1 : p.K <= 48 ? 3 : p.K <= 96 ? 6 : 12;
+  if (p.stats || stat_rows) {
+    if ((e.flags & SG_EPI_POOL) || p.mode3) return -1;
+    if (ti == 3 && ks == 3) return sg_launch_conv_sk_tp<3, 1, 1, 3, false, true>(p, e, st, stat_rows);
+    if (ti == 6 && ks == 6) return sg_launch_conv_sk_tp<3, 2, 1, 6, false, true>(p, e, st, stat_rows);
+    return -1;
+  }
 #define SG_SK_CASE(T_, TI_, NP_, KS_, TJ_) if (ti == T_ && ks == KS_) return sg_launch_conv_sk_t<TI_, NP_, TJ_, KS_>(p, e, st);
   SG_SK_CASE(1, 1, 1, 1, 2) SG_SK_CASE(1, 1, 1, 3, 2) SG_SK_CASE(1, 1, 1, 6, 2) SG_SK_CASE(1, 1, 1, 12, 1)
   SG_SK_CASE(2, 2, 1, 1, 2) SG_SK_CASE(2, 2, 1, 3, 2) SG_SK_CASE(2, 2, 1, 6, 1) SG_SK_CASE(2, 2, 1, 12, 1)
diff --git a/pytorch-studiogan_amd/csrc/conv_sk.hip b/pytorch-studiogan_amd/csrc/conv_sk.hip
--- a/pytorch-studiogan_amd/csrc/conv_sk.hip
+++ b/pytorch-studiogan_amd/csrc/conv_sk.hip
@@ -1,13 +1,13 @@
 #include "conv_common.h"
 #include "conv_sk.h"
 
-bool sg_conv_fwd_sk_try(const ConvFwdProblem& pb, hipStream_t st) {
+bool sg_conv_fwd_sk_try(const ConvFwdProblem& pb, hipStream_t st, float* stats, int* stat_rows) {
   const sg_conv_fwd_desc* d = pb.d;
   const Epilogue<bf16_t>& e = pb.e;
   const int I = pb.I, J = pb.J;
   const char mode = env_mode("SG_CONV_SK");
   if (mode == '0') return false;
-  const bool force = mode == 'f';
+  const bool force = mode == 'f' || stats || stat_rows;
   if (d->stride != 1 || (pb.pflags & SG_PIX_TRANSPOSED)) return false;
   const bool one = d->R == 1 && d->S == 1 && d->pad_h == 0 && d->pad_w == 0 && d->C <= 192;
   const bool stem = is_3x3_s1_p1(d) && d->C == 8 && !pb.up;
@@ -29,5 +29,6 @@
   p.Ho = d->Ho; p.Wo = d->Wo; p.wshift = pb.wshift; p.hshift = pb.hshift;
   p.mode3 = stem ? 1 : 0; p.flags = pb.pflags;
   p.I = I; p.J = J; p.K = pb.K; p.xbytes = (unsigned)pb.xbytes; p.nrb = 0;
-  return sg_launch_conv_sk(p, e, st) == 0;
+  p.stats = stats;
+  return sg_launch_conv_sk(p, e, st, stat_rows) == 0;
 }
diff --git a/pytorch-studiogan_amd/csrc/conv_wgrad.hip b/pytorch-studiogan_amd/csrc/conv_wgrad.hip
--- a/pytorch-studiogan_amd/csrc/conv_wgrad.hip
+++ b/pytorch-studiogan_amd/csrc/conv_wgrad.hip
@@ -33,7 +33,7 @@
   if (s.ok) s.nw = sg_wgrad_sk_waves((int)(K / 32));
   return s;
 }
-static int wgrad_sk_launch(const sg_conv_wgrad_desc* d, const SkPlan& s, hipStream_t st) {
+static int wgrad_sk_launch(const sg_conv_wgrad_desc* d, const SkPlan& s, hipStream_t st, bool unscaled = false) {
   WgradSkParams p;
   const long long K = (long long)d->N * d->Ho * d->Wo;
   const unsigned xbytes = wgrad_xbytes(d), gbytes = wgrad_gbytes(d);
@@ -41,7 +41,7 @@
   p.nchunk = (int)(K / 32);
   p.arelu = (d->x_flags & SG_PIX_RELU) ? 1 : 0;
   p.work = (float*)d->work; p.n = s.n;
-  p.alpha = d->alpha; p.alpha_ptr = d->alpha_ptr;
+  p.alpha = unscaled ? 1.f : d->alpha; p.alpha_ptr = unscaled ? nullptr : d->alpha_ptr;
   const int xup = (d->x_flags & SG_PIX_UPSAMPLE) ? 1 : 0, gup = (d->g_flags & SG_PIX_UPSAMPLE) ? 1 : 0;
   if (!s.swap) {
     p.a = (const bf16_t*)d->x; p.lda = d->ldx; p.CA = d->C; p.upA = xup; p.HsA = d->xHs; p.WsA = d->xWs; p.abytes = xbytes;
@@ -151,7 +151,7 @@
   bool fuses_bias;
   SkPlan sk; V3Plan v3; int BI, BJ;
 };
-static WgradChoice wgrad_choose(const sg_conv_wgrad_desc* d, bool launching) {
+static WgradChoice wgrad_choose(const sg_conv_wgrad_desc* d, bool launching, bool gain = false) {
   WgradChoice c = {};
   const auto have = [&](long long floats) { return !launching || (d->work && d->work_floats >= floats); };
   c.sk = wgrad_sk_plan(d);
@@ -168,7 +168,7 @@
   const int I = d->R * d->S * d->C, J = d->Cout, K = (int)((long long)d->N * d->Ho * d->Wo);
   const bool v2 = wgrad_v2_ok(d);
   wgrad_plan(I, J, K, d->dtype == SG_DTYPE_BF16 ? ET<bf16_t>::BK : ET<float>::BK, d->splits, c.BI, c.BJ, c.splits, v2);
-  c.engine = v2 ? WG_V2 : WG_GEMM; c.n = c.stride = (long long)I * J; c.work_floats = c.splits > 1 ? c.splits * c.n : 0;
+  c.engine = v2 ? WG_V2 : WG_GEMM; c.n = c.stride = (long long)I * J; c.work_floats = (c.splits > 1 || gain) ? c.splits * c.n : 0;
   return c;
 }
 
@@ -255,6 +255,65 @@
   }
 }
 
+struct WgradGain { const bf16_t* w; float* dsigma; float* scratch; };
+#define SG_FINISH_GAIN_MAX_BLOCKS 128
+static_assert(SG_FINISH_GAIN_MAX_BLOCKS + 1 <= SG_WGRAD_DSIGMA_SCRATCH, "scratch");
+__global__ __launch_bounds__(256) void k_splitk_finish_gain(const float* partial, float* out, int splits, long long n, long long stride, const bf16_t* w,
+                                                            float alpha, const float* sigma, float* dsigma, float* scratch) {
+  __shared__ f32x4 sm[4][64];
+  const long long n4 = n >> 2;
+  const int li = threadIdx.x & 63, q = threadIdx.x >> 6;
+  const float scale = alpha * *sigma;
+  float dot = 0.f;
+  for (long long i0 = blockIdx.x * 64ll; i0 < n4; i0 += (long long)gridDim.x * 64) {
+    const long long i = i0 + li;
+    f32x4 a[8];
+#pragma unroll
+    for (int k = 0; k < 8; k++) a[k] = (f32x4){0.f, 0.f, 0.f, 0.f};
+    if (i < n4) {
+      const float* src = partial + 4 * i;
+      int s = q;
+      for (; s + 28 < splits; s += 32) {
+        f32x4 v[8];
+#pragma unroll
+        for (int k = 0; k < 8; k++) v[k] = *(const f32x4*)(src + (long long)(s + 4 * k) * stride);
+#pragma unroll
+        for (int k = 0; k < 8; k++) a[k] += v[k];
+      }
+      for (; s < splits; s += 4) a[0] += *(const f32x4*)(src + (long long)s * stride);
+    }
+    sm[q][li] = ((a[0] + a[1]) + (a[2] + a[3])) + ((a[4] + a[5]) + (a[6] + a[7]));
+    __syncthreads();
+    if (q == 0 && i < n4) {
+      const f32x4 t = (sm[0][li] + sm[1][li]) + (sm[2][li] + sm[3][li]);
+      float* dst = out + 4 * i;
+      const f32x4 o = *(f32x4*)dst;
+      *(f32x4*)dst = o + t * scale;
+      const u32x2 wv = *(const u32x2*)(w + 4 * i);
+      dot += (t[0] * bf2f((bf16_t)(wv[0] & 0xffffu)) + t[1] * bf2f((bf16_t)(wv[0] >> 16))) +
+             (t[2] * bf2f((bf16_t)(wv[1] & 0xffffu)) + t[3] * bf2f((bf16_t)(wv[1] >> 16)));
+    }
+    __syncthreads();
+  }
+  if (q != 0) return;
+#pragma unroll
+  for (int m = 32; m >= 1; m >>= 1) dot += __shfl_xor(dot, m);
+  if (li != 0) return;
+  scratch[1 + blockIdx.x] = dot;
+  const unsigned ticket = __atomic_fetch_add((unsigned*)scratch, 1u, __ATOMIC_ACQ_REL);
+  if (ticket != gridDim.x - 1) return;
+  float total = 0.f;
+  for (unsigned b = 0; b < gridDim.x; b++) total += scratch[1 + b];
+  *dsigma += alpha * total;
+}
+static void splitk_finish_gain_launch(const float* partial, float* out, int splits, long long n, long long stride, const WgradGain& g, float alpha,
+                                      const float* sigma, hipStream_t st) {
+  long long blocks = (n / 4 + 63) / 64;
+  if (blocks > SG_FINISH_GAIN_MAX_BLOCKS) blocks = SG_FINISH_GAIN_MAX_BLOCKS;
+  if (blocks < 1) blocks = 1;
+  hipLaunchKernelGGL(k_splitk_finish_gain, dim3((int)blocks), dim3(256), 0, st, partial, out, splits, n, stride, g.w, alpha, sigma, g.dsigma, g.scratch);
+}
+
 template <typename T, class LM, bool TR, int SPLIT>
 static void conv_wgrad_tiles(const LM& lp, const LM& lq, const Epilogue<T>& e, int I, int J, int K, int BI, int BJ, int splits, hipStream_t st) {
   if (BI == 32) sg_launch_gemm<T, LM, LM, 32, 256, 1, 4, TR, SPLIT>(lp, lq, e, I, J, K, splits, 1, st);
@@ -284,7 +343,7 @@
 template <typename T> static double wgrad_alg_bytes(const sg_conv_wgrad_desc* d) {
   return sizeof(T) * ((double)d->N * d->xHs * d->xWs * d->C + (double)d->N * d->gHs * d->gWs * d->Cout) + 8.0 * (double)d->R * d->S * d->C * d->Cout;
 }
-template <typename T, bool TR> static int conv_wgrad_t(const sg_conv_wgrad_desc* d, hipStream_t st) {
+template <typename T, bool TR> static int conv_wgrad_t(const sg_conv_wgrad_desc* d, hipStream_t st, const WgradGain* gain = nullptr) {
   const int I = d->R * d->S * d->C;
   const int J = d->Cout;
   const long long Kll = (long long)d->N * d->Ho * d->Wo;
@@ -292,12 +351,13 @@
   SG_CHECK((long long)d->N * d->xHs * d->xWs * d->ldx < (1ll << 31) && (long long)d->N * d->gHs * d->gWs * d->ldg < (1ll << 31),
            "sg_conv2d_wgrad: tensor too large for 32-bit element offsets");
   const int K = (int)Kll;
-  const WgradChoice c = wgrad_choose(d, true);
+  const WgradChoice c = wgrad_choose(d, true, gain != nullptr);
+  if (gain) SG_CHECK(c.work_floats > 0 && d->work && d->work_floats >= c.work_floats, "sg_conv2d_wgrad_dsigma: the workspace of sg_conv2d_wgrad_dsigma_plan is required");
   const int prof = sg_prof_begin(st, 2.0 * (double)I * (double)J * (double)K, 1);
   int eng = SG_ENG_WGRAD_GEMM;
   bool two_stage = true;
   if (c.engine == WG_SK) {
-    if (wgrad_sk_launch(d, c.sk, st) != 0) { sg_set_error("sg_conv2d_wgrad: streaming kernel launch failed"); return -2; }
+    if (wgrad_sk_launch(d, c.sk, st, gain != nullptr) != 0) { sg_set_error("sg_conv2d_wgrad: streaming kernel launch failed"); return -2; }
     eng = SG_ENG_WGRAD_SK;
   } else if (c.engine == WG_V3) {
     if (wgrad_v3_launch(d, c.v3, st) != 0) { sg_set_error("sg_conv2d_wgrad: halo kernel launch failed"); return -2; }
@@ -308,7 +368,8 @@
     e.out = d->dw; e.out_bstride = 0; e.ldo = I; e.bias = nullptr; e.res = nullptr; e.res_bstride = 0; e.ldr = 0; e.beta = 0.f;
     e.mask = nullptr; e.mask_bstride = 0; e.ldm = 0; e.alpha = d->alpha; e.alpha_ptr = d->alpha_ptr; e.split_stride = 0;
     e.flags = SG_EPI_OUT_F32; e.I = I; e.J = J;
-    if (c.splits == 1) { e.res = d->dw; e.ldr = I; e.beta = 1.f; e.flags |= SG_EPI_RES_F32; }
+    if (gain) { e.alpha = 1.f; e.alpha_ptr = nullptr; e.out = d->work; e.split_stride = c.n; }
+    else if (c.splits == 1) { e.res = d->dw; e.ldr = I; e.beta = 1.f; e.flags |= SG_EPI_RES_F32; }
     else if (two_stage) { e.out = d->work; e.split_stride = c.n; }
     else e.flags |= SG_EPI_ATOMIC;
     if constexpr (std::is_same_v<T, bf16_t>) {
@@ -321,7 +382,9 @@
       else conv_wgrad_launch<T, TR, false>(d, e, I, J, K, c.BI, c.BJ, c.splits, st);
     }
   }
-  if (two_stage) {
+  if (gain) {
+    splitk_finish_gain_launch((const float*)d->work, d->dw, c.splits, c.n, c.stride, *gain, d->alpha, d->alpha_ptr, st);
+  } else if (two_stage) {
     splitk_reduce_launch((const float*)d->work, d->dw, c.splits, c.n, c.stride, c.fuses_bias ? d->dbias : nullptr, c.fuses_bias ? d->Cout : 0, st);
   }
   sg_prof_tag(prof, eng, wgrad_alg_bytes<T>(d));
@@ -341,3 +404,28 @@
   sg_set_error("sg_conv2d_wgrad: bad dtype");
   return -1;
 }
+
+extern "C" int sg_conv2d_wgrad_dsigma_ok(const sg_conv_wgrad_desc* d) {
+  if (!d || d->dtype != SG_DTYPE_BF16 || d->R != 1 || d->S != 1 || d->stride != 1 || d->pad_h || d->pad_w || !d->alpha_ptr || d->dbias) return 0;
+  if (((long long)d->C * d->Cout) % 4 || (d->x_flags | d->g_flags) & SG_PIX_TRANSPOSED) return 0;
+  return 1;
+}
+
+extern "C" int sg_conv2d_wgrad_dsigma_plan(const sg_conv_wgrad_desc* d, int* splits, long long* work_floats) {
+  SG_CHECK(d && splits && work_floats, "sg_conv2d_wgrad_dsigma_plan: null");
+  SG_CHECK(sg_conv2d_wgrad_dsigma_ok(d) == 1, "sg_conv2d_wgrad_dsigma_plan: not a problem of this entry point (sg_conv2d_wgrad_dsigma_ok)");
+  const WgradChoice c = wgrad_choose(d, false, true);
+  *splits = c.splits;
+  *work_floats = c.work_floats;
+  return 0;
+}
+
+extern "C" int sg_conv2d_wgrad_dsigma(const sg_conv_wgrad_desc* d, const void* w_fwd, float* dsigma, float* scratch, sg_stream_t stream) {
+  SG_CHECK(d && d->x && d->dy && d->dw && w_fwd && dsigma && scratch, "sg_conv2d_wgrad_dsigma: null pointer");
+  SG_CHECK(d->N > 0 && d->C > 0 && d->Cout > 0, "sg_conv2d_wgrad_dsigma: bad shape");
+  SG_CHECK(sg_conv2d_wgrad_dsigma_ok(d) == 1, "sg_conv2d_wgrad_dsigma: not a problem of this entry point (sg_conv2d_wgrad_dsigma_ok)");
+  SG_CHECK(aligned16(d->work) && aligned16(d->dw) && (((uintptr_t)w_fwd) & 7) == 0, "sg_conv2d_wgrad_dsigma: unaligned workspace, gradient or filter image");
+  const WgradGain g = {(const bf16_t*)w_fwd, dsigma, scratch};
+  if (d->no_tr) return conv_wgrad_t<bf16_t, false>(d, (hipStream_t)stream, &g);
+  return conv_wgrad_t<bf16_t, true>(d, (hipStream_t)stream, &g);
+}
diff --git a/pytorch-studiogan_amd/functional/_base.py b/pytorch-studiogan_amd/functional/_base.py
--- a/pytorch-studiogan_amd/functional/_base.py
+++ b/pytorch-studiogan_amd/functional/_base.py
@@ -99,7 +99,7 @@
 
 
 def conv2d_raw(x, w_ptr, Cin, Cout, R, S, stride=1, pad_h=0, pad_w=0, pix_flags=0, epi_flags=0, bias=None, res=None, mask=None,
-               alpha=1.0, beta=1.0, alpha_ptr=None, out=None, ldx=None, transposed_out_hw=None, out_coff=0, x_coff=0, desc=None):
+               alpha=1.0, beta=1.0, alpha_ptr=None, out=None, ldx=None, transposed_out_hw=None, out_coff=0, x_coff=0, desc=None, stats=False):
     N, Hs, Ws = x.shape[0], x.shape[1], x.shape[2]
     ldx = x.shape[3] if ldx is None else ldx
     up = 2 if (pix_flags & L.PIX_UPSAMPLE) else 1
@@ -132,6 +132,13 @@
     d.ldm = mask.shape[-1] if mask is not None else 0
     if desc is not None:
         return out
+    if stats:
+        rows = L.lib().sg_conv2d_fwd_stat_rows(L.C.byref(d))
+        if rows > 0:
+            st = torch.empty((rows, Cout, 2), dtype=torch.float32, device=x.device)
+            L.call("sg_conv2d_fwd_stats", d, st.data_ptr(), L.stream())
+            _offer_stats(out, st, rows, Cout)
+            return out
     L.call("sg_conv2d_fwd", d, L.stream())
     return out
 
@@ -157,7 +164,7 @@
 
 
 def conv2d_wgrad_raw(x, dy, dw_ptr, Cin, Cout, R, S, Ho, Wo, stride=1, pad_h=0, pad_w=0, x_flags=0, g_flags=0, alpha=1.0,
-                     alpha_ptr=None, splits=0, no_tr=0, ldg=None, dy_coff=0, dbias=None):
+                     alpha_ptr=None, splits=0, no_tr=0, ldg=None, dy_coff=0, dbias=None, dsigma=None, w_fwd=None, dry=False):
     d = L.ConvWgradDesc()
     d.dtype = L.dt(x)
     d.N = x.shape[0]
@@ -169,6 +176,19 @@
     d.x, d.dy, d.dw = L.ptr(x), L.ptr(dy) + dy_coff * dy.element_size(), dw_ptr
     d.alpha_ptr = L.ptr(alpha_ptr)
     d.splits, d.no_tr = splits, no_tr
+    if dsigma is not None or dry:
+        ok = dbias is None and L.lib().sg_conv2d_wgrad_dsigma_ok(L.C.byref(d)) == 1
+        if dry:
+            return ok
+        if not ok:
+            raise RuntimeError("conv2d_wgrad_raw: sg_conv2d_wgrad_dsigma does not take this problem (ask with dry=True first)")
+        sp, wf = L.C.c_int(0), L.C.c_longlong(0)
+        L.call("sg_conv2d_wgrad_dsigma_plan", d, L.C.byref(sp), L.C.byref(wf))
+        work = torch.empty(wf.value, dtype=torch.float32, device=x.device)
+        d.splits, d.work, d.work_floats = sp.value, work.data_ptr(), wf.value
+        scratch = zeros_small(L.WGRAD_DSIGMA_SCRATCH, torch.float32, x.device)
+        L.call("sg_conv2d_wgrad_dsigma", d, w_fwd, L.ptr(dsigma), L.ptr(scratch), L.stream())
+        return False
     fused = False
     if dbias is not None:
         d.dbias = L.ptr(dbias)
diff --git a/pytorch-studiogan_amd/functional/attention.py b/pytorch-studiogan_amd/functional/attention.py
--- a/pytorch-studiogan_amd/functional/attention.py
+++ b/pytorch-studiogan_amd/functional/attention.py
@@ -232,6 +232,17 @@
     return os.environ.get("SG_ATTN_PROJ", "1") != "0"
 
 
+def attn_dsigma_on():
+    return os.environ.get("SG_ATTN_DSIGMA", "1") != "0"
+
+
+def attn_out_stats_on():
+    return os.environ.get("SG_ATTN_OUT_STATS", "0") == "1"
+
+
+FUSED_CALLS = {"dsigma": 0, "out_stats": 0}
+
+
 def attn_proj_ok(x, rts):
     rt_t, rt_p, rt_g = rts
     if x.dtype != torch.bfloat16 or x.dim() != 4 or rt_t.rows_pad != rt_p.rows_pad or any(r.RS != 1 or r.trans or r.cin_pad != x.shape[3] for r in rts):
@@ -305,11 +316,16 @@
 class AttnOutFn(torch.autograd.Function):
 
     @staticmethod
-    def forward(ctx, x, o, weight, sigma, rt, slot, link=None):
+    def forward(ctx, x, o, weight, sigma, rt, slot, link=None, stats=False):
         bank = rt.bank()
         x, o = _c(x), _c(o)
         ctx.link = link
-        y = conv2d_raw(o, bank.w_fwd(slot, rt), rt.Cin, rt.rows, 1, 1, res=x, alpha_ptr=sigma)
+        stats = stats and _BN_FUSED_STATS[0] and attn_out_stats_on()
+        if stats:
+            _tick()
+        y = conv2d_raw(o, bank.w_fwd(slot, rt), rt.Cin, rt.rows, 1, 1, res=x, alpha_ptr=sigma, stats=stats)
+        if stats and _STATS_OFFER[0] is not None and _STATS_OFFER[0][0] == _SEQ[0] and _STATS_OFFER[0][1] == y.data_ptr():
+            FUSED_CALLS["out_stats"] += 1
         ctx.save_for_backward(o, sigma)
         ctx.rt, ctx.slot = rt, slot
         ctx.sigma_param = sigma
@@ -324,23 +340,29 @@
             if _param_grad_wanted(ctx.weight, ctx.sigma_param):
                 raise NotImplementedError("create_graph=True is supported for input gradients only (WGAN-GP / R1 path)")
             do = ScalePtrFn.apply(ConvDgradFn.apply(dy, o, ctx.weight, rt, slot, ConvCfg(1, 1)), ctx.sigma_param) if ctx.needs_input_grad[1] else None
-            return (dy if ctx.needs_input_grad[0] else None), do, None, None, None, None, None
+            return (dy if ctx.needs_input_grad[0] else None), do, None, None, None, None, None, None
         bank = rt.bank()
         dy = _c(dy)
         N, H, W, Cc = dy.shape
         do = None
-        if ctx.needs_input_grad[3]:
+        fused = (ctx.needs_input_grad[2] and ctx.needs_input_grad[3] and attn_dsigma_on()
+                 and conv2d_wgrad_raw(o, dy, None, rt.Cin, rt.rows, 1, 1, H, W, alpha_ptr=sigma, dry=True))
+        if ctx.needs_input_grad[3] and not fused:
             t = conv2d_raw(o, bank.w_fwd(slot, rt), rt.Cin, rt.rows, 1, 1)
             g = ensure_grad(ctx.sigma_param)
             L.call("sg_dot", L.dt(dy), L.ptr(dy), L.ptr(t), dy.numel(), L.ptr(g), 1.0, None, L.stream())
         if ctx.needs_input_grad[1]:
             do = conv2d_raw(dy, bank.w_dgrad(slot, rt), rt.rows, rt.Cin, 1, 1, alpha_ptr=sigma)
-        if ctx.needs_input_grad[2]:
+        if fused:
+            FUSED_CALLS["dsigma"] += 1
+            conv2d_wgrad_raw(o, dy, bank.dwt(slot, rt), rt.Cin, rt.rows, 1, 1, H, W, alpha_ptr=sigma, dsigma=ensure_grad(ctx.sigma_param),
+                             w_fwd=bank.w_fwd(slot, rt))
+        elif ctx.needs_input_grad[2]:
             conv2d_wgrad_raw(o, dy, bank.dwt(slot, rt), rt.Cin, rt.rows, 1, 1, H, W, alpha_ptr=sigma)
         dx = dy
         if ctx.link is not None and ctx.link.pending > 0 and ctx.needs_input_grad[0]:
             ctx.link.dx, dx = dy, None
-        return dx, do, None, None, None, None, None
-
-
-__all__ = ['AttnCoreFn', 'AttnOutFn', 'AttnPooledFn', 'AttnProjFn', 'attn_proj_ok', 'attn_proj_on', 'BmmFn', 'MaxPool2BwdFn', 'MaxPool2Fn', 'ScalePtrFn', 'SoftmaxRowsBwdFn', 'SoftmaxRowsFn', '_attn_reference_graph', '_maxpool2_bwd']
+        return dx, do, None, None, None, None, None, None
+
+
+__all__ = ['AttnCoreFn', 'AttnOutFn', 'AttnPooledFn', 'AttnProjFn', 'attn_proj_ok', 'attn_proj_on', 'attn_dsigma_on', 'attn_out_stats_on', 'FUSED_CALLS','BmmFn', 'MaxPool2BwdFn', 'MaxPool2Fn', 'ScalePtrFn', 'SoftmaxRowsBwdFn', 'SoftmaxRowsFn', '_attn_reference_graph', '_maxpool2_bwd']
diff --git a/pytorch-studiogan_amd/ops.py b/pytorch-studiogan_amd/ops.py
--- a/pytorch-studiogan_amd/ops.py
+++ b/pytorch-studiogan_amd/ops.py
@@ -282,7 +282,7 @@
             m._sg_rows_pad = pad8
         self.sigma = nn.Parameter(torch.zeros(1), requires_grad=True)
 
-    def forward_nhwc(self, x, slot=None):
+    def forward_nhwc(self, x, slot=None, stats=False):
         link = F.GradLink(chain=True) if (F._GRAD_LINK[0] and torch.is_grad_enabled() and x.requires_grad) else None
         rt = self.conv1x1_attn._sg_rt
         slot = slot if slot is not None else rt.bank().current
@@ -296,7 +296,7 @@
             phi = self.conv1x1_phi.forward_nhwc(x, slot, link=link)
             g = self.conv1x1_g.forward_nhwc(x, slot, link=link)
             o = F.AttnCoreFn.apply(theta, phi, g)
-        return F.AttnOutFn.apply(x, o, self.conv1x1_attn.master_weight, self.sigma, rt, slot, link)
+        return F.AttnOutFn.apply(x, o, self.conv1x1_attn.master_weight, self.sigma, rt, slot, link, stats)
 
     def forward(self, x):
         _, bank = _root_and_bank(self.conv1x1_theta)
```

Result: no change. 2096 (median of 6 runs) (+0.6%).
